# Xneonz0/JPEG-DSP-Studio

Measured on AMD Instinct MI355X. Metric: Mpixels/s forward+inverse pipeline @ Q=50 4:2:0; PSNR vs ref, higher is better.
Workload: dtype f32+f64; 1 GPU; 1920x1080 RGB, Q=50, 4:2:0, prefilter=on, 8x8 blocks (BASELINE configs[1]); global_batch_frames=64, pipeline=serial forward then inverse per step, parallelism=frame-shard x1, world_size=1, quant_table=local (one rank)

## Files before the change

### include/jds.h

```cpp
#ifndef JDS_H
#define JDS_H

#include <stdint.h>

#ifdef __cplusplus
extern "C" {
#endif

#define JDS_ABI_VERSION 3

#define JDS_OK       0
#define JDS_EINVAL  (-1)
#define JDS_ENOTSUP (-2)
#define JDS_EHIP    (-3)
#define JDS_ENOMEM  (-4)

#define JDS_SS_444 0
#define JDS_SS_422 1
#define JDS_SS_420 2
#define JDS_SS_GRAY 3

#define JDS_RUN_SSE 1u
#define JDS_RUN_FWD 2u
#define JDS_RUN_INV 4u
// ... 350 lines not shown
  int64_t H, W;
  int32_t has_box;
  float box[4];
  int32_t reserved;
} jds_resize_item;
int jds_resize_info(int32_t* tile_h, int32_t* tile_w, int32_t* max_taps);
int jds_rgb_resize(jds_ctx* ctx, const uint8_t* rgb, int32_t rgb_on_device, int64_t H, int64_t W, const float* box,
                   int64_t out_h, int64_t out_w, int32_t resample, uint8_t* out, int32_t out_on_device);
int jds_rgb_batch_resize(jds_ctx* ctx, const uint8_t* rgb_base_dev, const jds_resize_item* items, int32_t n,
                         int64_t out_h, int64_t out_w, int32_t resample, uint8_t* out_dev, void* stream);
int jds_jpeg_batch_to_tensor(jds_ctx* ctx, const uint8_t* const* data, const int64_t* lens, int32_t n, int64_t out_h,
                             int64_t out_w, int32_t resample, const int32_t* scale_denoms, const float* boxes,
                             uint8_t* out, int64_t out_cap, int32_t out_on_device, jds_jpeg_batch_item* items,
                             jds_jpeg_scaled_item* scaled, uint32_t* rounds_out);
int jds_selftest_resize(const uint8_t* rgb, int64_t H, int64_t W, const float* box, int64_t out_h, int64_t out_w,
                        int32_t resample, uint8_t* out, int64_t* worst);
int jds_selftest_resize_coeffs(int32_t in_size, float in0, float in1, int32_t out_size, int32_t resample,
                               int32_t* ksize, int32_t* bounds, int32_t* taps, int64_t cap);

#define JDS_PJPEG_MAX_SCANS 64
typedef struct {
  int32_t n_components;
  int32_t component[3];
  int32_t dc_table[3], ac_table[3];
  int32_t ss, se, ah, al;
  int32_t restart_interval;
  int32_t reserved;
  int64_t offset, length;
  int64_t dc_dht[3], ac_dht[3];
} jds_pjpeg_scan;

typedef struct {
  jds_jpeg_info frame;
  int32_t n_scans;
  int32_t complete;
  uint32_t status;
  uint32_t reserved;
  jds_pjpeg_scan scan[JDS_PJPEG_MAX_SCANS];
} jds_pjpeg_info;

int jds_pjpeg_parse(const uint8_t* data, int64_t len, jds_pjpeg_info* out);
int jds_pjpeg_decode(jds_ctx* ctx, const uint8_t* data, int64_t len, int16_t* coeffs, int64_t coeffs_cap,
                     jds_pjpeg_info* info);
int jds_pjpeg_decode_dev(jds_ctx* ctx, const uint8_t* data, int64_t len, int16_t* coeffs_dev, int64_t coeffs_cap,
                         jds_pjpeg_info* info);
int jds_selftest_pjpegdec(const uint8_t* data, int64_t len, int16_t* coeffs, int64_t coeffs_cap, jds_pjpeg_info* info);
int jds_pjpeg_scan_times(jds_ctx* ctx, double* us, int64_t cap, int64_t* count);
int jds_pjpeg_batch_layout(const uint8_t* const* data, const int64_t* lens, int32_t n, jds_jpeg_batch_item* items,
                           int64_t* rgb_bytes, int64_t* coef_entries, const int32_t* scale_denoms,
                           jds_jpeg_scaled_item* scaled);
int jds_pjpeg_batch_to_rgb(jds_ctx* ctx, const uint8_t* const* data, const int64_t* lens, int32_t n, uint8_t* rgb,
                           int64_t rgb_cap, int32_t rgb_on_device, int32_t render, const int32_t* scale_denoms,
                           jds_jpeg_batch_item* items, jds_jpeg_scaled_item* scaled, int16_t* coeffs);
int jds_pjpeg_to_rgb(jds_ctx* ctx, const uint8_t* data, int64_t len, uint8_t* rgb_out, int64_t rgb_cap,
                     int32_t rgb_on_device, int32_t render, int32_t scale_denom, int16_t* coeffs,
                     jds_pjpeg_info* info);
int jds_pjpeg_batch_transcode(jds_ctx* ctx, const uint8_t* const* data, const int64_t* lens, int32_t n,
                              int32_t optimize, uint8_t* out, int64_t out_cap, int32_t out_on_device,
                              jds_jpeg_transcode_item* items, int64_t* out_bytes);
int jds_pjpeg_transcode(jds_ctx* ctx, const uint8_t* data, int64_t len, int32_t optimize, uint8_t* out,
                        int64_t out_cap, int64_t* out_len, jds_pjpeg_info* info);

int jds_selftest_huffdec(const uint8_t* data, int64_t len, int32_t subseq_bits, int16_t* coeffs, int64_t coeffs_cap,
                         int32_t* rounds_out);

int jds_selftest_dct8x8(const double* in, double* out, int64_t n, int32_t inverse);
int jds_selftest_dct16x16(const double* in, double* out, int64_t n, int32_t inverse);

int jds_selftest_fwd32(int32_t subsampling, int32_t prefilter, const double* gauss, const uint8_t* rgb, int64_t H,
                       int64_t W, int32_t plane, int32_t rows_first, float* coeffs, double* bound);
int jds_selftest_fwd16(int32_t subsampling, int32_t prefilter, const double* gauss, const uint8_t* rgb, int64_t H,
                       int64_t W, int32_t plane, int32_t rows_first, float* coeffs, double* bound);

int jds_selftest_inv_fast(int32_t subsampling, const int16_t* coeffs, const double* qtable, int64_t H, int64_t W,
                          int32_t fuse, double* values, uint8_t* bytes);

int jds_selftest_inv_cert(const double* values, int64_t n, uint8_t* bytes, uint8_t* certain, double* consts);

int jds_selftest_inv_fast16(int32_t subsampling, const int16_t* coeffs, const double* qtable, int64_t H, int64_t W,
                            int32_t fuse, double* values, uint8_t* bytes);

int jds_selftest_inv_rows(int32_t subsampling, int64_t H, int32_t ty, int32_t* out, uint8_t* need);

int jds_selftest_area_tab(int32_t src, int32_t dst, int32_t* n, int32_t* si, double* a);

#ifdef __cplusplus
}
#endif

#endif
```

### jpeg-dsp-studio_amd/csrc/jds_abi.hip

```cpp
#include <algorithm>
#include <mutex>
#include <new>
#include <string>

#include "jds_abi.hpp"
#include "jds_dct16.hpp"
#include "jds_dct8.hpp"

#ifdef JDS_INV6
#define JDS_INV6_LIST 1
#else
#define JDS_INV6_LIST 0
#endif

static const double SSIM_C1 = (0.01 * 255) * (0.01 * 255);
static const double SSIM_C2 = (0.03 * 255) * (0.03 * 255);

thread_local char g_err[512] = "";

constexpr int SSIM_ROWS_MIN = 32;
constexpr size_t SSIM_SCRATCH = (size_t)16 << 30;

static int run_ssim_batch(jds_ctx* c, int items, const uint8_t* const* a, const uint8_t* const* b, int H, int W,
                          double* out, int out_stride, unsigned long long* sse) {
// ... 3 lines not shown
  auto bytes_of = [&](int k) {
    return ssim_batch_scratch_doubles(H, W, !rows, ssim_batch_planes(k)) * sizeof(double) * (size_t)k;
  };
  int group = std::min(per, items);
  if (bytes_of(group) > budget) {
    const size_t each_np = ssim_batch_scratch_doubles(H, W, !rows, false) * sizeof(double);
    group = (int)std::max<size_t>(1, std::min<size_t>((size_t)group, budget / each_np));
    if (ssim_batch_planes(group) && bytes_of(group) > budget) {
      const size_t each_p = ssim_batch_scratch_doubles(H, W, !rows, true) * sizeof(double);
      group = (int)std::max<size_t>(1, std::min<size_t>((size_t)group, budget / each_p));
    }
  }
  size_t need = bytes_of(group);
  const int last = items % group;
  if (last) need = std::max(need, bytes_of(last));
  HIP_TRY(c->ss_planes.ensure(need));
  if (!c->ss_side) {
    HIP_TRY(hipStreamCreateWithFlags(&c->ss_side, hipStreamNonBlocking));
    HIP_TRY(hipEventCreateWithFlags(&c->ss_fork, hipEventDisableTiming));
    HIP_TRY(hipEventCreateWithFlags(&c->ss_join, hipEventDisableTiming));
  }
  const size_t pbytes = sizeof(const void*) * 2 * (size_t)items;
  if (c->ss_pairs_cap < pbytes) {
    if (c->ss_pairs_host) HIP_TRY(hipHostFree(c->ss_pairs_host));
    c->ss_pairs_host = nullptr;
    c->ss_pairs_cap = 0;
    HIP_TRY(hipHostMalloc(&c->ss_pairs_host, pbytes, hipHostMallocDefault));
    c->ss_pairs_cap = pbytes;
  }
  const void** ph = (const void**)c->ss_pairs_host;
  for (int i = 0; i < items; ++i) {
    ph[2 * i] = a[i];
    ph[2 * i + 1] = b[i];
  }
  HIP_TRY(c->ss_pairs.ensure(pbytes));
  HIP_TRY(hipMemcpyAsync(c->ss_pairs.p, ph, pbytes, hipMemcpyHostToDevice, c->stream));
  auto pairs_at = [&](int i0) { return (const void*)((const char*)c->ss_pairs.p + sizeof(const void*) * 2 * (size_t)i0); };
  if (sse) HIP_TRY(hipMemsetAsync(sse, 0, sizeof(unsigned long long) * items, c->stream));
  if (rows) {
    const size_t each_rgb = ssim_rgb_scratch_doubles(H, W) * sizeof(double);
    const int group_rgb = (int)std::min<size_t>((size_t)items, std::max<size_t>(1, ((size_t)4 << 30) / each_rgb));
    HIP_TRY(c->ss_rgb.ensure(each_rgb * group_rgb));
    HIP_TRY(hipEventRecord(c->ss_fork, c->stream));
    HIP_TRY(hipStreamWaitEvent(c->ss_side, c->ss_fork, 0));
    for (int i0 = 0; i0 < items; i0 += group_rgb) {
      const int k = std::min(group_rgb, items - i0);
#ifdef JDS_SSIM_PROBE_NORGB
      continue;
#endif
      HIP_TRY(launch_ssim_rgb(pairs_at(i0), k, H, W, SSIM_C1, SSIM_C2, (double*)c->ss_rgb.p,
                              out + (size_t)i0 * out_stride, out_stride, c->ss_side));
    }
    HIP_TRY(hipEventRecord(c->ss_join, c->ss_side));
  }
  for (int i0 = 0; i0 < items; i0 += group) {
    const int k = std::min(group, items - i0);
#ifdef JDS_SSIM_PROBE_NOLUMA
    if (rows) continue;
#endif
    HIP_TRY(launch_psnr_ssim_batch(pairs_at(i0), k, H, W, SSIM_C1, SSIM_C2, (double*)c->ss_planes.p,
                                   out + (size_t)i0 * out_stride, out_stride, sse ? sse + i0 : nullptr, c->stream,
                                   !rows, c->ss_side, c->ss_fork, c->ss_join));
  }
  if (rows) HIP_TRY(hipStreamWaitEvent(c->stream, c->ss_join, 0));
  return JDS_OK;
}

static int run_ssim(jds_ctx* c, const uint8_t* a, const uint8_t* b, int H, int W, double* dres) {
  return run_ssim_batch(c, 1, &a, &b, H, W, dres, 5, nullptr);
}

struct jds_plan {
  jds_ctx* ctx = nullptr;
  int n = 0, mode = 0;
  int nq = 1;
  DevBuf dct32;
  bool pf = false;
  Geo g{};
  DevBuf fq, gk, part;
  DevBuf fq32, gk32, fixbits, fixlist, counters, part32;
  DevBuf invfix;
  DevBuf invlist;
  unsigned inv_runs = 0;
  bool last_inv_fast = false;
  bool inv_fast_ok = true;
  bool inv_fast_any = true;
  bool last_fwd16_fast = false;
  unsigned fwd16_runs = 0;
  unsigned fwd8_runs = 0;
  int last_fwd8_bank = -1;
  InvFix inv_fix() const {
    return {(unsigned*)invfix.p, (unsigned*)invfix.p + 16, 0, (int)(inv_runs & 1u), (int)(inv_runs % 3u),
            (int)(inv_runs % 16u == 15u), (uint2*)invlist.p, 0};
  }
  bool apriori_ok = false;
  DevBuf planes;
  double* qt = nullptr;
  DevBuf ent[8], ent_hdr, ent_tab;
  DevBuf dec_tab, dec_scr, dec_info;
  unsigned dec_rounds = 0;
  DevBuf rst_hdr, rst_work;
  int rst_hdr_interval = 0;
  DevBuf gen_tab, gen_sub, gen_rec;
  GenBufs gen() const { return {(const AreaTap*)gen_tab.p, (double*)gen_sub.p, (double*)gen_rec.p}; }
  bool prof_on = false;
  KMarks marks;
};

namespace jds {
thread_local KMarks* t_kmarks = nullptr;

void kmark(hipStream_t s, const char* fmt, ...) {
  KMarks* m = t_kmarks;
  if (!m) return;
  if (m->n >= m->cap) {
    m->dropped++;
    return;
  }
  if (hipEventRecord(m->ev[m->n], s) != hipSuccess) return;
  va_list ap;
  va_start(ap, fmt);
  vsnprintf(m->name[m->n], sizeof m->name[0], fmt, ap);
  va_end(ap);
  m->n++;
}
}

struct MarkScope {
  explicit MarkScope(jds_plan* p, hipStream_t s) {
    if (!p->prof_on) return;
    t_kmarks = &p->marks;
    kmark(s, "(between runs)");
  }
  ~MarkScope() { t_kmarks = nullptr; }
};

static void marks_release(KMarks& m) {
  for (int i = 0; i < m.cap; ++i) (void)hipEventDestroy(m.ev[i]);
  free(m.ev);
  free(m.name);
  m = KMarks{};
}


static int make_geo(const jds_params* p, int64_t H, int64_t W, Geo* g, int* mode_out, bool* pf_out) {
  if (!p || !g) return fail(JDS_EINVAL, "null argument");
  if (p->block_size != 8 && p->block_size != 16)
    return fail(JDS_ENOTSUP, "operands could not be broadcast together with shapes (%d,%d) (8,8) ",
                p->block_size, p->block_size);
  const int B = p->block_size;
  if (p->subsampling < JDS_SS_444 || p->subsampling > JDS_SS_420)
    return fail(JDS_EINVAL, "Unknown subsampling mode: %d", p->subsampling);
  if (int rc = check_taps(p->gauss, p->subsampling, p->prefilter)) return rc;
  if (H < 1 || W < 1 || H > 65536 || W > 65536 || H * W > (int64_t)1 << 28)
    return fail(JDS_EINVAL, "unsupported image size %lldx%lld", (long long)H, (long long)W);
  const int mode = p->subsampling;
  const int sy = mode == JDS_SS_420 ? 2 : 1, sx = mode == JDS_SS_444 ? 1 : 2;
  if (H / sy < 1 || W / sx < 1)
    return fail(JDS_EINVAL,
                "OpenCV(4.8.0) resize.cpp: error: (-215:Assertion failed) !dsize.empty() in function 'resize' "
                "(image %lldx%lld, %s)",
                (long long)H, (long long)W, mode == JDS_SS_420 ? "4:2:0" : "4:2:2");
  const bool gen = (sy == 2 && (H % 2)) || (sx == 2 && (W % 2));
  if (gen && B == 16)
    return fail(JDS_ENOTSUP, "16x16 blocks with an odd %s image size (%lldx%lld) are not supported",
                mode == JDS_SS_420 ? "4:2:0" : "4:2:2", (long long)H, (long long)W);
// ... 262 lines not shown
  if ((e = p->fq.ensure(sizeof(FrameQ) * n)) != hipSuccess || (e = p->gk.ensure(3 * sizeof(double))) != hipSuccess ||
      (e = p->part.ensure(sizeof(double) * (size_t)n *
                          (size_t)std::max(std::max(g.tiles_y * g.tiles_x, g.gen ? gen_px_tiles(g) : 0),
                                           g.bs == 16 ? inv16_tiles(mode, (int)H, (int)W) : 0))) !=
          hipSuccess ||
      (e = hipMemcpy(p->fq.p, hq, sizeof(FrameQ) * n, hipMemcpyHostToDevice)) != hipSuccess ||
      (e = hipMemcpy(p->gk.p, params[0].gauss, 3 * sizeof(double), hipMemcpyHostToDevice)) != hipSuccess) {
    free(hq);
    p->fq.release();
    p->gk.release();
    p->part.release();
    delete p;
    return fail(e == hipErrorOutOfMemory ? JDS_ENOMEM : JDS_EHIP, "plan upload: %s", hipGetErrorString(e));
  }
  free(hq);
  if (g.gen) {
    if ((rc = gen_prepare(g, n_frames, n, p->gen_tab, p->gen_sub, p->gen_rec, ctx->stream))) {
      jds_plan_destroy(p);
      return rc;
    }
  } else if (g.bs == 16) {
    const size_t fqs = fast_q16_size();
    char* h16 = (char*)malloc(fqs * (size_t)n);
    if (!h16) {
      jds_plan_destroy(p);
      return fail(JDS_ENOMEM, "host allocation failed");
    }
    for (int i = 0; i < n; ++i) fast_fwd16_thresholds(params[i].qtable, mode, pf, params[i].gauss, h16 + fqs * i);
    float gk32[5];
    combined_taps32(params[0].gauss, gk32);
    const size_t nblk = (size_t)n * (size_t)(g.cpf / 256);
    if ((e = p->planes.ensure(mode == JDS_SS_444 ? sizeof(double) * 2 * (size_t)n * g.hc * g.wc : 8)) !=
            hipSuccess ||
        (e = p->fq32.ensure(fqs * n)) != hipSuccess || (e = p->gk32.ensure(sizeof gk32)) != hipSuccess ||
        (e = p->fixlist.ensure(8 * nblk)) != hipSuccess || (e = p->counters.ensure(64)) != hipSuccess ||
        (e = p->invfix.ensure(64 + 12 * (size_t)n)) != hipSuccess ||
        (e = hipMemset(p->invfix.p, 0, 64 + 12 * (size_t)n)) != hipSuccess ||
        (e = p->part32.ensure(sizeof(uint32_t) * 52 * (size_t)n * g.tiles_y * g.tiles_x)) != hipSuccess ||
        (e = hipMemcpy(p->fq32.p, h16, fqs * n, hipMemcpyHostToDevice)) != hipSuccess ||
        (e = hipMemcpy(p->gk32.p, gk32, sizeof gk32, hipMemcpyHostToDevice)) != hipSuccess ||
        (e = hipMemset(p->counters.p, 0, 64)) != hipSuccess) {
      free(h16);
      jds_plan_destroy(p);
      return fail(e == hipErrorOutOfMemory ? JDS_ENOMEM : JDS_EHIP, "plan upload: %s", hipGetErrorString(e));
    }
    free(h16);
  } else {
    const size_t fqs = fast_q_size();
    char* h32 = (char*)malloc(fqs * (size_t)n);
    if (!h32) {
      jds_plan_destroy(p);
      return fail(JDS_ENOMEM, "host allocation failed");
    }
    for (int i = 0; i < n; ++i) {
      float* f = (float*)(h32 + fqs * i);
      fast_fwd_thresholds(params[i].qtable, mode, pf, params[i].gauss, f, f + 64);
    }
    const double* gs = params[0].gauss;
    float gk32[5];
    combined_taps32(gs, gk32);
    const size_t nblk = (size_t)n * (size_t)(g.cpf / 64);
    const size_t ptiles = (size_t)(n_q > 1 ? quant_mq_tiles(g) : g.tiles_y * g.tiles_x);
    if ((e = p->fq32.ensure(fqs * n)) != hipSuccess || (e = p->gk32.ensure(sizeof gk32)) != hipSuccess ||
        (e = p->fixbits.ensure(4 * (size_t)n * (size_t)fix_wpi(g))) != hipSuccess ||
        (e = p->fixlist.ensure(8 * nblk)) != hipSuccess ||
        (e = p->counters.ensure(8 * (size_t)n + 64)) != hipSuccess ||
        (e = p->part32.ensure(sizeof(uint32_t) * (n_q > 1 ? 52 * (size_t)n * ptiles
                                                          : std::max((size_t)52 * n * ptiles, fast_part_words(g, n))))) !=
            hipSuccess ||
        (e = hipMemset(p->part32.p, 0, p->part32.n)) != hipSuccess ||
        (e = p->invfix.ensure(64 + 12 * (size_t)n)) != hipSuccess ||
        (e = hipMemset(p->invfix.p, 0, 64 + 12 * (size_t)n)) != hipSuccess ||
        (JDS_INV6_LIST && mode == JDS_SS_420 && (e = p->invlist.ensure(8 * (size_t)n * inv_tiles(mode, (int)H, (int)W))) != hipSuccess) ||
        (n_q > 1 && (e = p->dct32.ensure(sizeof(float) * (size_t)n_frames * g.cpf)) != hipSuccess) ||
        (e = hipMemcpy(p->fq32.p, h32, fqs * n, hipMemcpyHostToDevice)) != hipSuccess ||
        (e = hipMemcpy(p->gk32.p, gk32, sizeof gk32, hipMemcpyHostToDevice)) != hipSuccess ||
        (e = hipMemset(p->counters.p, 0, 8 * (size_t)n + 64)) != hipSuccess ||
        (e = hipMemset(p->fixbits.p, 0, 4 * (size_t)n * (size_t)fix_wpi(g))) != hipSuccess) {
      free(h32);
      jds_plan_destroy(p);
      return fail(e == hipErrorOutOfMemory ? JDS_ENOMEM : JDS_EHIP, "plan upload: %s", hipGetErrorString(e));
    }
    free(h32);
    if (p->inv_fast_any && !p->inv_fast_ok) {
      std::vector<unsigned> seed(3 * (size_t)n, 0u);
      const unsigned nt = (unsigned)inv_tiles(mode, (int)H, (int)W);
      for (int i = 0; i < n; ++i)
        if (params[i].qtable[0] > 60.0) seed[i] = seed[n + i] = seed[2 * (size_t)n + i] = nt;
      if ((e = hipMemcpy((unsigned*)p->invfix.p + 16, seed.data(), sizeof(unsigned) * seed.size(),
                         hipMemcpyHostToDevice)) != hipSuccess) {
        jds_plan_destroy(p);
        return fail(JDS_EHIP, "plan upload: %s", hipGetErrorString(e));
      }
    }
  }
  *out = p;
  return JDS_OK;
}

int jds_plan_fix_counts(const jds_plan* p, uint32_t* counts) {
  if (!p || !counts) return fail(JDS_EINVAL, "null argument");
  counts[0] = counts[1] = 0u;
  if (p->g.bs == 16) {
    hipError_t e = hipDeviceSynchronize();
    if (e == hipSuccess && p->last_fwd16_fast)
      e = hipMemcpy(counts, (const uint32_t*)p->counters.p + 2, 4, hipMemcpyDeviceToHost);
    if (e == hipSuccess && p->last_inv_fast)
      e = hipMemcpy(counts + 1, (const uint32_t*)p->invfix.p + ((p->inv_runs + 1u) & 1u), 4, hipMemcpyDeviceToHost);
    if (e != hipSuccess) return fail(JDS_EHIP, "fix_counts: %s", hipGetErrorString(e));
    return JDS_OK;
  }
  if (p->g.gen || p->counters.n < 8 * (size_t)p->n) return JDS_OK;
  uint32_t* c = (uint32_t*)malloc(4 * (size_t)p->n + 4);
  if (!c) return fail(JDS_ENOMEM, "fix_counts: host allocation");
  hipError_t e = hipDeviceSynchronize();
  const int bank = p->nq > 1 ? 1 : (p->last_fwd8_bank < 0 ? 1 : p->last_fwd8_bank);
  if (e == hipSuccess)
    e = hipMemcpy(c, (const uint32_t*)p->counters.p + bank * p->n, 4 * (size_t)p->n, hipMemcpyDeviceToHost);
  if (e == hipSuccess && p->last_inv_fast)
    e = hipMemcpy(c + p->n, (const uint32_t*)p->invfix.p + ((p->inv_runs + 1u) & 1u), 4, hipMemcpyDeviceToHost);
  if (e != hipSuccess) {
    free(c);
    return fail(JDS_EHIP, "fix_counts: %s", hipGetErrorString(e));
  }
  for (int i = 0; i < p->n; ++i) counts[0] += std::min(c[i], (uint32_t)(p->g.cpf / 64));
  counts[1] = p->last_inv_fast ? c[p->n] : 0u;
  free(c);
  return JDS_OK;
}

int jds_plan_geometry(const jds_plan* p, jds_geometry* out) {
  if (!p || !out) return fail(JDS_EINVAL, "null argument");
  fill_geometry(p->g, p->mode, out);
  return JDS_OK;
}

int jds_plan_run(jds_plan* p, const uint8_t* rgb, uint8_t* rgb_out, int16_t* coeffs, jds_frame_stats* stats,
                 uint32_t flags, void* stream) {
  if (!p || !rgb || !rgb_out || !coeffs || !stats) return fail(JDS_EINVAL, "null argument");
  if (((uintptr_t)rgb | (uintptr_t)rgb_out | (uintptr_t)coeffs | (uintptr_t)stats) & 15u)
    return fail(JDS_EINVAL, "rgb, rgb_out, coeffs and stats must be 16-byte aligned");
  hipStream_t s = (hipStream_t)stream;
  const MarkScope marks_(p, s);
  int phases = (flags & JDS_RUN_FWD ? 1 : 0) | (flags & JDS_RUN_INV ? 2 : 0);
  if (!phases) phases = 3;
  const bool exact = (flags & JDS_RUN_EXACT) != 0;
  if (p->g.gen) {
    if (phases & 1) HIP_TRY(hipMemsetAsync(stats, 0, sizeof(jds_frame_stats) * p->n, s));
    const GenBufs gb = p->gen();
    HIP_TRY(launch_codec(p->mode, p->pf, p->g, p->n, rgb, rgb_out, coeffs, (const FrameQ*)p->fq.p,
                         (const double*)p->gk.p, stats, (double*)p->part.p, (flags & JDS_RUN_SSE) != 0, nullptr,
                         nullptr, nullptr, 0, s, nullptr, phases, p->nq, &gb));
    return JDS_OK;
  }
  if (p->g.bs == 16) {
    const Fwd16Fast ff{p->fq32.p, (const float*)p->gk32.p, (uint32_t*)p->part32.p, (uint2*)p->fixlist.p,
                       (unsigned*)p->counters.p,
                       (flags & JDS_RUN_FWD_FIXALL) ? 1 : 0, (int)(p->fwd16_runs & 1u)};
    if (phases & 1) HIP_TRY(hipMemsetAsync(stats, 0, sizeof(jds_frame_stats) * p->n, s));
    InvFix fx16 = p->inv_fix();
    fx16.fix_all = (flags & JDS_RUN_INV_FIXALL) ? 1 : 0;
    const bool fast_inv16 = (phases & 2) && !exact && !(flags & JDS_RUN_EXACT_INV) &&
                            !(flags & JDS_RUN_SSE) && p->mode != JDS_SS_444 && p->invfix.p;
    HIP_TRY(launch_codec16(p->mode, p->pf, p->g, p->n, rgb, rgb_out, coeffs, (const FrameQ*)p->fq.p,
                           (const double*)p->gk.p, stats, (double*)p->part.p, (double*)p->planes.p,
                           (flags & JDS_RUN_SSE) != 0, nullptr, nullptr, s, nullptr, phases, exact ? nullptr : &ff,
                           fast_inv16 ? &fx16 : nullptr));
    if (phases & 1) {
      p->last_fwd16_fast = !exact;
      if (!exact) p->fwd16_runs++;
    }
    if (phases & 2) {
      p->last_inv_fast = fast_inv16;
      if (fast_inv16) p->inv_runs++;
    }
    return JDS_OK;
  }
  if (phases & 1) {
    if (exact) HIP_TRY(hipMemsetAsync(stats, 0, sizeof(jds_frame_stats) * p->n, s));
    if (exact)
      HIP_TRY(launch_codec(p->mode, p->pf, p->g, p->n, rgb, rgb_out, coeffs, (const FrameQ*)p->fq.p,
                           (const double*)p->gk.p, stats, (double*)p->part.p, false, nullptr, nullptr, nullptr, 0,
                           s, nullptr, 1, p->nq, nullptr));
    else
      HIP_TRY(launch_fast_fwd(p->mode, p->pf, p->g, p->n, p->nq, rgb, coeffs, (const FrameQ*)p->fq.p, p->fq32.p,
                              (const double*)p->gk.p, (const float*)p->gk32.p, stats, (uint32_t*)p->part32.p,
                              (uint32_t*)p->fixbits.p, (uint2*)p->fixlist.p, (unsigned*)p->counters.p,
                              (float*)p->dct32.p, s,
                              phases == 1,
                              (int)(p->fwd8_runs & 1u)));
    if (!exact && p->nq == 1) p->last_fwd8_bank = (int)(p->fwd8_runs++ & 1u);
  }
  InvFix fx = p->inv_fix();
  fx.fix_all = (flags & JDS_RUN_INV_FIXALL) ? 1 : 0;
  fx.apriori = phases == 3 && p->apriori_ok;
  const bool exact_inv = exact || (flags & JDS_RUN_EXACT_INV) != 0 || (!p->inv_fast_any && !(flags & JDS_RUN_INV_FAST));
  if (phases & 2)
    HIP_TRY(launch_codec(p->mode, p->pf, p->g, p->n, rgb, rgb_out, coeffs, (const FrameQ*)p->fq.p,
                         (const double*)p->gk.p, stats, (double*)p->part.p, (flags & JDS_RUN_SSE) != 0, nullptr,
                         nullptr, nullptr, 0, s, nullptr, exact ? 6 : (phases == 3 ? 2 | 8 : 2), p->nq, nullptr,
                         exact_inv || !p->invfix.p ? nullptr : &fx));
  if (phases & 2) {
    const bool sse444 = (flags & JDS_RUN_SSE) && p->mode == JDS_SS_444;
    p->last_inv_fast = !exact_inv && p->invfix.p && !sse444;
    if (p->last_inv_fast) p->inv_runs++;
  }
  return JDS_OK;
}

static int marks_enable(KMarks& marks, bool& on, int device, int enable) {
  if (enable && !marks.cap) {
    HIP_TRY(hipSetDevice(device));
    const int cap = 8192;
    KMarks m;
    m.ev = (hipEvent_t*)calloc(cap, sizeof(hipEvent_t));
    m.name = (char(*)[64])calloc(cap, sizeof *m.name);
    if (!m.ev || !m.name) {
      free(m.ev);
      free(m.name);
      return fail(JDS_ENOMEM, "host allocation failed");
    }
    for (; m.cap < cap; ++m.cap) {
      hipError_t e = hipEventCreateWithFlags(&m.ev[m.cap], hipEventDisableSystemFence);
      if (e != hipSuccess) {
        marks_release(m);
        return fail(JDS_EHIP, "hipEventCreate: %s", hipGetErrorString(e));
      }
    }
    marks = m;
  }
  on = enable != 0;
  marks.n = 0;
  marks.dropped = 0;
  return JDS_OK;
}

int jds_plan_profile(jds_plan* p, int enable) {
  if (!p) return fail(JDS_EINVAL, "null argument");
  return marks_enable(p->marks, p->prof_on, p->ctx->device, enable);
}

static int marks_read(KMarks& m, int device, jds_kernel_time* out, int max, int* n_out, double* span_ms) {
  if (!n_out || (max > 0 && !out)) return fail(JDS_EINVAL, "null argument");
  *n_out = 0;
  if (span_ms) *span_ms = 0.0;
  if (m.dropped) {
    const long long d = m.dropped;
    if (m.n) (void)hipEventSynchronize(m.ev[m.n - 1]);
    m.n = 0;
    m.dropped = 0;
    return fail(JDS_EINVAL, "profile overflow: %lld launch marks dropped (pool of %d); read every <= %d runs",
                d, m.cap, m.cap / 8);
  }
  if (m.n < 2) {
    m.n = 0;
    return JDS_OK;
  }
  HIP_TRY(hipSetDevice(device));
  HIP_TRY(hipEventSynchronize(m.ev[m.n - 1]));
  int k = 0;
  for (int i = 1; i < m.n; ++i) {
    float ms = 0.f;
    HIP_TRY(hipEventElapsedTime(&ms, m.ev[i - 1], m.ev[i]));
    int j = 0;
    while (j < k && strncmp(out[j].name, m.name[i], sizeof out[j].name) != 0) ++j;
    if (j == k) {
      if (k == max) continue;
      memset(&out[k], 0, sizeof out[k]);
      snprintf(out[k].name, sizeof out[k].name, "%s", m.name[i]);
      ++k;
    }
    out[j].total_ms += ms;
    out[j].launches += 1;
  }
  if (span_ms) {
    float ms = 0.f;
    HIP_TRY(hipEventElapsedTime(&ms, m.ev[0], m.ev[m.n - 1]));
    *span_ms = ms;
  }
  *n_out = k;
  m.n = 0;
  return JDS_OK;
}

int jds_plan_profile_read(jds_plan* p, jds_kernel_time* out, int max, int* n_out, double* span_ms) {
  if (!p) return fail(JDS_EINVAL, "null argument");
  return marks_read(p->marks, p->ctx->device, out, max, n_out, span_ms);
}

int jds_ctx_profile(jds_ctx* c, int enable) {
  if (!c) return fail(JDS_EINVAL, "null argument");
  return marks_enable(c->marks, c->prof_on, c->device, enable);
}

int jds_ctx_profile_read(jds_ctx* c, jds_kernel_time* out, int max, int* n_out, double* span_ms) {
  if (!c) return fail(JDS_EINVAL, "null argument");
  return marks_read(c->marks, c->device, out, max, n_out, span_ms);
}

void jds_plan_destroy(jds_plan* p) {
  if (!p) return;
  (void)hipSetDevice(p->ctx->device);
  (void)hipStreamSynchronize(p->ctx->stream);
  p->fq.release();
  p->gk.release();
  p->part.release();
  p->fq32.release();
  p->gk32.release();
  p->fixlist.release();
  p->counters.release();
  p->fixbits.release();
  p->part32.release();
  p->invfix.release();
  p->invlist.release();
  p->planes.release();
  p->dct32.release();
  p->gen_tab.release();
  p->gen_sub.release();
  p->gen_rec.release();
  for (DevBuf& b : p->ent) b.release();
  p->ent_hdr.release();
  p->ent_tab.release();
  p->dec_tab.release();
  p->dec_scr.release();
  p->dec_info.release();
  p->rst_hdr.release();
  p->rst_work.release();
  free(p->qt);
  marks_release(p->marks);
  delete p;
}

int jds_compress_reconstruct(jds_ctx* c, const jds_params* prm, const uint8_t* rgb, int64_t H, int64_t W,
                             uint8_t* rgb_out, int16_t* coeffs, jds_frame_stats* stats, double* error_map_y,
                             double* error_map_rgb, int32_t sel_by, int32_t sel_bx, jds_selected_block* sel,
                             int32_t* sel_valid) {
  if (!c || !prm || !rgb || !rgb_out || !stats) return fail(JDS_EINVAL, "null argument");
  if ((error_map_y == nullptr) != (error_map_rgb == nullptr))
    return fail(JDS_EINVAL, "error_map_y and error_map_rgb must be requested together");
  Geo g;
  int mode;
  bool pf;
  int rc = make_geo(prm, H, W, &g, &mode, &pf);
  if (rc) return rc;
  if ((rc = check_tables(prm))) return rc;
  HIP_TRY(hipSetDevice(c->device));
  const size_t npx = (size_t)H * (size_t)W, nimg = npx * 3, ncf = (size_t)g.cpf;
  const int tiles = std::max(std::max(g.tiles_y * g.tiles_x, g.gen ? gen_px_tiles(g) : 0),
                             g.bs == 16 ? inv16_tiles(mode, (int)H, (int)W) : 0);
  HIP_TRY(c->rgb.ensure(nimg));
  HIP_TRY(c->out.ensure(nimg));
  HIP_TRY(c->coeffs.ensure(ncf * sizeof(int16_t)));
  HIP_TRY(c->stats.ensure(sizeof(jds_frame_stats)));
  HIP_TRY(c->part.ensure(sizeof(double) * tiles));
  HIP_TRY(c->fq.ensure(sizeof(FrameQ)));
  HIP_TRY(c->gk.ensure(3 * sizeof(double)));
  const bool maps = error_map_y != nullptr;
  if (maps) {
    HIP_TRY(c->erry.ensure(npx * sizeof(double)));
    HIP_TRY(c->errrgb.ensure(npx * sizeof(double)));
  }
  int sel_blk = -1;
  if (sel && g.bs == 16) {
    if (sel_valid) *sel_valid = 0;
  } else if (sel) {
    const long long bpr = g.nbx;
    const long long ti = (long long)sel_by * bpr + sel_bx;
    const long long nyb = (long long)g.nby * g.nbx;
    if (ti >= 0 && ti < nyb) sel_blk = (int)ti;
    if (sel_valid) *sel_valid = sel_blk >= 0;
    if (sel_blk >= 0) HIP_TRY(c->sel.ensure(sizeof(jds_selected_block)));
  }
  FrameQ hq;
  make_fq(prm, &hq);
  hipStream_t s = c->stream;
  GenBufs gb{};
  if (g.gen) {
    if ((rc = gen_prepare(g, 1, 1, c->gen_tab, c->gen_sub, c->gen_rec, s))) return rc;
    gb = {(const AreaTap*)c->gen_tab.p, (double*)c->gen_sub.p, (double*)c->gen_rec.p};
  }
  HIP_TRY(hipMemcpyAsync(c->fq.p, &hq, sizeof hq, hipMemcpyHostToDevice, s));
  HIP_TRY(hipMemcpyAsync(c->gk.p, prm->gauss, 3 * sizeof(double), hipMemcpyHostToDevice, s));
  HIP_TRY(hipMemcpyAsync(c->rgb.p, rgb, nimg, hipMemcpyHostToDevice, s));
  HIP_TRY(hipMemsetAsync(c->stats.p, 0, sizeof(jds_frame_stats), s));
  jds_selected_block* dsel = sel_blk >= 0 ? (jds_selected_block*)c->sel.p : nullptr;
  if (g.bs == 16) {
// ... 739 lines not shown
    return fail(JDS_EINVAL, "bad argument");
  const bool pf = prefilter != 0 && subsampling != JDS_SS_444;
  double E[128];
  fast_fwd_bounds(subsampling, pf, gauss, E);
  memcpy(bound, E + (plane ? 64 : 0), 64 * sizeof(double));
  if (fwd32_host_plane(subsampling, pf, gauss, rgb, (int)H, (int)W, plane, rows_first, coeffs))
    return fail(JDS_EINVAL, "plane size must be a multiple of 8");
  return JDS_OK;
}

int jds_selftest_fwd16(int32_t subsampling, int32_t prefilter, const double* gauss, const uint8_t* rgb, int64_t H,
                       int64_t W, int32_t plane, int32_t rows_first, float* coeffs, double* bound) {
  if (!gauss || !rgb || !coeffs || !bound || H < 1 || W < 1 || H > 4096 || W > 4096 || plane < 0 || plane > 2 ||
      subsampling < JDS_SS_444 || subsampling > JDS_SS_420)
    return fail(JDS_EINVAL, "bad argument");
  const bool pf = prefilter != 0 && subsampling != JDS_SS_444;
  double E[512];
  fast_fwd16_bounds(subsampling, pf, gauss, E);
  memcpy(bound, E + (plane ? 256 : 0), 256 * sizeof(double));
  if (fwd16_host_plane(subsampling, pf, gauss, rgb, (int)H, (int)W, plane, rows_first, coeffs))
    return fail(JDS_EINVAL, "plane size must be a multiple of 16");
  return JDS_OK;
}

int jds_selftest_inv_fast(int32_t subsampling, const int16_t* coeffs, const double* qtable, int64_t H, int64_t W,
                          int32_t fuse, double* values, uint8_t* bytes) {
  if (!coeffs || !qtable || !values || !bytes || H < 1 || W < 1 || H > 4096 || W > 4096 ||
      subsampling < JDS_SS_444 || subsampling > JDS_SS_420)
    return fail(JDS_EINVAL, "bad argument");
  if (inv_fast_host(subsampling, coeffs, qtable, (int)H, (int)W, fuse, 8, values, bytes))
    return fail(JDS_EINVAL, "odd chroma geometry: the certified inverse runs even sizes only");
  return JDS_OK;
}

int jds_selftest_inv_cert(const double* values, int64_t n, uint8_t* bytes, uint8_t* certain, double* consts) {
  if (!values || !bytes || !certain || !consts || n < 0) return fail(JDS_EINVAL, "bad argument");
  for (int64_t i = 0; i < n; ++i)
    if (!(fabs(values[i]) < 0x1p+19)) return fail(JDS_EINVAL, "values[%lld] outside (-2^19, 2^19)", (long long)i);
  inv_cert_forms_host(values, n, bytes, certain, consts);
  return JDS_OK;
}

int jds_selftest_inv_fast16(int32_t subsampling, const int16_t* coeffs, const double* qtable, int64_t H, int64_t W,
                            int32_t fuse, double* values, uint8_t* bytes) {
  if (!coeffs || !qtable || !values || !bytes || H < 1 || W < 1 || H > 4096 || W > 4096 ||
      subsampling < JDS_SS_444 || subsampling > JDS_SS_420)
    return fail(JDS_EINVAL, "bad argument");
  if (inv_fast_host(subsampling, coeffs, qtable, (int)H, (int)W, fuse, 16, values, bytes))
    return fail(JDS_EINVAL, "odd chroma geometry: the certified inverse runs even sizes only");
  return JDS_OK;
}

int jds_selftest_area_tab(int32_t src, int32_t dst, int32_t* n, int32_t* si, double* a) {
  if (src < 1 || dst < 1 || dst > src || !n || !si || !a) return fail(JDS_EINVAL, "bad argument");
  AreaTap* t = (AreaTap*)malloc(sizeof(AreaTap) * (size_t)dst);
  if (!t) return fail(JDS_ENOMEM, "host allocation failed");
  if (area_tab_build(src, dst, t) < 0) {
    free(t);
    return fail(JDS_EINVAL, "more than 4 taps per sample");
  }
  for (int d = 0; d < dst; ++d) {
    n[d] = t[d].n;
    for (int k = 0; k < 4; ++k) {
      si[4 * d + k] = k < t[d].n ? t[d].si[k] : -1;
      a[4 * d + k] = k < t[d].n ? t[d].a[k] : 0.0;
    }
  }
  free(t);
  return JDS_OK;
}

int jds_selftest_inv_rows(int32_t subsampling, int64_t H, int32_t ty, int32_t* out, uint8_t* need) {
  if (!out || H < 1 || H > 65536 || ty < 0 || subsampling < JDS_SS_444 || subsampling > JDS_SS_420)
    return fail(JDS_EINVAL, "bad argument");
  int o[8];
  inv_rows(subsampling, (int)H, ty, o);
  for (int i = 0; i < 8; ++i) out[i] = o[i];
  if (need)
    for (int i = 0; i < o[5]; ++i)
      for (int r = 0; r < 8; ++r) need[8 * i + r] = (uint8_t)inv_rows_need(subsampling, (int)H, ty, o[4] + i, r);
  return JDS_OK;
}

int jds_selftest_dct16x16(const double* in, double* out, int64_t n, int32_t inverse) {
  if (!in || !out || n < 0) return fail(JDS_EINVAL, "bad argument");
  for (int64_t b = 0; b < n; ++b) {
    double t[256], c[16];
    memcpy(t, in + 256 * b, sizeof t);
    for (int col = 0; col < 16; ++col) {
      for (int i = 0; i < 16; ++i) c[i] = t[i * 16 + col];
      if (inverse) dct3_line16(c); else dct2_line16(c);
      for (int i = 0; i < 16; ++i) t[i * 16 + col] = c[i];
    }
    for (int r = 0; r < 16; ++r) {
      if (inverse) dct3_line16(t + 16 * r); else dct2_line16(t + 16 * r);
    }
    for (int i = 0; i < 256; ++i) out[256 * b + i] = t[i] * 0.03125;
  }
  return JDS_OK;
}

}
```

### jpeg-dsp-studio_amd/csrc/jds_abi.hpp

```cpp
#pragma once

#include <hip/hip_runtime.h>
#include <math.h>
#include <stdarg.h>
#include <stdio.h>
#include <stdlib.h>
#include <string.h>

#include <cmath>
#include <thread>
#include <vector>

#include "jds_huffdec.hpp"
#include "jds_huffopt.hpp"
#include "jds_internal.hpp"
#include "jds_jpeg_inv.hpp"

namespace jds {
hipError_t launch_codec(int mode, bool pf, const Geo& g, int n, const uint8_t* rgb, uint8_t* rgb_out,
                        int16_t* coeffs, const FrameQ* fq, const double* gk, jds_frame_stats* st,
                        double* part, bool want_sse, double* err_y, double* err_rgb, jds_selected_block* sel,
                        int sel_blk, hipStream_t s, hipEvent_t* ev, int phases, int in_div, const GenBufs* gb,
                        const InvFix* fx = nullptr);
int inv_tiles(int mode, int H, int W);
void inv_rows(int mode, int H, int ty, int* out);
int inv_rows_need(int mode, int H, int ty, int by, int r);
int area_tab_build(int src, int dst, AreaTap* tab);
size_t gen_sub_doubles(const Geo& g);
size_t gen_rec_doubles(const Geo& g);
int gen_px_tiles(const Geo& g);
hipError_t stage_area_gen(const double* in, int H, int W, const AreaTap* ytab, const AreaTap* xtab, double* out,
                          int oh, int ow, hipStream_t s);
hipError_t launch_psnr_ssim_batch(const void* pairs_dev, int items, int H, int W, double c1, double c2,
                                  double* scratch, double* out, int out_stride, unsigned long long* sse,
                                  hipStream_t s, bool rgb, hipStream_t side, hipEvent_t fork, hipEvent_t join);
hipError_t launch_ssim_rgb(const void* pairs_dev, int items, int H, int W, double c1, double c2, double* scratch,
                           double* out, int out_stride, hipStream_t s);
size_t ssim_batch_scratch_doubles(int H, int W, bool rgb, bool planes);
bool ssim_batch_planes(int items);
size_t ssim_rgb_scratch_doubles(int H, int W);
int ssim_batch_max_items();
hipError_t launch_sse_u8(const uint8_t* a, const uint8_t* b, long long n, unsigned long long* out, hipStream_t s);
size_t mag_scratch_bytes(long long nblocks, int max_chunks);
hipError_t launch_mag_f32(const int16_t* coeffs, long long nblocks, unsigned* chunk_sum, int max_chunks,
                          double* out, hipStream_t s);
void combined_taps32(const double* gk, float* out5);
size_t fast_part_words(const Geo& g, int n);
hipError_t launch_fast_fwd(int mode, bool pf, const Geo& g, int n, int nq, const uint8_t* rgb, int16_t* coeffs,
                           const FrameQ* fq, const void* fq32, const double* gk, const float* gk32,
                           jds_frame_stats* st, uint32_t* part, uint32_t* fixbits, uint2* fixlist, unsigned* fixcount,
                           float* dct32,
                           hipStream_t s, bool finish, int par);
int quant_mq_tiles(const Geo& g);
int inv16_tiles(int mode, int H, int W);
constexpr int MAXQ_SHARED = 8;
void fast_fwd_bounds(int mode, bool pf, const double* gk, double* E);
int fwd32_host_plane(int mode, bool pf, const double* gk, const uint8_t* rgb, int H, int W, int plane,
                     int flags, float* out);
void fast_fwd_thresholds(const double* Q, int mode, bool pf, const double* gk, float* rq, float* thr);
int inv_fast_host(int mode, const int16_t* cf, const double* Q, int H, int W, int fuse, int block, double* vout,
                  uint8_t* bout);
void inv_cert_forms_host(const double* v, long long n, uint8_t* bytes, uint8_t* certain, double* consts);
size_t fast_q_size();
hipError_t stage_rgb_ycc(const double* in, double* out, long long n, int inverse, hipStream_t s);
hipError_t stage_subsample(const double* in, double* tmp, double* tmp2, double* out, int H, int W, int sy,
                           int prefilter, const double* k, hipStream_t s);
hipError_t stage_resize(const double* in, int h, int w, double* out, int H, int W, int nearest, hipStream_t s);
hipError_t stage_block(const double* in, double* out, long long n, int bs, int op, hipStream_t s);
hipError_t stage_quant(const void* in, const double* q, void* out, long long n, int dequant, int period,
                       hipStream_t s);
int tile_dims16(int mode, int* MY, int* MX);
struct EntTab;
void ent_build_tables(EntTab* t);
size_t ent_tab_size();
int ent_header(const double* q, int mode, int H, int W, uint8_t* o);
long long ent_capacity(const Geo& g);
void ent_sizes(const Geo& g, int n, size_t* sz);
hipError_t launch_entropy(const Geo& g, int n, const int16_t* coeffs, void* const* buf, const uint8_t* hdr_dev,
                          const void* tab_dev, uint8_t* out, long long stride, unsigned long long* lengths,
                          unsigned long long* scan_bits, hipStream_t s);
int ent_restart_interval();
int ent_header_rst(const double* q, int mode, int H, int W, int interval, uint8_t* o);
long long ent_capacity_rst(const Geo& g);
hipError_t launch_entropy_rst(const Geo& g, int n, const int16_t* coeffs, void* const* buf, const uint8_t* hdr_dev,
                              const void* tab_dev, uint8_t* out, long long stride, unsigned long long* lengths,
                              unsigned long long* scan_bits, hipStream_t s);
long long ent_capacity_opt(const Geo& g, bool rst);
hipError_t launch_entropy_opt(const Geo& g, int n, const int16_t* coeffs, void* const* buf, const uint8_t* hdr_dev,
                              const void* tab_dev, uint8_t* out, long long stride, unsigned long long* lengths,
                              unsigned long long* scan_bits, hipStream_t s);
hipError_t launch_entropy_rst_opt(const Geo& g, int n, const int16_t* coeffs, void* const* buf,
                                  const uint8_t* hdr_dev, const void* tab_dev, uint8_t* out, long long stride,
                                  unsigned long long* lengths, unsigned long long* scan_bits, hipStream_t s);
int ent_std_table(int idx, const uint8_t** bits, const uint8_t** vals);
void opt_table_host(const uint32_t* freq, HoTable* t);
hipError_t launch_opt_tables_selftest(int n, const uint32_t* freq, uint8_t* bits, uint8_t* vals, int32_t* nv,
                                      int32_t* fell, hipStream_t s);
void rst_constants(int* lane_max);
int rst_group_lanes();
size_t rst_work_bytes(int n, const RstGeo& rg);
hipError_t launch_dec_rst(const uint8_t* files, const RstIv* ivs_dev, long long niv, const HuffDecTab* tabs_dev,
                          int16_t* coeffs, uint32_t* status, hipStream_t s, const HdMcu* mcu_dev);
hipError_t launch_dec_rst_plan(const uint8_t* files, long long stride, const unsigned long long* lengths,
                               const uint8_t* hdr_dev, int hl, int n, const RstGeo& rg, void* work,
                               const HuffDecTab* tabs_dev, int16_t* coeffs, uint32_t* status, hipStream_t s);
void dec_constants(int* s, int* g);
long long dec_layout(DecScan* sc, int nscans, int* max_ngrp);
size_t dec_scratch_bytes(long long ngroups, int nscans);
size_t dec_hdr_bytes(int n);
hipError_t launch_dec_hdr(const uint8_t* files, long long stride, const unsigned long long* lengths,
                          const uint8_t* hdr_dev, int hl, int n, void* work, uint32_t* status, hipStream_t s);
hipError_t dec_run(const uint8_t* files, const DecScan* sc, int nscans, long long ngroups, int max_ngrp,
                   const HuffDecTab* tabs_dev, void* scratch, int16_t* coeffs, long long n_coeffs, uint32_t* status,
                   hipStream_t s, unsigned* rounds, int* too_many, const HdMcu* mcu_dev, int16_t* dcs);
hipError_t dec_run_groups(const uint8_t* files, const DecGroup* grp, int ngrp, const HuffDecTab* tabs_dev,
                          int16_t* coeffs, long long n_coeffs, uint32_t* status, hipStream_t s, unsigned* rounds,
                          int* too_many, const HdMcu* mcu_dev, int16_t* dcs);
hipError_t launch_codec16(int mode, bool pf, const Geo& g, int n, const uint8_t* rgb, uint8_t* rgb_out,
                          int16_t* coeffs, const FrameQ* fq, const double* gk, jds_frame_stats* st, double* part,
                          double* planes, bool want_sse, double* err_y, double* err_rgb, hipStream_t s,
                          hipEvent_t* ev, int phases, const Fwd16Fast* ff, const InvFix* fx);
void fast_fwd16_bounds(int mode, bool pf, const double* gk, double* E);
void fast_fwd16_thresholds(const double* Q8, int mode, bool pf, const double* gk, void* out);
size_t fast_q16_size();
int fwd16_host_plane(int mode, bool pf, const double* gk, const uint8_t* rgb, int H, int W, int plane,
                     int flags, float* out);
void jpeg_inv_constants(int* th, int* tw);
bool jpeg_inv_fits(const JInvArgs& a);
hipError_t launch_jpeg_inv(const JInvArgs& a, const int16_t* coeffs, uint8_t* rgb, hipStream_t s);
void jpeg_inv_host(const JInvArgs& a, const int16_t* coeffs, uint8_t* rgb);
hipError_t launch_jpeg_inv_batch(const JInvRec* recs, const JInvMap* maps, const int map_off[JI_MODES],
                                 const int nmap[JI_MODES], const int tiles[JI_MODES], const uint32_t* status,
                                 const int16_t* coeffs, uint8_t* rgb, hipStream_t s);
hipError_t launch_jpeg_ljt(const JInvArgs& a, const int16_t* coeffs, uint8_t* rgb, hipStream_t s);
hipError_t launch_jpeg_ljt_batch(const JInvRec* recs, const JInvMap* maps, const int map_off[JI_MODES],
// ... 159 lines not shown
```

### jpeg-dsp-studio_amd/csrc/jds_fast.hip

```cpp
#include <hip/hip_runtime.h>
#include <math.h>
#include <stdint.h>
#include <stdlib.h>

#include "jds_dct8.hpp"
#include "jds_device.hpp"
#include "jds_internal.hpp"
#include "jds_fwd_common.hpp"

#pragma clang fp contract(off)


namespace jds {

#define JA 0x1.6a09e6p-2f
#define JC1 0x1.f6297cp-2f
#define JC2 0x1.d906bcp-2f
#define JC3 0x1.a9b662p-2f
#define JC5 0x1.1c73b4p-2f
#define JC6 0x1.87de2ap-3f
#define JC7 0x1.8f8b84p-4f

static constexpr float FW[8][4] = {
    {JA, JA, JA, JA},      {JC1, JC3, JC5, JC7},    {JC2, JC6, -JC6, -JC2}, {JC3, -JC7, -JC1, -JC5},
    {JA, -JA, -JA, JA},    {JC5, -JC1, JC7, JC3},   {JC6, -JC2, JC2, -JC6}, {JC7, -JC5, JC3, -JC1},
};

__host__ __device__ __forceinline__ void fdct8_f32(float (&x)[8]) {
  const float s0 = x[0] + x[7], s1 = x[1] + x[6], s2 = x[2] + x[5], s3 = x[3] + x[4];
  const float d0 = x[0] - x[7], d1 = x[1] - x[6], d2 = x[2] - x[5], d3 = x[3] - x[4];
#pragma unroll
  for (int k = 0; k < 8; k += 2) {
    x[k] = fmaf(FW[k][3], s3, fmaf(FW[k][2], s2, fmaf(FW[k][1], s1, FW[k][0] * s0)));
    x[k + 1] = fmaf(FW[k + 1][3], d3, fmaf(FW[k + 1][2], d2, fmaf(FW[k + 1][1], d1, FW[k + 1][0] * d0)));
  }
}

__device__ __forceinline__ void unpack32(uint32_t v, float& R, float& G, float& B) {
  R = (float)(v & 255u);
  G = (float)((v >> 8) & 255u);
  B = (float)(v >> 16);
}

struct FastQ {
  float rq[64];
  float thr[2][64];
};

constexpr int BS32 = 72;

template <int SY>
__device__ __forceinline__ int csw(int row) { return (row / SY) & 3; }

template <int SY>
__device__ __forceinline__ int psw(int row) { return (row / SY) & 7; }

__device__ __forceinline__ uint32_t byte_at(const uint32_t (&w)[6], int b) { return (w[b >> 2] >> (8 * (b & 3))) & 255u; }

struct LaneStats {
  unsigned nz = 0u, mb = 0u, hn = 0u, nflag = 0u;
};

constexpr int RH_COPIES = 4, RH_STRIDE = 53;
constexpr int RH_WORDS = RH_COPIES * RH_STRIDE + 64;

__device__ __forceinline__ unsigned rare_bin_total(const unsigned* s_rh, int b) {
  unsigned t = 0u;
#pragma unroll
  for (int c = 0; c < RH_COPIES; ++c) t += s_rh[c * RH_STRIDE + b] + (b == 49 ? s_rh[c * RH_STRIDE + 50] : 0u);
  return t;
}

template <bool REPL = false>
__device__ __forceinline__ void quant8(const float (&v)[8], const float (&rq)[8], const float (&thr)[8], bool valid,
                                       int (&q)[8], LaneStats& ls, unsigned* s_st) {
  unsigned nrare = 0u;
  unsigned ok = 0xffffffffu, orr = 0u;
  unsigned top;
  asm("v_mov_b32 %0, 0x80000000" : "=v"(top));
#pragma unroll
  for (int k = 0; k < 8; ++k) {
    const float t = v[k] * rq[k];
    const float f = t + QMAGIC;
    const float r = f - QMAGIC;
    const uint32_t fb = __float_as_uint(f);
    const float e = fabsf(t - r) - fmaf(fabsf(t), -0x1p-22f, thr[k]);
    ok &= __float_as_uint(e);
    q[k] = (int)(fb - QMAGIC_BITS);
    const int x = __builtin_amdgcn_frexp_expf(r);
    ls.nz += (unsigned)(x + 15) >> 4;
    ls.mb += (unsigned)x;
    const unsigned o = fb - (QMAGIC_BITS - 12u);
    ls.hn += top >> ((o & 28u) ^ 31u);
    orr |= o;
  }
  ls.nflag += (~ok) >> 31;
  nrare = REPL ? orr : (orr >= 32u ? 1u : 0u);
  if constexpr (REPL) {
    if (nrare >= 32u) {
      const int lane = threadIdx.x & 63;
      unsigned* copy = s_st + (lane & (RH_COPIES - 1)) * RH_STRIDE;
      unsigned* dummy = s_st + RH_COPIES * RH_STRIDE + lane;
#pragma unroll
      for (int k = 0; k < 8; ++k) {
        const unsigned o = (unsigned)(q[k] + 12);
        const bool rare = o >= 32u;
        ls.hn -= rare ? 1u << (o & 28u) : 0u;
        const unsigned h = (unsigned)(q[k] + 100);
        atomicAdd(rare && valid && h <= 200u ? copy + (h >> 2) : dummy, 1u);
      }
    }
  } else if (nrare != 0u) {
#pragma unroll
    for (int k = 0; k < 8; ++k) {
      const unsigned o = (unsigned)(q[k] + 12);
      if (o >= 32u) {
        ls.hn -= 1u << (o & 28u);
        if (valid && (unsigned)(q[k] + 100) <= 200u) atomicAdd(&s_st[2 + (q[k] == 100 ? 49 : (q[k] + 100) >> 2)], 1u);
      }
    }
  }
}

__device__ __forceinline__ uint4 pack_q(const int (&q)[8]) {
  return make_uint4((uint32_t)(uint16_t)q[0] | ((uint32_t)(uint16_t)q[1] << 16),
                    (uint32_t)(uint16_t)q[2] | ((uint32_t)(uint16_t)q[3] << 16),
                    (uint32_t)(uint16_t)q[4] | ((uint32_t)(uint16_t)q[5] << 16),
                    (uint32_t)(uint16_t)q[6] | ((uint32_t)(uint16_t)q[7] << 16));
}

__device__ __forceinline__ void flag_block_list(const LaneStats& ls, bool valid, int line, int item, int plane,
                                                int bidx, uint2* fixlist, unsigned* fixcount, long long cap) {
  const unsigned long long fm = __ballot(valid && ls.nflag != 0u);
  if (!fm) return;
  const int lane = threadIdx.x & 63;
  const bool mine = valid && line == 0 && ((fm >> (lane & ~7)) & 0xffull);
  const unsigned long long lm = __ballot(mine);
  unsigned base = 0u;
  if (lane == __ffsll((long long)lm) - 1) base = atomicAdd(fixcount + item, (unsigned)__popcll(lm));
  base = __shfl(base, __ffsll((long long)lm) - 1, 64);
  if (mine) {
    const unsigned slot = base + (unsigned)__popcll(lm & ((1ull << lane) - 1ull));
    if (slot < (unsigned long long)cap)
      fixlist[(size_t)item * cap + slot] = make_uint2((unsigned)item, ((unsigned)plane << 24) | (unsigned)bidx);
  }
}

__device__ __forceinline__ void flag_block_bits(const LaneStats& ls, bool valid, int line, int item, long long gblk,
                                                uint32_t* fixbits, int wpi) {
  const unsigned long long fm = __ballot(valid && ls.nflag != 0u);
  if (!fm) return;
  const int lane = threadIdx.x & 63;
  if (valid && line == 0 && ((fm >> (lane & ~7)) & 0xffull))
    atomicOr(fixbits + (size_t)item * wpi + (gblk >> 5), 1u << (gblk & 31));
}

constexpr int NW_MAX = 8;
__device__ __forceinline__ void stats_flush(LaneStats ls, bool valid, uint32_t* __restrict__ slot) {
  if (!valid) ls = LaneStats();
  const unsigned h = ls.hn;
  unsigned v[3] = {h & 0x0f0f0f0fu, (h >> 4) & 0x0f0f0f0fu, ls.nz | ((valid ? 1u : 0u) << 8) | (ls.mb << 16)};
  row_sums3(v);
  const int lane = threadIdx.x & 63, w = threadIdx.x >> 6;
  if ((lane & 15) == 15)
    *reinterpret_cast<uint4*>(slot + 4 * (4 * w + (lane >> 4))) = make_uint4(v[0], v[1], v[2], 0u);
}

constexpr int PSLOT = 128;
__device__ __forceinline__ unsigned* rare_row(uint32_t* part, const Geo& g, int nframes, int frame) {
  return part + (size_t)nframes * g.tiles_y * g.tiles_x * PSLOT + (size_t)frame * 64;
}

template <int MODE, bool PF, bool MQ = false>
__global__ void __launch_bounds__(Cfg<MODE>::TF)
k_fwd32(const Geo g, const uint8_t* __restrict__ rgb, int16_t* __restrict__ coeffs,
        const FastQ* __restrict__ fq, const float* __restrict__ gk32, uint32_t* __restrict__ part,
        uint2* __restrict__ fixlist, unsigned* __restrict__ fixcount, const int border, const int4 rect,
        float* __restrict__ dct32,
        jds_frame_stats* __restrict__ stz, const int nzq) {
  using C = Cfg<MODE>;
  constexpr int WR = C::TH + 2, WC = C::TW + 2, WN = WR * WC;
  constexpr bool CPLANE = (MODE != M444) && PF;
  constexpr int BLK_F = C::NB * BS32;
  constexpr int GPL_F = CPLANE ? 2 * WN : 0;
  constexpr int U_F = GPL_F > BLK_F ? GPL_F : BLK_F;
  static_assert((WN * 4) % 16 == 0, "plane alignment");

  __shared__ uint32_t s_rgb[WN];
  __shared__ __attribute__((aligned(16))) float s_u[U_F];
  __shared__ __attribute__((aligned(16))) float s_rq[64];
  __shared__ __attribute__((aligned(16))) float s_thr[2][64];

  const int tid = threadIdx.x;
  const int frame = blockIdx.y;
  int ty, tx;
  if (stz != nullptr && blockIdx.x == 0) {
    uint64_t* z = reinterpret_cast<uint64_t*>(stz + (size_t)frame * nzq);
    for (int i = tid; i < nzq * (int)(sizeof(jds_frame_stats) / 8); i += blockDim.x) z[i] = 0ull;
    if (MQ && tid < nzq) fixcount[gridDim.y * nzq + frame * nzq + tid] = 0u;
  }
  if (border) {
    int e = blockIdx.x;
    const int top = rect.x * g.tiles_x, bottom = (g.tiles_y - 1 - rect.y) * g.tiles_x;
    const int rows = rect.y - rect.x + 1, left = rect.z * rows;
    if (e < top) {
      ty = e / g.tiles_x;
      tx = e - ty * g.tiles_x;
    } else if ((e -= top) < bottom) {
      ty = rect.y + 1 + e / g.tiles_x;
      tx = e - (ty - rect.y - 1) * g.tiles_x;
    } else if ((e -= bottom) < left) {
      ty = rect.x + e / rect.z;
      tx = e - (ty - rect.x) * rect.z;
    } else {
      e -= left;
      const int nr = g.tiles_x - 1 - rect.w;
      ty = rect.x + e / nr;
      tx = rect.w + 1 + e - (ty - rect.x) * nr;
    }
  } else {
    ty = blockIdx.x / g.tiles_x;
    tx = blockIdx.x - ty * g.tiles_x;
  }
  const int m0y = ty * C::MY - g.ty_off, m0x = tx * C::MX - g.tx_off;
  const int y0 = m0y * C::MH, x0 = m0x * C::MW;
  const uint8_t* img = rgb + (size_t)frame * g.H * g.W * 3;
  if (!MQ && tid < 64) {
    s_rq[tid] = fq[frame].rq[tid];
    s_thr[0][tid] = fq[frame].thr[0][tid];
    s_thr[1][tid] = fq[frame].thr[1][tid];
  }

  const int blk = tid >> 3, line = tid & 7;
  int plane, by_t, bx_t;
  if (blk < C::NYB) {
    plane = 0;
    by_t = blk / C::YBC;
    bx_t = blk % C::YBC;
  } else {
    const int bi = (blk - C::NYB) % C::NCB;
    plane = 1 + (blk - C::NYB) / C::NCB;
    by_t = bi / C::CBC;
    bx_t = bi % C::CBC;
  }
  const int gy = plane == 0 ? m0y * C::SY + by_t : m0y + by_t;
  const int gx = plane == 0 ? m0x * C::SX + bx_t : m0x + bx_t;
  const int nby = plane ? g.ncy : g.nby, nbx = plane ? g.ncx : g.nbx;
  const bool valid = gy >= 0 && gx >= 0 && gy < nby && gx < nbx;
  const int bidx = gy * nbx + gx;
  const float k0 = gk32[0], k1 = gk32[1], k2 = gk32[2];
  float v[8];

  const bool inside = y0 - 1 >= 0 && x0 - 1 >= 0 && y0 + C::TH + 1 <= g.H && x0 + C::TW + 1 <= g.W;
  constexpr int NL = (WN + C::TF - 1) / C::TF;
  {
    uint32_t px[NL];
#pragma unroll
    for (int l = 0; l < NL; ++l) {
      const int i = tid + l * C::TF;
      px[l] = 0u;
      if (i < WN) {
        const int r = i / WC, c = i - r * WC;
// ... 56 lines not shown
    if (plane == 0 || MODE == M444) {
      const int sx = reflect_pad(gx * 8 + line, g.W) - x0 + 1;
#pragma unroll
      for (int i = 0; i < 8; ++i) {
        const int sy = reflect_pad(gy * 8 + i, g.H) - y0 + 1;
        float R, G, B;
        unpack32(s_rgb[sy * WC + sx], R, G, B);
        v[i] = plane == 0 ? luma32(R, G, B) - 128.0f : (plane == 1 ? cb32m(R, G, B) : cr32m(R, G, B));
      }
    } else if constexpr (CPLANE) {
      constexpr int HW = C::TW / 2;
      const float* s_pl = s_u + (plane == 1 ? 0 : WN) + (reflect_pad(gx * 8 + line, g.wc) - x0 / C::SX);
#pragma unroll
      for (int i = 0; i < 8; ++i) {
        const int wr0 = C::SY * reflect_pad(gy * 8 + i, g.hc) - y0 + 1;
        const float* col = s_pl + wr0 * HW;
        if constexpr (C::SY == 2)
          v[i] = fmaf(k2, col[2 * HW], fmaf(gk32[4], col[HW], fmaf(gk32[3], col[0], k0 * col[-HW]))) * 0.25f;
        else
          v[i] = fmaf(k0, col[HW] + col[-HW], k1 * col[0]) * 0.5f;
      }
    } else {
      const float* s_pl = s_u + (plane == 1 ? 0 : WN);
      const int sc = reflect_pad(gx * 8 + line, g.wc);
      const int wc0 = C::SX * sc - x0 + 1;
#pragma unroll
      for (int i = 0; i < 8; ++i) {
        const int sr = reflect_pad(gy * 8 + i, g.hc);
        const int wr0 = C::SY * sr - y0 + 1;
        float s[C::SY][2];
#pragma unroll
        for (int a = 0; a < C::SY; ++a) {
#pragma unroll
          for (int b = 0; b < 2; ++b) {
            const int w = (wr0 + a) * WC + wc0 + b;
            {
              float R, G, B;
              unpack32(s_rgb[w], R, G, B);
              s[a][b] = plane == 1 ? cb32m(R, G, B) : cr32m(R, G, B);
            }
          }
        }
        if constexpr (C::SY == 2)
          v[i] = (((s[0][0] + s[0][1]) + s[1][0]) + s[1][1]) * 0.25f;
        else
          v[i] = (s[0][0] + s[0][1]) * 0.5f;
      }
    }
    fdct8_f32(v);
  }
  if constexpr (CPLANE) __syncthreads();
  float* s_blk = s_u + blk * BS32;
  if (valid) {
#pragma unroll
    for (int i = 0; i < 8; ++i) s_blk[i * 8 + line] = v[i];
  }
  __syncthreads();

  const int u = line;
#pragma unroll
  for (int k = 0; k < 8; ++k) v[k] = valid ? s_blk[u * 8 + k] : 0.0f;
  fdct8_f32(v);
  if constexpr (MQ) {
    if (valid) {
      float4* d = reinterpret_cast<float4*>(dct32 + (long long)frame * g.cpf +
                                            (plane == 0 ? 0 : (plane == 1 ? g.off_cb : g.off_cr)) +
                                            (long long)bidx * 64 + u * 8);
      d[0] = make_float4(v[0], v[1], v[2], v[3]);
      d[1] = make_float4(v[4], v[5], v[6], v[7]);
    }
    return;
  }
  const float4* rq4 = reinterpret_cast<const float4*>(s_rq + u * 8);
  const float4* th4 = reinterpret_cast<const float4*>(s_thr[plane ? 1 : 0] + u * 8);
  const float4 ra = rq4[0], rb = rq4[1], ta = th4[0], tb = th4[1];
  const float rq[8] = {ra.x, ra.y, ra.z, ra.w, rb.x, rb.y, rb.z, rb.w};
  const float thr[8] = {ta.x, ta.y, ta.z, ta.w, tb.x, tb.y, tb.z, tb.w};
  int q[8];
  LaneStats ls;
  quant8(v, rq, thr, valid, q, ls, rare_row(part, g, gridDim.y, frame));
  if (valid)
    *reinterpret_cast<uint4*>(coeffs + (long long)frame * g.cpf + (plane == 0 ? 0 : (plane == 1 ? g.off_cb : g.off_cr)) +
                              (long long)bidx * 64 + u * 8) = pack_q(q);
  flag_block_list(ls, valid, line, frame, plane, bidx, fixlist, fixcount, g.cpf / 64);
  stats_flush(ls, valid, part + ((size_t)frame * g.tiles_y * g.tiles_x + ty * g.tiles_x + tx) * PSLOT);
}

template <int MODE, bool PF, bool MQ = false>
__global__ void __launch_bounds__(Cfg<MODE>::TF)
k_fwd32i(const Geo g, const uint8_t* __restrict__ rgb, int16_t* __restrict__ coeffs,
         const FastQ* __restrict__ fq, const float* __restrict__ gk32, uint32_t* __restrict__ part,
         uint2* __restrict__ fixlist, unsigned* __restrict__ fixcount, const int4 rect,
         float* __restrict__ dct32,
         jds_frame_stats* __restrict__ stz, const int nzq) {
  using C = Cfg<MODE>;
  constexpr int TH = C::TH, TW = C::TW, WR = TH + 2, SEG = TW / 8;
  static_assert(16 % SEG == 0, "staging segment groups tile the 16-lane DPP rows");
  constexpr bool SUB = MODE != M444;
  constexpr bool CPLANE = SUB && PF;
  constexpr int CR = SUB ? (CPLANE ? WR : TH) : TH;
  constexpr int NCD = SUB ? 2 * C::NCB : 1;
  constexpr int YS = TW;
  __shared__ __attribute__((aligned(16))) float s_y[TH * YS];
  constexpr int CW = CPLANE ? TW / 2 : TW;
  __shared__ __attribute__((aligned(16))) float s_c[2 * CR * CW];
  __shared__ __attribute__((aligned(16))) float s_cd[NCD * BS32];
  __shared__ __attribute__((aligned(16))) float s_rqT[64];
  __shared__ __attribute__((aligned(16))) float s_thT[2][64];

  const int tid = threadIdx.x, frame = blockIdx.y;
  const int ncol = rect.w - rect.z + 1;
  if (stz != nullptr && blockIdx.x == 0) {
    uint64_t* z = reinterpret_cast<uint64_t*>(stz + (size_t)frame * nzq);
    for (int i = tid; i < nzq * (int)(sizeof(jds_frame_stats) / 8); i += blockDim.x) z[i] = 0ull;
    if (MQ && tid < nzq) fixcount[gridDim.y * nzq + frame * nzq + tid] = 0u;
  }
  const int ty = rect.x + (int)blockIdx.x / ncol, tx = rect.z + (int)blockIdx.x % ncol;
  const int m0y = ty * C::MY - g.ty_off, m0x = tx * C::MX - g.tx_off;
  const int y0 = m0y * C::MH, x0 = m0x * C::MW;
  const uint8_t* img = rgb + (size_t)frame * g.H * g.W * 3;
  static_assert((TH + 2) * (TW / 8) <= Cfg<MODE>::TF - 64, "the last wave is idle in the staging pass");
  if (!MQ && tid >= Cfg<MODE>::TF - 64) {
    const int l = tid - (Cfg<MODE>::TF - 64);
    const int t = (l & 7) * 8 + (l >> 3);
    s_rqT[l] = fq[frame].rq[t];
    s_thT[0][l] = fq[frame].thr[0][t];
    s_thT[1][l] = fq[frame].thr[1][t];
  }
  const float k0 = gk32[0], k1 = gk32[1], k2 = gk32[2];
  float* s_cb = s_c;
  float* s_cr = s_c + CR * CW;

  if (tid < WR * SEG) {
    const int r = tid < TH * SEG ? 1 + tid / SEG : (tid < (TH + 1) * SEG ? 0 : TH + 1), c = tid % SEG;
    if (CPLANE || (r >= 1 && r <= TH)) {
      int yrow = y0 - 1 + r;
      yrow = yrow < 0 ? -yrow : (yrow >= g.H ? 2 * g.H - 2 - yrow : yrow);
      const uint8_t* p = img + ((size_t)yrow * g.W + x0 + 8 * c) * 3;
      const uint2* p2 = reinterpret_cast<const uint2*>(p);
      const bool left_edge = x0 == 0, right_edge = x0 + TW == g.W;
      const uint2 a = p2[0], b = p2[1], d = p2[2];
      const uint2 ring = CPLANE ? p2[c == 0 ? (left_edge ? 0 : -1) : (right_edge ? 0 : 3)] : make_uint2(0u, 0u);
      const uint32_t w[6] = {a.x, a.y, b.x, b.y, d.x, d.y};
      float yy[8], cb[8], cr[8];
#pragma unroll
      for (int k = 0; k < 8; ++k) {
        const float R = (float)byte_at(w, 3 * k), G = (float)byte_at(w, 3 * k + 1), B = (float)byte_at(w, 3 * k + 2);
        yy[k] = luma32m(R, G, B);
        cb[k] = cb32m(R, G, B);
        cr[k] = cr32m(R, G, B);
      }
      const int o = (r - 1) * TW + 8 * c;
      if (r >= 1 && r <= TH) {
        fdct8_f32(yy);
        float4* dy = reinterpret_cast<float4*>(s_y + (r - 1) * YS + 8 * c);
        dy[0] = make_float4(yy[0], yy[1], yy[2], yy[3]);
        dy[1] = make_float4(yy[4], yy[5], yy[6], yy[7]);
      }
      if constexpr (!SUB) {
        if (r >= 1 && r <= TH) {
          fdct8_f32(cb);
          fdct8_f32(cr);
          float4* db = reinterpret_cast<float4*>(s_cb + o);
          float4* dr = reinterpret_cast<float4*>(s_cr + o);
          db[0] = make_float4(cb[0], cb[1], cb[2], cb[3]);
          db[1] = make_float4(cb[4], cb[5], cb[6], cb[7]);
          dr[0] = make_float4(cr[0], cr[1], cr[2], cr[3]);
          dr[1] = make_float4(cr[4], cr[5], cr[6], cr[7]);
        }
      } else if constexpr (CPLANE) {
        float lb = dpp_f32<0x111>(cb[7]), lr = dpp_f32<0x111>(cr[7]);
        float rb = dpp_f32<0x101>(cb[0]), rr = dpp_f32<0x101>(cr[0]);
        if (c == 0) {
          const float R = (float)((ring.y >> 8) & 255u), G = (float)((ring.y >> 16) & 255u), B = (float)(ring.y >> 24);
          lb = left_edge ? cb[1] : cb32m(R, G, B);
          lr = left_edge ? cr[1] : cr32m(R, G, B);
        }
// ... 73 lines not shown
    int q[8];
    quant8(v, rq, thr, valid, q, ls, rare_row(part, g, gridDim.y, frame));
    int16_t* tq = reinterpret_cast<int16_t*>(src);
#pragma unroll
    for (int k = 0; k < 8; ++k) tq[k * rs * 2 + line] = (int16_t)q[k];
    __builtin_amdgcn_wave_barrier();
    const uint4 row = *reinterpret_cast<const uint4*>(tq + line * rs * 2);
    if (valid) *reinterpret_cast<uint4*>(dst + line * 8) = row;
  };

  if constexpr (SUB) {
    if (plane == 0) {
      column(s_y + by_t * 8 * YS + bx_t * 8, YS, 0);
    } else {
      const float* P = plane == 1 ? s_cb : s_cr;
      const int i = line;
      int gs = gy * 8 + i;
      gs = (gs < g.hc || !valid) ? gs : 2 * (g.hc - 1) - gs;
      const int pr = C::SY * (gs - m0y * 8);
      const int xc = 2 * bx_t * 8;
      float v[8];
      if constexpr (CPLANE) {
        float R[C::SY + 2][8];
        const int f0 = 2 * bx_t;
#pragma unroll
        for (int j = 0; j < C::SY + 2; ++j) {
          const int hs = psw<C::SY>(pr + j);
          const float4* s4 = reinterpret_cast<const float4*>(P + (pr + j) * CW);
          const float4 x = s4[f0 ^ hs], y = s4[(f0 + 1) ^ hs];
          R[j][0] = x.x; R[j][1] = x.y; R[j][2] = x.z; R[j][3] = x.w;
          R[j][4] = y.x; R[j][5] = y.y; R[j][6] = y.z; R[j][7] = y.w;
        }
#pragma unroll
        for (int jj = 0; jj < 8; ++jj) {
          if constexpr (C::SY == 2)
            v[jj] = fmaf(k2, R[3][jj], fmaf(gk32[4], R[2][jj], fmaf(gk32[3], R[1][jj], k0 * R[0][jj]))) * 0.25f;
          else
            v[jj] = fmaf(k0, R[2][jj] + R[0][jj], k1 * R[1][jj]) * 0.5f;
        }
      } else {
#pragma unroll
      for (int h = 0; h < 2; ++h) {
        float rows[C::SY + 2][8];
#pragma unroll
        for (int j = 0; j < (CPLANE ? C::SY + 2 : C::SY); ++j) {
          const int hs = csw<C::SY>(pr + j), f = (xc + 8 * h) >> 2;
          const float4* s4 = reinterpret_cast<const float4*>(P + (pr + j) * TW);
          const float4 x = s4[f ^ hs], y = s4[(f + 1) ^ hs];
          rows[j][0] = x.x; rows[j][1] = x.y; rows[j][2] = x.z; rows[j][3] = x.w;
          rows[j][4] = y.x; rows[j][5] = y.y; rows[j][6] = y.z; rows[j][7] = y.w;
        }
#pragma unroll
        for (int jj = 0; jj < 4; ++jj) {
          float s[C::SY][2];
#pragma unroll
          for (int aa = 0; aa < C::SY; ++aa) {
#pragma unroll
            for (int bb = 0; bb < 2; ++bb) {
              const int x = 2 * jj + bb;
              if constexpr (CPLANE)
                s[aa][bb] = fmaf(k0, rows[aa + 2][x] + rows[aa][x], k1 * rows[aa + 1][x]);
              else
                s[aa][bb] = rows[aa][x];
            }
          }
          if constexpr (C::SY == 2)
            v[4 * h + jj] = (((s[0][0] + s[0][1]) + s[1][0]) + s[1][1]) * 0.25f;
          else
            v[4 * h + jj] = (s[0][0] + s[0][1]) * 0.5f;
        }
      }
      }
      fdct8_f32(v);
      float4* d4 = reinterpret_cast<float4*>(s_cd + (blk - C::NYB) * BS32 + i * 8);
      d4[0] = make_float4(v[0], v[1], v[2], v[3]);
      d4[1] = make_float4(v[4], v[5], v[6], v[7]);
      column(s_cd + (blk - C::NYB) * BS32, 8, plane);
    }
  } else {
    float* P = plane == 0 ? s_y : (plane == 1 ? s_cb : s_cr);
    column(P + by_t * 8 * TW + bx_t * 8, TW, plane);
  }
  if constexpr (!MQ) {
    flag_block_list(ls, valid, line, frame, plane, bidx, fixlist, fixcount, g.cpf / 64);
    stats_flush(ls, valid, part + ((size_t)frame * g.tiles_y * g.tiles_x + ty * g.tiles_x + tx) * PSLOT);
  }
}

constexpr int F444_WAVES = 4;

__global__ void __launch_bounds__(64 * F444_WAVES) __attribute__((amdgpu_waves_per_eu(5)))
k_fwd444w(const Geo g, const uint8_t* __restrict__ rgb, int16_t* __restrict__ coeffs, const FastQ* __restrict__ fq,
          uint32_t* __restrict__ part, uint2* __restrict__ fixlist, unsigned* __restrict__ fixcount,
          jds_frame_stats* __restrict__ stz) {
  __shared__ __attribute__((aligned(16))) float s_blk[8 * F444_WAVES * BS32];
  __shared__ __attribute__((aligned(16))) float s_rqT[64];
  __shared__ __attribute__((aligned(16))) float s_thT[2][64];
  const int tid = threadIdx.x, lv = tid & 7, lb = tid >> 3;
  const int frame = blockIdx.y;
  if (blockIdx.x == 0) {
    uint64_t* z = reinterpret_cast<uint64_t*>(stz + frame);
    for (int i = tid; i < (int)(sizeof(jds_frame_stats) / 8); i += blockDim.x) z[i] = 0ull;
  }
  if (tid < 64) {
    const int t = (tid & 7) * 8 + (tid >> 3);
    s_rqT[tid] = fq[frame].rq[t];
    s_thT[0][tid] = fq[frame].thr[0][t];
    s_thT[1][tid] = fq[frame].thr[1][t];
  }
  __syncthreads();

  const int nblk = g.nby * g.nbx;
  const int blk = blockIdx.x * (8 * F444_WAVES) + lb;
  const bool valid = blk < nblk;
  const int bq = valid ? blk : 0;
  const int by = bq / g.nbx, bx = bq - by * g.nbx;
  const int y = by * 8 + lv, x0 = bx * 8;
  const uint8_t* img = rgb + (size_t)frame * g.H * g.W * 3;
  uint32_t w[6];
  {
    const int yr = reflect_pad(y, g.H);
    const uint8_t* row = img + (size_t)yr * g.W * 3;
    if (x0 + 8 <= g.W && (g.W & 7) == 0) {
      const uint2* p2 = reinterpret_cast<const uint2*>(row + (size_t)x0 * 3);
      const uint2 a = p2[0], b = p2[1], c = p2[2];
      w[0] = a.x; w[1] = a.y; w[2] = b.x; w[3] = b.y; w[4] = c.x; w[5] = c.y;
    } else {
#pragma unroll
      for (int i = 0; i < 6; ++i) w[i] = 0u;
#pragma unroll
      for (int k = 0; k < 8; ++k) {
        const uint8_t* px = row + (size_t)reflect_pad(x0 + k, g.W) * 3;
#pragma unroll
        for (int c = 0; c < 3; ++c) w[(3 * k + c) >> 2] |= (uint32_t)px[c] << (8 * ((3 * k + c) & 3));
      }
    }
  }

  LaneStats ls;
  unsigned acc[4] = {0u, 0u, 0u, 0u};
  float* slot = s_blk + lb * BS32;
  int16_t* tq = reinterpret_cast<int16_t*>(slot);
#pragma unroll
  for (int p = 0; p < 3; ++p) {
    float v[8];
#pragma unroll
    for (int k = 0; k < 8; ++k) {
      const float R = (float)byte_at(w, 3 * k), G = (float)byte_at(w, 3 * k + 1), B = (float)byte_at(w, 3 * k + 2);
      v[k] = p == 0 ? luma32m(R, G, B) : (p == 1 ? cb32m(R, G, B) : cr32m(R, G, B));
    }
    fdct8_f32(v);
    float4* d4 = reinterpret_cast<float4*>(slot + lv * 8);
    d4[0] = make_float4(v[0], v[1], v[2], v[3]);
    d4[1] = make_float4(v[4], v[5], v[6], v[7]);
    __builtin_amdgcn_wave_barrier();
    float c[8];
#pragma unroll
    for (int i = 0; i < 8; ++i) c[i] = slot[i * 8 + lv];
    fdct8_f32(c);
    const float4* rq4 = reinterpret_cast<const float4*>(s_rqT + lv * 8);
    const float4* th4 = reinterpret_cast<const float4*>(s_thT[p ? 1 : 0] + lv * 8);
    const float4 ra = rq4[0], rb = rq4[1], ta = th4[0], tb = th4[1];
    const float rq[8] = {ra.x, ra.y, ra.z, ra.w, rb.x, rb.y, rb.z, rb.w};
    const float thr[8] = {ta.x, ta.y, ta.z, ta.w, tb.x, tb.y, tb.z, tb.w};
    int q[8];
    ls.hn = 0u;
    ls.nflag = 0u;
// ... 410 lines not shown
    const int bidx = (int)(b - (plane == 0 ? 0 : (plane == 1 ? nyb : nyb + ncb)));
    const float v[8] = {nx.x, nx.y, nx.z, nx.w, ny.x, ny.y, ny.z, ny.w};
    nrows += valid ? 1u : 0u;
    if (rw + step < rows) { nx = src[(rw + step) * 2]; ny = src[(rw + step) * 2 + 1]; }
#pragma unroll
    for (int q = 0; q < MAXQ; ++q) {
      if (q < nq) {
        const float4* rq4 = reinterpret_cast<const float4*>(&s_rq[q][u * 8]);
        const float4* th4 = reinterpret_cast<const float4*>(&s_th[q][plane ? 1 : 0][u * 8]);
        const float4 ra = rq4[0], rb = rq4[1], ta = th4[0], tb = th4[1];
        const float rq[8] = {ra.x, ra.y, ra.z, ra.w, rb.x, rb.y, rb.z, rb.w};
        const float thr[8] = {ta.x, ta.y, ta.z, ta.w, tb.x, tb.y, tb.z, tb.w};
        int qv[8];
        LaneStats ls;
        quant8<true>(v, rq, thr, valid, qv, ls, s_rh[q]);
        const int item = f * nq + q;
        if (valid) *reinterpret_cast<uint4*>(coeffs + (long long)item * g.cpf + rw * 8) = pack_q(qv);
        flag_block_bits(ls, valid, u, item, b, fixbits, fix_wpi(g));
        if (valid) {
          nz[q] += ls.nz;
          mb[q] += ls.mb;
          be[q] += ls.hn & 0x0f0f0f0fu;
          bo[q] += (ls.hn >> 4) & 0x0f0f0f0fu;
        }
      }
    }
  }
  const unsigned wrows = __reduce_add_sync(~0ull, nrows);
#pragma unroll
  for (int q = 0; q < MAXQ; ++q) {
    if (q < nq) {
      const unsigned w0 = __reduce_add_sync(~0ull, be[q] & 0x00ff00ffu), w1 = __reduce_add_sync(~0ull, (be[q] >> 8) & 0x00ff00ffu);
      const unsigned w2 = __reduce_add_sync(~0ull, bo[q] & 0x00ff00ffu), w3 = __reduce_add_sync(~0ull, (bo[q] >> 8) & 0x00ff00ffu);
      const unsigned wmb = __reduce_add_sync(~0ull, mb[q]), wnz = __reduce_add_sync(~0ull, nz[q]);
      if ((tid & 63) == 0) {
        atomicAdd(&s_st[q][0], wnz);
        atomicAdd(&s_st[q][1], wmb + wnz);
        const unsigned zeros = 8u * wrows - wnz;
        const unsigned c[8] = {w0 & 0xffffu, w2 & 0xffffu, w1 & 0xffffu, (w3 & 0xffffu) - zeros,
                               w0 >> 16,     w2 >> 16,     w1 >> 16,     w3 >> 16};
#pragma unroll
        for (int j = 0; j < 8; ++j)
          if (c[j]) atomicAdd(&s_st[q][2 + 22 + j], c[j]);
      }
    }
  }
  __syncthreads();
  for (int i = tid; i < nq * NSTAT; i += 256) {
    const int q = i / NSTAT, j = i - q * NSTAT;
    part[((size_t)(f * nq + q) * ptiles + blockIdx.x) * NSTAT + j] =
        s_st[q][j] + (j >= 2 ? rare_bin_total(s_rh[q], j - 2) : 0u);
  }
}


hipError_t launch_fwd_finish(const Geo& g, int n, jds_frame_stats* st, const uint32_t* part, int ptiles,
                             hipStream_t s);
template <int MODE>
static void fold_rows(const Geo& g, int4& rect) {
  using C = Cfg<MODE>;
  if (g.H % 8 != 0 || g.H < C::TH + 2) return;
  if (rect.x == 1) {
    const int y0 = -g.ty_off * C::MH;
    if (1 - y0 <= g.H - 1) rect.x = 0;
  }
  if (rect.y == g.tiles_y - 2) {
    const int y0 = ((g.tiles_y - 1) * C::MY - g.ty_off) * C::MH;
    bool ok = y0 >= 1 && y0 + C::TH <= 2 * g.H - 2;
    const int hp = g.ncy * 8;
    if (MODE != M444 && hp > g.hc) {
      const int rmin = 2 * (g.hc - 1) - (hp - 1);
      ok = ok && rmin >= 0 && C::SY * rmin >= y0;
    }
    if (ok) rect.y = g.tiles_y - 1;
  }
}

constexpr int FIX_GRID = 16384;

template <int MODE, bool PF>
static hipError_t fast_fwd_t(const Geo& g, int n, int nq, const uint8_t* rgb, int16_t* coeffs, const FrameQ* fq,
                             const FastQ* fq32, const double* gk, const float* gk32, jds_frame_stats* st,
                             uint32_t* part, uint32_t* fixbits, uint2* fixlist, unsigned* fixcount, float* dct32, hipStream_t s,
                             bool finish, int par) {
  using C = Cfg<MODE>;
  const bool mq = nq > 1;
  const int nf = n / nq;
  unsigned* const fc = mq ? fixcount : fixcount + par * n;
  if (MODE == M444 && !mq) {
    const int ng = fwd444w_groups(g);
    hipLaunchKernelGGL(k_fwd444w, dim3(ng, n), dim3(64 * F444_WAVES), 0, s, g, rgb, coeffs, fq32, part, fixlist, fc, st);
    kmark(s, "k_fwd444w");
    hipError_t e = hipGetLastError();
    if (e != hipSuccess) return e;
    const int gx = FIX_GRID / n > 1 ? FIX_GRID / n : 1;
    static_assert(F444_WAVES * 4 == 16, "16 row records per k_fwd444w workgroup");
    const int nred = (ng + FIX_RED_TILES - 1) / FIX_RED_TILES;
    hipLaunchKernelGGL((k_fix_fwd<MODE, PF, 16, 1>), dim3(gx + nred, n), dim3(64), 0, s, g, rgb, coeffs, fq, gk, st,
                       fixlist, fixcount + par * n, nq, 0, fixcount + (par ^ 1) * n, part, ng, nred);
    kmark(s, "k_fix_fwd<%d,%d>", MODE, (int)PF);
    if ((e = hipGetLastError()) != hipSuccess) return e;
    return finish ? launch_fwd_finish(g, n, st, nullptr, 0, s) : hipSuccess;
  }
  int4 rect;
  rect.x = (g.ty_off * C::MH > 0) ? 1 : 0;
  rect.y = (g.H / C::MH + g.ty_off) / C::MY - 1;
  rect.z = (g.tx_off * C::MW > 0) ? 1 : 0;
  rect.w = (g.W / C::MW + g.tx_off) / C::MX - 1;
  const bool split = (g.W % 8) == 0 && g.H >= 2 && g.W >= 2 && rect.y >= rect.x && rect.w >= rect.z;
  if (split) fold_rows<MODE>(g, rect);
  hipError_t e;
  if (split) {
    const int nin = (rect.y - rect.x + 1) * (rect.w - rect.z + 1), nout = g.tiles_y * g.tiles_x - nin;
    if (nout > 0) {
      if (mq)
        hipLaunchKernelGGL((k_fwd32<MODE, PF, true>), dim3(nout, nf), dim3(C::TF), 0, s, g, rgb, coeffs, fq32, gk32,
                           part, fixlist, fixcount, 1, rect, dct32, nullptr, nq);
      else
        hipLaunchKernelGGL((k_fwd32<MODE, PF>), dim3(nout, n), dim3(C::TF), 0, s, g, rgb, coeffs, fq32, gk32, part,
                           fixlist, fc, 1, rect, nullptr, nullptr, 1);
      kmark(s, "k_fwd32<%d,%d%s>", MODE, (int)PF, mq ? ",mq" : "");
      if ((e = hipGetLastError()) != hipSuccess) return e;
    }
    if (mq)
      hipLaunchKernelGGL((k_fwd32i<MODE, PF, true>), dim3(nin, nf), dim3(C::TF), 0, s, g, rgb, coeffs, fq32, gk32,
                         part, fixlist, fixcount, rect, dct32, st, nq);
    else
      hipLaunchKernelGGL((k_fwd32i<MODE, PF>), dim3(nin, n), dim3(C::TF), 0, s, g, rgb, coeffs, fq32, gk32, part,
                         fixlist, fc, rect, nullptr, st, 1);
    kmark(s, "k_fwd32i<%d,%d%s>", MODE, (int)PF, mq ? ",mq" : "");
    if ((e = hipGetLastError()) != hipSuccess) return e;
  } else {
    if (mq)
      hipLaunchKernelGGL((k_fwd32<MODE, PF, true>), dim3(g.tiles_y * g.tiles_x, nf), dim3(C::TF), 0, s, g, rgb,
                         coeffs, fq32, gk32, part, fixlist, fixcount, 0, rect, dct32, st, nq);
    else
      hipLaunchKernelGGL((k_fwd32<MODE, PF>), dim3(g.tiles_y * g.tiles_x, n), dim3(C::TF), 0, s, g, rgb, coeffs,
                         fq32, gk32, part, fixlist, fc, 0, rect, nullptr, st, 1);
    kmark(s, "k_fwd32<%d,%d%s>", MODE, (int)PF, mq ? ",mq" : "");
    if ((e = hipGetLastError()) != hipSuccess) return e;
  }
  int ptiles = g.tiles_y * g.tiles_x;
  if (mq) {
    ptiles = quant_mq_tiles(g);
    hipLaunchKernelGGL(k_quant_mq, dim3(ptiles, nf), dim3(256), 0, s, g, nq, dct32, coeffs, fq32, part, fixbits);
    kmark(s, "k_quant_mq");
    if ((e = hipGetLastError()) != hipSuccess) return e;
  }
  const int gx = FIX_GRID / n > 1 ? FIX_GRID / n : 1;
  if (!mq) {
    static_assert(C::TF <= 64 * NW_MAX, "row records fit the tile slot");
    const int nred = (ptiles + FIX_RED_TILES - 1) / FIX_RED_TILES;
    hipLaunchKernelGGL((k_fix_fwd<MODE, PF, 4 * (C::TF / 64)>), dim3(gx + nred, n), dim3(64), 0, s, g, rgb, coeffs,
                       fq, gk, st, fixlist, fixcount + par * n, nq, 0, fixcount + (par ^ 1) * n, part, ptiles, nred);
    kmark(s, "k_fix_fwd<%d,%d>", MODE, (int)PF);
    if ((e = hipGetLastError()) != hipSuccess) return e;
    return finish ? launch_fwd_finish(g, n, st, nullptr, 0, s) : hipSuccess;
  }
  hipLaunchKernelGGL(k_fwd_reduce_fix, dim3((ptiles + 63) / 64, n), dim3(512), 0, s, g, st, part, ptiles,
                     fixbits, fixlist, fixcount);
  kmark(s, "k_fwd_reduce_fix");
  if ((e = hipGetLastError()) != hipSuccess) return e;
  if (n < 8192) {
    hipLaunchKernelGGL((k_fix_fwd<MODE, PF>), dim3(FIX_GRID), dim3(64), sizeof(unsigned) * (n + 1), s, g, rgb,
                       coeffs, fq, gk, st, fixlist, fixcount + n, nq, n, nullptr);
    kmark(s, "k_fix_fwd<%d,%d>", MODE, (int)PF);
  } else {
    hipLaunchKernelGGL((k_fix_fwd<MODE, PF>), dim3(gx, n), dim3(64), 0, s, g, rgb, coeffs, fq, gk, st, fixlist,
                       fixcount + n, nq, 0, nullptr);
    kmark(s, "k_fix_fwd<%d,%d>", MODE, (int)PF);
  }
  if ((e = hipGetLastError()) != hipSuccess) return e;
  return finish ? launch_fwd_finish(g, n, st, nullptr, 0, s) : hipSuccess;
}

hipError_t launch_fast_fwd(int mode, bool pf, const Geo& g, int n, int nq, const uint8_t* rgb, int16_t* coeffs,
                           const FrameQ* fq, const void* fq32, const double* gk, const float* gk32,
                           jds_frame_stats* st, uint32_t* part, uint32_t* fixbits, uint2* fixlist, unsigned* fixcount, float* dct32,
                           hipStream_t s, bool finish, int par) {
  const FastQ* f = (const FastQ*)fq32;
  switch (mode) {
    case M420:
      return pf ? fast_fwd_t<M420, true>(g, n, nq, rgb, coeffs, fq, f, gk, gk32, st, part, fixbits, fixlist, fixcount, dct32, s, finish, par)
                : fast_fwd_t<M420, false>(g, n, nq, rgb, coeffs, fq, f, gk, gk32, st, part, fixbits, fixlist, fixcount, dct32, s, finish, par);
    case M422:
      return pf ? fast_fwd_t<M422, true>(g, n, nq, rgb, coeffs, fq, f, gk, gk32, st, part, fixbits, fixlist, fixcount, dct32, s, finish, par)
                : fast_fwd_t<M422, false>(g, n, nq, rgb, coeffs, fq, f, gk, gk32, st, part, fixbits, fixlist, fixcount, dct32, s, finish, par);
    default:
      return fast_fwd_t<M444, false>(g, n, nq, rgb, coeffs, fq, f, gk, gk32, st, part, fixbits, fixlist, fixcount, dct32, s, finish, par);
  }
}


void pass_bound(double X, double e, const double* Xin, const double* ein, double* Xout, double* eout,
                       const double W[8][4]) {
  const double u = 0x1p-24;
  for (int k = 0; k < 8; ++k) {
    double b = 0, P = 0, pre = 0;
    for (int i = 0; i < 4; ++i) {
      b += fabs(W[k][i]);
      pre += fabs(W[k][i]);
      P += pre;
    }
    const double x = Xin ? Xin[0] : X, er = ein ? ein[0] : e;
    Xout[k] = 2 * x * b;
    eout[k] = b * (2 * er + 2 * u * x) + 2 * u * x * (b + P);
  }
}

void combined_taps32(const double* gk, float* out5) {
  out5[0] = (float)gk[0];
  out5[1] = (float)gk[1];
  out5[2] = (float)gk[2];
  out5[3] = (float)(gk[0] + gk[1]);
  out5[4] = (float)(gk[1] + gk[2]);
}

static double combined_chain_error(const double* gk, double X, double e) {
  const double u = 0x1p-24;
  float h[5];
  combined_taps32(gk, h);
  const double hf[4] = {h[0], h[3], h[4], h[2]};
  const double hx[4] = {gk[0], gk[0] + gk[1], gk[1] + gk[2], gk[2]};
  double sh = 0, dh = 0, pre = 0, P = 0;
  for (int i = 0; i < 4; ++i) {
    sh += fabs(hf[i]);
    dh += fabs(hf[i] - hx[i]);
    pre += fabs(hf[i]);
    P += pre;
  }
  return sh * e + dh * X + u * X * P + 1e-12;
}

static double taps_abs_sum(const double* gk) {
  const double A = (fabs(gk[0]) + fabs(gk[1])) + fabs(gk[2]);
  return A <= 1.0 + 0x1p-40 ? 1.0 : A;
}

double fwd_sample_bound(int plane, int mode, bool pf, const double* gk) {
  if (plane == 0 || mode == M444 || !pf) return 128.0;
  const double A = taps_abs_sum(gk);
  return 128.0 * (A * A);
}

double fwd_input_error(int plane, int mode, bool pf, const double* gk, int chains) {
  const double u = 0x1p-24;
  const double dkl = fabs((double)0.299f - 0.299) + fabs((double)0.587f - 0.587) + fabs((double)0.114f - 0.114);
  if (plane == 0) return 255 * dkl + u * 255 * (0.299 + 0.886 + 1.0) + u * 128 + 1e-12;
  const double dkb = fabs((double)-0.168736f + 0.168736) + fabs((double)-0.331264f + 0.331264);
  const double dkr = fabs((double)-0.081312f + 0.081312) + fabs((double)-0.418688f + 0.418688);
  const double ec = 255 * (dkb > dkr ? dkb : dkr) + 2 * u * 128 + 1e-12;
  double e = ec;
  double e_comb = 0.0;
  double e_sum = 0.0;
  if (mode != M444 && pf) {
    const double k0 = fabs(gk[0]), k1 = fabs(gk[1]);
    const double k0f = fabs((double)(float)gk[0]), k1f = fabs((double)(float)gk[1]),
                 k2f = fabs((double)(float)gk[2]);
    const double dk = fabs((double)(float)gk[0] - gk[0]) + fabs((double)(float)gk[1] - gk[1]) +
                      fabs((double)(float)gk[2] - gk[2]);
    const double A = taps_abs_sum(gk);
    const double S = (gk[0] + gk[1]) + gk[2];
    const double S2 = S * S <= 1.0 + 0x1p-40 ? 1.0 : S * S;
    e_sum = 128 * (fabs(S * S - 1.0) + 0x1p-50 * S2);
    const double er = (k0f + k1f + k2f) * e + dk * 128 + u * 128 * (k0 + (k0 + k1) + A) + 1e-12;
    e = (k1f + 2 * k0f) * er + dk * (256 * A) + u * (256 * A + k1 * (128 * A) + 128 * (A * A)) + 1e-12;
    const double eh = combined_chain_error(gk, 128, ec);
    if (mode == M420)
      e_comb = combined_chain_error(gk, 256 * A, eh) / 4;
    else
      e_comb = ((k1f + 2 * k0f) * eh + dk * (512 * A) + u * (512 * A + k1 * (256 * A) + 256 * (A * A)) + 1e-12) / 2;
    if (mode == M420) e = e + u * ((256 + 384 + 512) * (A * A)) / 4;
// ... 127 lines not shown
```

### jpeg-dsp-studio_amd/csrc/jds_internal.hpp

```cpp
#pragma once
#include <hip/hip_runtime.h>
#include <stdint.h>

#include "jds.h"

namespace jds {

enum Mode : int { M444 = JDS_SS_444, M422 = JDS_SS_422, M420 = JDS_SS_420 };

struct Geo {
  int H, W;
  int hc, wc;
  int nby, nbx;
  int ncy, ncx;
  int nmy, nmx;
  int tiles_y, tiles_x, ty_off, tx_off;
  long long cpf;
  long long off_cb, off_cr;
  double up_sy, up_sx;
  int bs;
  int gen;
  int afx, afy;
  int inv_yoff;
};

__host__ __device__ inline int inv_tile_yoff(int mode, int H) {
  return mode == M420 && (H + 8 + 63) / 64 == (H + 63) / 64 ? 8 : 0;
}

inline void area_fast_scales(int src_h, int dst_h, int src_w, int dst_w, int* fy, int* fx) {
  const double sy = 1.0 / ((double)dst_h / (double)src_h), sx = 1.0 / ((double)dst_w / (double)src_w);
  const double ry = __builtin_rint(sy), rx = __builtin_rint(sx);
  const double eps = 2.220446049250313e-16;
  const bool fast = __builtin_fabs(sy - ry) < eps && __builtin_fabs(sx - rx) < eps;
  *fy = fast ? (int)ry : 0;
  *fx = fast ? (int)rx : 0;
}

struct AreaTap {
  int n;
  int si[4];
  int pad;
  double a[4];
};

struct GenBufs {
  const AreaTap* tabs;
  double* sub;
  double* rec;
};

__host__ __device__ inline int fix_wpi(const Geo& g) { return (int)((g.cpf / 64 + 31) / 32); }

struct Fwd16Fast {
  const void* fq16;
  const float* gk32;
  uint32_t* part;
  uint2* fixlist;
  unsigned* counters;
  int fix_all;
  int parity;
};

struct InvFix {
  unsigned* count;
  unsigned* item;
  int fix_all;
  int parity;
  int rot;
  int probe;
  uint2* list;
  int apriori;
};

struct FrameQ {
  double q16[64];
  double q[64];
  double qmax;
  double pad_;
};

template <int MODE>
struct Cfg {
  static constexpr int SY = (MODE == M420) ? 2 : 1;
  static constexpr int SX = (MODE == M444) ? 1 : 2;
  static constexpr int MH = 8 * SY, MW = 8 * SX;
  static constexpr int TH = (MODE == M444) ? 16 : 32;
  static constexpr int TW = 64;
  static constexpr int MY = TH / MH, MX = TW / MW;
  static constexpr int YBR = TH / 8, YBC = TW / 8;
  static constexpr int CBR = TH / MH, CBC = TW / MW;
  static constexpr int NYB = YBR * YBC, NCB = CBR * CBC;
  static constexpr int NB = NYB + 2 * NCB;
  static constexpr int TF = NB * 8;
  static constexpr int RY = (SY == 2) ? 1 : 0, RX = (SX == 2) ? 1 : 0;
  static constexpr int RBR = CBR + 2 * RY, RBC = CBC + 2 * RX;
  static constexpr int NRB = RBR * RBC;
  static constexpr int CWR = 8 * CBR + 2 * RY;
  static constexpr int CWC = 8 * CBC + 2 * RX;
  static constexpr int TI = 384;
};

struct KMarks {
  hipEvent_t* ev = nullptr;
  char (*name)[64] = nullptr;
  int n = 0, cap = 0;
  long long dropped = 0;
};
extern thread_local KMarks* t_kmarks;
void kmark(hipStream_t s, const char* fmt, ...) __attribute__((format(printf, 2, 3)));

__device__ inline void finalize_frame(const Geo& g, jds_frame_stats* s, int zero_bin) {
  s->total_coeffs = (uint64_t)g.cpf;
  s->block_overhead_bits = 2ull * (uint64_t)g.nby * (uint64_t)g.nbx;
  s->pixels = (uint64_t)g.H * (uint64_t)g.W;
  if (zero_bin) s->hist[25] += (uint64_t)g.cpf - s->nonzero;
}

__device__ inline void reduce_partials(jds_frame_stats* st, const uint32_t* __restrict__ part, int ptiles) {
  __shared__ unsigned long long s_sum[8][64];
  const int f = blockIdx.y, j = threadIdx.x & 63, grp = threadIdx.x >> 6;
  const int t0 = blockIdx.x * 64 + grp * 8;
  unsigned long long a = 0ull;
  if (j < 52) {
    unsigned v[8];
#pragma unroll
    for (int i = 0; i < 8; ++i) v[i] = t0 + i < ptiles ? part[((size_t)f * ptiles + t0 + i) * 52 + j] : 0u;
#pragma unroll
    for (int i = 0; i < 8; ++i) a += v[i];
  }
  s_sum[grp][j] = a;
  __syncthreads();
  if (threadIdx.x < 52) {
    unsigned long long b = 0ull;
#pragma unroll
    for (int i = 0; i < 8; ++i) b += s_sum[i][threadIdx.x];
    jds_frame_stats* s = st + f;
    unsigned long long* dst = threadIdx.x == 0 ? (unsigned long long*)&s->nonzero
                              : threadIdx.x == 1 ? (unsigned long long*)&s->magnitude_bits
                                                 : (unsigned long long*)&s->hist[threadIdx.x - 2];
    if (b) atomicAdd(dst, b);
  }
}

}
```

### jpeg-dsp-studio_amd/csrc/jds_inv.hip

```cpp
#include <hip/hip_runtime.h>
#include <stdint.h>

#include "jds_dct8.hpp"
#include "jds_device.hpp"
#include "jds_internal.hpp"
#include "jds_inv_common.hpp"
#include "jds_inv_exact.hpp"

#pragma clang fp contract(off)

namespace jds {

template <int MODE, int XTRA>
__global__ void __launch_bounds__(Inv<MODE>::NT) __attribute__((amdgpu_waves_per_eu(XTRA > 1 ? 2 : Inv<MODE>::WPE)))
k_inv2(const Geo g, const int tiles_x, const int16_t* __restrict__ coeffs, const FrameQ* __restrict__ fq,
       const uint8_t* __restrict__ rgb_in, uint8_t* __restrict__ rgb_out, jds_frame_stats* __restrict__ st,
       double* __restrict__ sse_y_part, double* __restrict__ err_y, double* __restrict__ err_rgb, const int in_div,
       const int fin) {
  __shared__ __attribute__((aligned(16))) InvShared<MODE, XTRA> sh;
  if (XTRA == 0 && fin >= 0 && blockIdx.x == 0 && threadIdx.x == 0) finalize_frame(g, st + blockIdx.y, fin);
  inv2_tile<MODE, XTRA>(sh, g, tiles_x, gridDim.x, blockIdx.y, blockIdx.x, coeffs, fq, rgb_in, rgb_out, st,
                        sse_y_part, err_y, err_rgb, in_div);
}

__global__ void __launch_bounds__(64) k_sel_recon(const int16_t* __restrict__ coeffs, const FrameQ* __restrict__ fq,
                                                  jds_selected_block* sel, int sel_blk) {
  __shared__ __attribute__((aligned(16))) double s[MS];
  const int t = threadIdx.x;
  if (t < 8) {
    int qs[64];
#pragma unroll
    for (int r = 0; r < 8; ++r) qs[r * 8 + t] = (int)fq[0].q[r * 8 + t];
    idct_col(coeffs + (long long)sel_blk * 64, qs, t, s);
  }
  __syncthreads();
  if (t < 8) {
    double c[8];
    idct_row(s, t, c);
#pragma unroll
    for (int k = 0; k < 8; ++k) sel->reconstructed[t * 8 + k] = c[k];
  }
}


template <int MODE>
static int inv_tiles_t(int H, int W, int* tx) {
  const int ty = (H + Inv<MODE>::TH - 1) / Inv<MODE>::TH;
  *tx = (W + Inv<MODE>::TW - 1) / Inv<MODE>::TW;
  return ty * *tx;
}

int inv_tiles(int mode, int H, int W) {
  int tx;
  return mode == M420 ? inv_tiles_t<M420>(H, W, &tx)
                      : (mode == M422 ? inv_tiles_t<M422>(H, W, &tx) : inv_tiles_t<M444>(H, W, &tx));
}

template <int MODE>
static void inv_rows_t(int H, int ty, int* out) {
  const int yoff = inv_tile_yoff(MODE, H);
  const InvRows<MODE> r(ty, yoff);
  out[0] = yoff;
  out[1] = (H + Inv<MODE>::TH - 1) / Inv<MODE>::TH;
  out[2] = r.y0;
  out[3] = Inv<MODE>::TH;
  out[4] = r.cby0;
  out[5] = r.ncbr;
  out[6] = r.cwy0;
  out[7] = Inv<MODE>::CWR;
}
void inv_rows(int mode, int H, int ty, int* out) {
  if (mode == M420) inv_rows_t<M420>(H, ty, out);
  else if (mode == M422) inv_rows_t<M422>(H, ty, out);
  else inv_rows_t<M444>(H, ty, out);
}
int inv_rows_need(int mode, int H, int ty, int by, int r) {
  const int yoff = inv_tile_yoff(mode, H);
  return mode == M420 ? InvRows<M420>(ty, yoff).need(by, r)
                      : (mode == M422 ? InvRows<M422>(ty, yoff).need(by, r) : InvRows<M444>(ty, yoff).need(by, r));
}

template <int MODE>
static hipError_t inv2_t(const Geo& g, int n, const int16_t* coeffs, const FrameQ* fq, const uint8_t* rgb_in,
                         uint8_t* rgb_out, jds_frame_stats* st, double* part, double* err_y, double* err_rgb,
                         hipStream_t s, int in_div, int fin) {
  int tx;
  const int tiles = inv_tiles_t<MODE>(g.H, g.W, &tx);
  const dim3 grid(tiles, n), blk(Inv<MODE>::NT);
  if (err_y)
    hipLaunchKernelGGL((k_inv2<MODE, 2>), grid, blk, 0, s, g, tx, coeffs, fq, rgb_in, rgb_out, st, part, err_y,
                       err_rgb, in_div, -1);
  else if (rgb_in)
    hipLaunchKernelGGL((k_inv2<MODE, 1>), grid, blk, 0, s, g, tx, coeffs, fq, rgb_in, rgb_out, st, part, nullptr,
                       nullptr, in_div, -1);
  else
    hipLaunchKernelGGL((k_inv2<MODE, 0>), grid, blk, 0, s, g, tx, coeffs, fq, nullptr, rgb_out, st, part, nullptr,
                       nullptr, in_div, fin);
  kmark(s, "k_inv2<%d,%d>", MODE, err_y ? 2 : rgb_in ? 1 : 0);
  return hipGetLastError();
}

hipError_t launch_inv2(int mode, const Geo& g, int n, const int16_t* coeffs, const FrameQ* fq,
                       const uint8_t* rgb_in, uint8_t* rgb_out, jds_frame_stats* st, double* part, double* err_y,
                       double* err_rgb, hipStream_t s, int in_div, int fin) {
  switch (mode) {
    case M420: return inv2_t<M420>(g, n, coeffs, fq, rgb_in, rgb_out, st, part, err_y, err_rgb, s, in_div, fin);
    case M422: return inv2_t<M422>(g, n, coeffs, fq, rgb_in, rgb_out, st, part, err_y, err_rgb, s, in_div, fin);
    default: return inv2_t<M444>(g, n, coeffs, fq, rgb_in, rgb_out, st, part, err_y, err_rgb, s, in_div, fin);
  }
}

hipError_t launch_sel_recon(const int16_t* coeffs, const FrameQ* fq, jds_selected_block* sel, int sel_blk,
                            hipStream_t s) {
  hipLaunchKernelGGL(k_sel_recon, dim3(1), dim3(64), 0, s, coeffs, fq, sel, sel_blk);
  kmark(s, "k_sel_recon");
  return hipGetLastError();
}

}
```

### jpeg-dsp-studio_amd/csrc/jds_inv_common.hpp

```cpp
#pragma once
#include <hip/hip_runtime.h>
#include <stdint.h>

#include "jds_internal.hpp"


namespace jds {

template <int MODE>
struct Inv {
  static constexpr int SY = Cfg<MODE>::SY, SX = Cfg<MODE>::SX;
  static constexpr int TH = (MODE == M420) ? 64 : 32;
  static constexpr int TW = (MODE == M444) ? 64 : 128;
  static constexpr int NT = (MODE == M444) ? 256 : 512;
  static constexpr int RY = (SY == 2) ? 1 : 0, RX = (SX == 2) ? 1 : 0;
  static constexpr int YBC = TW / 8, NYB = (TH / 8) * YBC;
  static constexpr int RB = NT / 8;
  static constexpr int CBR = TH / (8 * SY) + 2 * RY, CBC = TW / (8 * SX) + 2 * RX;
  static constexpr int NCB = CBR * CBC;
  static constexpr int CWR = TH / SY + 2 * RY, CWC = TW / SX + 2 * RX;
  static constexpr int CWS = SX == 2 ? CWC + 4 : CWC;
  static constexpr int NROW = (CBR - 2 * RY) * CBC * 8 + 2 * RY * CBC;
  static constexpr int MB = NCB > RB ? NCB : RB;
  static constexpr int WPE = (MODE == M444) ? 3 : 4;
  static_assert(NCB * 8 <= NT && NROW <= NT && NYB % RB == 0, "one round per chroma plane");
};

template <int MODE>
struct InvRows {
  int y0, cby0, ncbr, cwy0;
  __host__ __device__ __forceinline__ InvRows(int ty, int yoff) {
    using I = Inv<MODE>;
    y0 = ty * I::TH - yoff;
    cby0 = ty * (I::TH / (8 * I::SY)) - I::RY;
    ncbr = I::CBR - (yoff ? 1 : 0);
    cwy0 = y0 / I::SY - I::RY;
  }
  __host__ __device__ __forceinline__ bool need(int by, int r) const {
    return !Inv<MODE>::RY || (unsigned)(by * 8 + r - cwy0) < (unsigned)Inv<MODE>::CWR;
  }
};

constexpr int MS = 72;

__device__ __forceinline__ int tslot(int r, int c) { return r * 8 + ((((c >> 1) ^ (r & 3)) << 1) | (c & 1)); }

struct Col16 {
  int16_t q[8];
};
__device__ __forceinline__ Col16 load_col(const int16_t* __restrict__ plane, long long boff, int v, bool ok) {
  const int16_t* blk = plane + (ok ? boff : 0ll);
  Col16 c;
#pragma unroll
  for (int r = 0; r < 8; ++r) c.q[r] = blk[r * 8 + v];
  return c;
}

struct Col32 {
  int q[8];
};
__device__ __forceinline__ Col32 load_col32(const int16_t* __restrict__ plane, long long boff, int v, bool ok) {
  const int16_t* blk = plane + (ok ? boff : 0ll);
  Col32 c;
#pragma unroll
  for (int r = 0; r < 8; ++r) c.q[r] = __builtin_annotation((int)blk[r * 8 + v], "sext16");
  return c;
}

#ifdef JDS_INV6
typedef short jds_short2 __attribute__((ext_vector_type(2)));
struct Col16p {
  jds_short2 w[4];
  __device__ __forceinline__ int q(int r) const { return (int)((r & 1) ? w[r >> 1].y : w[r >> 1].x); }
};
__device__ __forceinline__ Col16p load_colp(const int16_t* __restrict__ plane, long long boff, int v, bool ok) {
  const int16_t* blk = plane + (ok ? boff : 0ll);
  Col16p c;
#pragma unroll
  for (int i = 0; i < 4; ++i) {
    c.w[i].x = blk[(2 * i) * 8 + v];
    c.w[i].y = blk[(2 * i + 1) * 8 + v];
  }
  return c;
}

__device__ __forceinline__ uint4 load_rowq(const int16_t* __restrict__ plane, long long boff, int k, bool ok) {
  return *reinterpret_cast<const uint4*>(plane + (ok ? boff : 0ll) + 8 * k);
}
__device__ __forceinline__ uint4 load_rowq_b(__amdgpu_buffer_rsrc_t r, long long boff, int k, bool ok) {
  typedef unsigned u4 __attribute__((ext_vector_type(4)));
  const u4 v = __builtin_amdgcn_raw_buffer_load_b128(r, (int)(((ok ? boff : 0ll) + 8 * k) * 2), 0, 0);
  return make_uint4(v.x, v.y, v.z, v.w);
}
__device__ __forceinline__ Col16p xpose_q16(uint4 v) {
  uint32_t w[4] = {v.x, v.y, v.z, v.w};
#pragma unroll
  for (int i = 0; i < 2; ++i) {
    const auto a = __builtin_amdgcn_permlane32_swap(w[i], w[i + 2], false, false);
    w[i] = a[0];
    w[i + 2] = a[1];
  }
#pragma unroll
  for (int i = 0; i < 4; i += 2) {
    const auto a = __builtin_amdgcn_permlane16_swap(w[i], w[i + 1], false, false);
    w[i] = a[0];
    w[i + 1] = a[1];
  }
  const bool odd = (threadIdx.x >> 3) & 1;
  const uint32_t sel = odd ? 0x03020706u : 0x05040100u;
  Col16p c;
#pragma unroll
  for (int i = 0; i < 4; ++i) {
    const uint32_t p = (uint32_t)__builtin_amdgcn_mov_dpp((int)w[i], 0x128, 0xf, 0xf, true);
    const uint32_t r = __builtin_amdgcn_perm(p, w[i], sel);
    c.w[i].x = (short)(r & 0xffffu);
    c.w[i].y = (short)(r >> 16);
  }
  return c;
}

struct W6 {
  static constexpr int TH = 64, TW = 128, NT = 512, SY = 2, SX = 2;
  static constexpr int RB = 64, NYB = 128, YBC = 16;
  static constexpr int CBR = 6, CBC = 10, NCB = 60;
  static constexpr int CWR = 34, CX = 8, CWC = 80, CWS = 82;
// ... 41 lines not shown
```

### jpeg-dsp-studio_amd/csrc/jds_inv_exact.hpp

```cpp
#pragma once
#include <hip/hip_runtime.h>
#include <stdint.h>

#include "jds_dct8.hpp"
#include "jds_device.hpp"
#include "jds_internal.hpp"
#include "jds_inv_common.hpp"

#pragma clang fp contract(off)

namespace jds {

__device__ __forceinline__ void idct_col(const int16_t* __restrict__ blk, const int* __restrict__ qi, int v,
                                         double* __restrict__ dst) {
  double c[8];
#pragma unroll
  for (int r = 0; r < 8; ++r) c[r] = (double)__mul24((int)blk[r * 8 + v], qi[r * 8 + v]);
  dct3_line(c[0], c[1], c[2], c[3], c[4], c[5], c[6], c[7]);
#pragma unroll
  for (int r = 0; r < 8; ++r) dst[tslot(r, v)] = c[r];
}

__device__ __forceinline__ void idct_col(const Col16& in, const int* __restrict__ qi, int v,
                                         double* __restrict__ dst) {
// ... 43 lines not shown
      for (int i = 0; i < 4; ++i) {
        const double e = fma(s[i], 0.25, q75[i + 1]), o = fma(s[i + 2], 0.25, q75[i + 1]);
        if (rr == 0) {
          h0[2 * i] = e;
          h0[2 * i + 1] = o;
        } else {
          C[2 * i] = vblend(h0[2 * i], e);
          C[2 * i + 1] = vblend(h0[2 * i + 1], o);
        }
      }
    }
    if constexpr (I::SY == 1) {
#pragma unroll
      for (int k = 0; k < 8; ++k) C[k] = h0[k];
    }
#pragma unroll
    for (int side = 0; side < 2; ++side) {
      const int kl = side == 0 ? (x0 == 0 ? 0 : -1) : (g.W - 1 - x0 < 8 ? g.W - 1 - x0 : -1);
      if (kl >= 0) {
        const int e = (side == 0 ? 0 : g.wc - 1) - cwx0;
        const double v0 = cw[wq * I::CWS + e];
        double v = v0;
        if constexpr (I::SY == 2) v = vblend(v0, cw[wt * I::CWS + e]);
#pragma unroll
        for (int k = 0; k < 8; ++k) C[k] = k == kl ? v : C[k];
      }
    }
  }
}

__device__ __forceinline__ void colour8_exact_cb(const double (&Yv)[8], const double (&Cb)[8], double (&Gt)[8],
                                                 uint32_t (&pk)[6]) {
#pragma unroll
  for (int w = 0; w < 6; ++w) pk[w] = 0u;
#pragma unroll
  for (int k = 0; k < 8; ++k) {
    const double B = Yv[k] + 1.772 * (Cb[k] - 128.0);
    Gt[k] = Yv[k] - 0.344136 * (Cb[k] - 128.0);
    const int b = 3 * k + 2;
    pk[b >> 2] |= (uint32_t)clampi((int)B, 0, 255) << (8 * (b & 3));
  }
}
__device__ __forceinline__ void colour8_exact_cr(const double (&Yv)[8], const double (&Gt)[8], const double (&Cr)[8],
                                                 uint32_t (&pk)[6]) {
#pragma unroll
  for (int k = 0; k < 8; ++k) {
    const double R = Yv[k] + 1.402 * (Cr[k] - 128.0);
    const double G = Gt[k] - 0.714136 * (Cr[k] - 128.0);
    const int b = 3 * k;
    pk[b >> 2] |= (uint32_t)clampi((int)R, 0, 255) << (8 * (b & 3));
    pk[(b + 1) >> 2] |= (uint32_t)clampi((int)G, 0, 255) << (8 * ((b + 1) & 3));
  }
}

template <int MODE, int XTRA>
struct InvShared {
  double mid[Inv<MODE>::MB * MS];
  double cw[2][Inv<MODE>::CWR * Inv<MODE>::CWS];
  int q[64];
  double red[Inv<MODE>::NT / 64];
  unsigned long long sse;
  int redo;
};

template <int MODE, int XTRA, bool REDO = false>
__device__ __forceinline__ void inv2_tile(InvShared<MODE, XTRA>& sh, const Geo& g, const int tiles_x, const int ntiles,
                                          const int frame, const int tile, const int16_t* __restrict__ coeffs,
                                          const FrameQ* __restrict__ fq, const uint8_t* __restrict__ rgb_in,
                                          uint8_t* __restrict__ rgb_out, jds_frame_stats* __restrict__ st,
                                          double* __restrict__ sse_y_part, double* __restrict__ err_y,
                                          double* __restrict__ err_rgb, const int in_div,
                                          const unsigned redo_mask = ~0u, unsigned long long* rsse = nullptr,
                                          double* rssy = nullptr) {
  using I = Inv<MODE>;
  static_assert(I::NYB / I::RB <= 2, "at most two luma rounds per lane");
  double* s_mid = sh.mid;
  double (*s_cw)[I::CWR * I::CWS] = sh.cw;
  int* s_q = sh.q;
  double* s_red = sh.red;
  unsigned long long& s_sse = sh.sse;

  const int tid = threadIdx.x, lv = tid & 7, lb = tid >> 3;
  const int ty = tile / tiles_x, tx = tile - ty * tiles_x;
  const InvRows<MODE> rows(ty, g.inv_yoff);
  const int Y0 = rows.y0, X0 = tx * I::TW;
  const int16_t* cf = coeffs + (size_t)frame * g.cpf;
  if (tid < 64) s_q[tid] = (int)fq[frame].q[tid];
  if (XTRA && tid == 0) s_sse = 0ull;
  __syncthreads();

  const int cby0 = rows.cby0, cbx0 = X0 / (8 * I::SX) - I::RX;
  const int cwy0 = rows.cwy0, cwx0 = X0 / I::SX - I::RX;
  auto luma_blk = [&](int r, int& by, int& bx) {
    const int blk = r * I::RB + lb;
    const int bi = blk / I::YBC, bj = blk - bi * I::YBC;
    by = Y0 / 8 + bi;
    bx = X0 / 8 + bj;
    return by >= 0 && by < g.nby && bx < g.nbx;
  };
  Col16 lq;
  {
    int by, bx;
    const bool ok = luma_blk(0, by, bx);
    lq = load_col(cf, ((long long)by * g.nbx + bx) * 64, lv, ok);
  }
  if (lb < rows.ncbr * I::CBC) {
    const int i = lb / I::CBC, j = lb - i * I::CBC;
    const int by = cby0 + i, bx = cbx0 + j;
    const bool bvalid = by >= 0 && bx >= 0 && by < g.ncy && bx < g.ncx;
    const bool need = rows.need(by, lv);
    const long long boff = ((long long)by * g.ncx + bx) * 64;
    Col16 cq = load_col(cf + g.off_cb, boff, lv, bvalid);
#pragma unroll 1
    for (int p = 0; p < 2; ++p) {
      const Col16 cur = cq;
      if (p == 0) cq = load_col(cf + g.off_cr, boff, lv, bvalid);
      if (bvalid) {
        idct_col(cur, s_q, lv, s_mid + lb * MS);
        if (need) {
          double c[8];
          idct_row(s_mid + lb * MS, lv, c);
          double* w = &s_cw[p][(by * 8 + lv - cwy0) * I::CWS];
          const int wc0 = bx * 8 - cwx0;
#pragma unroll
          for (int k = 0; k < 8; ++k)
            if ((unsigned)(wc0 + k) < (unsigned)I::CWC) w[wc0 + k] = c[k];
        }
      }
    }
  }
  __syncthreads();
  const bool want_in = XTRA > 0;
  unsigned long long sse = 0ull;
  double ssy = 0.0;
  const uint8_t* in_f = want_in ? rgb_in + (size_t)(frame / in_div) * g.H * g.W * 3 : nullptr;
  uint8_t* out_f = rgb_out + (size_t)frame * g.H * g.W * 3;
#pragma unroll 1
  for (int r = 0; r < I::NYB / I::RB; ++r) {
    int by, bx;
    const bool bvalid = luma_blk(r, by, bx) && (!REDO || ((redo_mask >> r) & 1u));
    unsigned long long r_sse = 0ull;
    double r_ssy = 0.0;
    const Col16 cur = lq;
    if (r + 1 < I::NYB / I::RB) {
      int by1, bx1;
      const bool ok1 = luma_blk(r + 1, by1, bx1);
      lq = load_col(cf, ((long long)by1 * g.nbx + bx1) * 64, lv, ok1);
    }
    if (bvalid) idct_col(cur, s_q, lv, s_mid + lb * MS);
    const int y = by * 8 + lv, x0 = bx * 8;
    if (bvalid && y < g.H && x0 < g.W) {
      double Yv[8];
      idct_row(s_mid + lb * MS, lv, Yv);
      int wq, wt = 0;
      if constexpr (I::SY == 2) {
        float fy = (float)((y + 0.5) * g.up_sy - 0.5);
        const int sy = (int)floorf(fy);
        fy -= (float)sy;
        const int r0 = clampi(clampi(sy, 0, g.hc - 1) - cwy0, 0, I::CWR - 1);
        const int r1 = clampi(clampi(sy + 1, 0, g.hc - 1) - cwy0, 0, I::CWR - 1);
        const bool q0 = fy == 0.75f;
        wq = q0 ? r0 : r1;
        wt = q0 ? r1 : r0;
      } else {
        wq = y - cwy0;
      }
      const int nx = g.W - x0 < 8 ? g.W - x0 : 8;
      uint8_t* o = out_f + ((size_t)y * g.W + x0) * 3;
      const bool wide = nx == 8 && ((((uintptr_t)o) & 7u) == 0);
      uint32_t in[6] = {0u, 0u, 0u, 0u, 0u, 0u};
      if constexpr (XTRA > 0) {
        const uint8_t* src = in_f + ((size_t)y * g.W + x0) * 3;
        if (wide) {
          const uint2* s2 = reinterpret_cast<const uint2*>(src);
          const uint2 a = s2[0], b = s2[1], c = s2[2];
          in[0] = a.x; in[1] = a.y; in[2] = b.x; in[3] = b.y; in[4] = c.x; in[5] = c.y;
        } else {
#pragma unroll
          for (int k = 0; k < 24; ++k)
            if (k < 3 * nx) in[k >> 2] |= (uint32_t)src[k] << (8 * (k & 3));
        }
      }
      auto byte_of = [](const uint32_t (&w)[6], int b) { return (int)((w[b >> 2] >> (8 * (b & 3))) & 255u); };
      uint32_t pk[6] = {0u, 0u, 0u, 0u, 0u, 0u};
      double eB[8];
      {
        double C[8], Gt[8];
        chroma8<MODE>(s_cw[0], g, x0, cwx0, wq, wt, C);
#pragma unroll
        for (int k = 0; k < 8; ++k) {
          const double B = Yv[k] + 1.772 * (C[k] - 128.0);
          Gt[k] = Yv[k] - 0.344136 * (C[k] - 128.0);
// ... 79 lines not shown
```

### jpeg-dsp-studio_amd/csrc/jds_inv_fast.hip

```cpp
#include <hip/hip_runtime.h>
#include <stdint.h>
#include <string.h>

#include <algorithm>
#include <cmath>
#include <vector>

#include "jds_device.hpp"
#include "jds_internal.hpp"
#include "jds_inv_common.hpp"
#include "jds_inv_exact.hpp"
#include "jds_inv16_exact.hpp"

#pragma clang fp contract(fast)

namespace jds {

constexpr double K_LIN = 8.762155e-13 * 1.01;
constexpr double K_CONST = 1.024801e-12 * 1.01;
constexpr double K_LIN16 = 3.345910e-12 * 1.01;
constexpr double K_CONST16 = 1.024801e-12 * 1.01;

constexpr double AP_DMAX = 1152.0;
constexpr uint32_t ceil_u32(double x) { return (uint32_t)x + ((double)(uint32_t)x < x ? 1u : 0u); }
// ... 135 lines not shown
      C[2 * i + 1] = fhsum(vb[i + 2], vb[i + 1]);
    }
  }
}

constexpr double MAGIC = 0x1.8p+20;
constexpr uint32_t MAGIC_HI = 0x41380000u;

__device__ __forceinline__ uint32_t byte_cert_y(double y, uint32_t& lo_min, uint32_t& lo_max) {
  const uint32_t lo = (uint32_t)__double2loint(y), hi = (uint32_t)__double2hiint(y);
  lo_min = lo_min < lo ? lo_min : lo;
  lo_max = lo_max > lo ? lo_max : lo;
  const uint32_t c = hi < MAGIC_HI ? MAGIC_HI : hi;
  return c > MAGIC_HI + 255u ? MAGIC_HI + 255u : c;
}

template <bool AP = false>
__device__ __forceinline__ uint32_t cert_hi(double y, uint32_t& lo_min, uint32_t& lo_max) {
  const uint32_t lo = (uint32_t)__double2loint(y), hi = (uint32_t)__double2hiint(y);
  lo_min = lo_min < lo ? lo_min : lo;
  if constexpr (!AP) lo_max = lo_max > lo ? lo_max : lo;
  return hi;
}
template <bool AP>
constexpr double Y_OFF = MAGIC + 128.0 + (AP ? (double)AP_S * 0x1p-32 : 0.0);
__device__ __forceinline__ uint32_t sat_pk_u8_i16(uint32_t x) {
  uint32_t r;
  asm("v_sat_pk_u8_i16 %0, %1" : "=v"(r) : "v"(x));
  return r;
}
__device__ __forceinline__ uint32_t pack4s(uint32_t a, uint32_t b, uint32_t c, uint32_t d) {
  const uint32_t ab = sat_pk_u8_i16(__builtin_amdgcn_perm(b, a, 0x05040100u));
  const uint32_t cd = sat_pk_u8_i16(__builtin_amdgcn_perm(d, c, 0x05040100u));
  return ab | (cd << 16);
}

__device__ __forceinline__ uint32_t pack4(uint32_t a, uint32_t b, uint32_t c, uint32_t d) {
  const uint32_t ab = __builtin_amdgcn_perm(b, a, 0x0c0c0400u);
  const uint32_t cd = __builtin_amdgcn_perm(d, c, 0x04000c0cu);
  return ab | cd;
}

template <int SH>
__device__ __forceinline__ void cert_row_step(uint32_t& mn, uint32_t& mx, uint32_t& qm) {
  const uint32_t a = (uint32_t)__builtin_amdgcn_update_dpp((int)0xffffffff, (int)mn, 0x110 + SH, 0xf, 0xf, false);
  const uint32_t b = (uint32_t)__builtin_amdgcn_update_dpp(0, (int)mx, 0x110 + SH, 0xf, 0xf, false);
  const uint32_t c = (uint32_t)__builtin_amdgcn_update_dpp(0, (int)qm, 0x110 + SH, 0xf, 0xf, false);
  mn = mn < a ? mn : a;
  mx = mx > b ? mx : b;
  qm = qm > c ? qm : c;
}
__device__ __forceinline__ void cert_to_lds(uint32_t mn, uint32_t mx, uint32_t qm, uint32_t* s_cert) {
  cert_row_step<1>(mn, mx, qm);
  cert_row_step<2>(mn, mx, qm);
  cert_row_step<4>(mn, mx, qm);
  cert_row_step<8>(mn, mx, qm);
  if ((threadIdx.x & 15) == 15) {
    atomicMin(&s_cert[0], mn);
    atomicMax(&s_cert[1], mx);
    atomicMax(&s_cert[2], qm);
  }
}

template <int MODE, int XTRA, bool AP>
__device__ __forceinline__ bool inv_fast_tile(InvShared<MODE, XTRA>& sh, const Geo& g, const int tiles_x,
                                              const int frame, const int tile, const int16_t* __restrict__ coeffs,
                                              const FrameQ* __restrict__ fq, const uint8_t* __restrict__ rgb_in,
                                              uint8_t* __restrict__ rgb_out, jds_frame_stats* __restrict__ st,
                                              double* __restrict__ sse_y_part, unsigned* __restrict__ fixcount,
                                              unsigned* __restrict__ next_count, unsigned* __restrict__ cnt_now,
                                              const int in_div, const int fix_all) {
  using I = Inv<MODE>;
  constexpr int USH_ = USH<I::SY, I::SX>;
  double* s_mid = sh.mid;
  double (*s_cw)[I::CWR * I::CWS] = sh.cw;
  __shared__ __attribute__((aligned(16))) double s_qs[QS_WORDS];
  __shared__ double s_qmax;
  __shared__ double s_red[I::NT / 64], s_dq[I::NT / 64];
  __shared__ uint32_t s_lmin[I::NT / 64], s_lmax[I::NT / 64];
  __shared__ uint32_t s_cert[3];
  __shared__ unsigned long long s_sse;
  const int tid = threadIdx.x, lv = tid & 7, lb = tid >> 3;
  const int ty = tile / tiles_x, tx = tile - ty * tiles_x;
  const InvRows<MODE> rows(ty, g.inv_yoff);
  const int Y0 = rows.y0, X0 = tx * I::TW;
  const int16_t* cf = coeffs + (size_t)frame * g.cpf;
  int qhi = 0, qlo = 0;

  const int cby0 = rows.cby0, cbx0 = X0 / (8 * I::SX) - I::RX;
  const int cwy0 = rows.cwy0, cwx0 = X0 / I::SX - I::RX;
  auto luma_blk = [&](int r, int& by, int& bx) {
    const int blk = r * I::RB + lb;
    const int bi = blk / I::YBC, bj = blk - bi * I::YBC;
    by = Y0 / 8 + bi;
    bx = X0 / 8 + bj;
    return by >= 0 && by < g.nby && bx < g.nbx;
  };
  auto table_setup = [&]() {
    if (tid < 64) {
      const double q = fq[frame].q[tid];
      s_qs[qs_index(tid >> 3, tid & 7)] = q * c_aan[tid >> 3] * c_aan[tid & 7] * 0.125;
      if (!AP && tid == 0) {
        s_cert[0] = 0xffffffffu;
        s_cert[1] = 0u;
        s_cert[2] = 0u;
      }
    }
    if (XTRA && tid == 0) s_sse = 0ull;
    __syncthreads();
  };
  auto luma_load = [&](int r) {
    int by, bx;
    const bool ok = luma_blk(r, by, bx);
    return load_col32(cf, ((long long)by * g.nbx + bx) * 64, lv, ok);
  };
  Col32 lq = luma_load(0);
  auto chroma_task = [&](const int p, const int by, const int bx, const Col32& cur) __attribute__((always_inline)) {
    const bool need = rows.need(by, lv);
    fast_col<AP>(cur, s_qs, lv, s_mid + lb * MS, qhi, qlo);
    if (need) {
      double c[8];
      fast_row<-128>(s_mid + lb * MS, lv, c);
      double* w = &s_cw[p][(by * 8 + lv - cwy0) * I::CWS];
      const int wc0 = bx * 8 - cwx0;
      if constexpr (I::RX == 0) {
#pragma unroll
        for (int k = 0; k < 8; ++k) w[wc0 + k] = c[k];
      } else {
        static_assert((I::TW / I::SX) % 8 == 0, "block columns at 8 j - 7");
        const int j = bx - cbx0;
        const bool ring = j == 0 || j == I::CBC - 1;
        double* const base = ring ? s_mid + lb * MS + lv * 8 : w + wc0;
#pragma unroll
        for (int k = 0; k < 8; ++k) base[k] = c[k];
        if (ring) *(j == 0 ? w : w + (I::CWC - 1)) = j == 0 ? c[7] : c[0];
      }
      if constexpr (I::SX == 2) {
        if (bx == 0 && wc0 >= 1) w[wc0 - 1] = c[0];
        const int ke = g.wc - 1 - bx * 8;
        if ((unsigned)ke < 8u) {
          const double e = (ke == 0 ? c[0] : ke == 1 ? c[1] : ke == 2 ? c[2] : ke == 3 ? c[3]
                            : ke == 4 ? c[4] : ke == 5 ? c[5] : ke == 6 ? c[6] : c[7]);
          for (int col = wc0 + ke + 1; col < I::CWC; ++col) w[col] = e;
        }
      }
    }
  };
  constexpr bool MIXP = 1 && MODE == M422 && 2 * I::NCB > I::RB && 2 * I::NCB <= 2 * I::RB;
  if constexpr (MIXP) {
    constexpr int NTASK = 2 * I::NCB;
    auto tinfo = [&](int tt, int& pp, int& ii, int& by, int& bx, bool& ok) -> long long {
      pp = tt >= I::NCB ? 1 : 0;
      const int b = tt - pp * I::NCB;
      ii = b / I::CBC;
      const int jj = b - ii * I::CBC;
      by = cby0 + ii;
      bx = cbx0 + jj;
      ok = tt < NTASK && by >= 0 && bx >= 0 && by < g.ncy && bx < g.ncx;
      return ((long long)by * g.ncx + bx) * 64;
    };
    static_assert(NTASK <= 2 * I::RB, "two tasks per lane group at the most");
    int p0, p1, ii, by0, bx0, by1, bx1;
    bool ok0, ok1;
    const long long off0 = tinfo(lb, p0, ii, by0, bx0, ok0);
    const Col32 cq0 = load_col32(cf + (p0 ? g.off_cr : g.off_cb), off0, lv, ok0);
    table_setup();
    if (!AP && tid == 0) s_qmax = fq[frame].qmax;
    const bool two = lb + I::RB < NTASK;
    const long long off1 = tinfo(lb + I::RB, p1, ii, by1, bx1, ok1);
    Col32 cq1;
    if (two) cq1 = load_col32(cf + (p1 ? g.off_cr : g.off_cb), off1, lv, ok1);
    if (ok0) chroma_task(p0, by0, bx0, cq0);
    if (two && ok1) chroma_task(p1, by1, bx1, cq1);
  } else {
    const bool ctask = lb < rows.ncbr * I::CBC;
    const int ci = lb / I::CBC, cj = lb - ci * I::CBC;
    const int cby = cby0 + ci, cbx = cbx0 + cj;
    const bool cvalid = ctask && cby >= 0 && cbx >= 0 && cby < g.ncy && cbx < g.ncx;
    const long long cboff = ((long long)cby * g.ncx + cbx) * 64;
    const Col32 cqb = load_col32(cf + g.off_cb, cboff, lv, cvalid);
    table_setup();
    if (!AP && tid == 0) s_qmax = fq[frame].qmax;
    if (ctask) {
      const Col32 cqr = load_col32(cf + g.off_cr, cboff, lv, cvalid);
      if (cvalid) {
        chroma_task(0, cby, cbx, cqb);
        chroma_task(1, cby, cbx, cqr);
      }
    }
  }
  __syncthreads();

  uint32_t lo_min = 0xffffffffu, lo_max = 0u;
  unsigned long long sse = 0ull;
  double ssy = 0.0;
  const uint8_t* in_f = XTRA ? rgb_in + (size_t)(frame / in_div) * g.H * g.W * 3 : nullptr;
  uint8_t* out_f = rgb_out + (size_t)frame * g.H * g.W * 3;
  auto luma_round = [&](const int r, const Col32& cur) __attribute__((always_inline)) {
    int by, bx;
    const bool bvalid = luma_blk(r, by, bx);
    unsigned long long r_sse = 0ull;
    double r_ssy = 0.0;
    if (bvalid) fast_col<AP>(cur, s_qs, lv, s_mid + lb * MS, qhi, qlo);
    const int y = by * 8 + lv, x0 = bx * 8;
    if (bvalid && y < g.H && x0 < g.W) {
      double Yv[8];
      fast_row<-128>(s_mid + lb * MS, lv, Yv);
      int wq, wt = 0;
      if constexpr (I::SY == 2) {
        const int m = y >> 1;
        const int rq = (y & 1) ? m + 1 : m - 1;
        wq = clampi(clampi(rq, 0, g.hc - 1) - cwy0, 0, I::CWR - 1);
        wt = clampi(clampi(m, 0, g.hc - 1) - cwy0, 0, I::CWR - 1);
      } else {
        wq = y - cwy0;
      }
      const int nx = g.W - x0 < 8 ? g.W - x0 : 8;
      uint8_t* o = out_f + ((size_t)y * g.W + x0) * 3;
      const bool wide = nx == 8 && ((((uintptr_t)o) & 7u) == 0);
      uint32_t in[6] = {0u, 0u, 0u, 0u, 0u, 0u};
      if constexpr (XTRA > 0) {
        const uint8_t* src = in_f + ((size_t)y * g.W + x0) * 3;
        if (wide) {
          const uint2* s2 = reinterpret_cast<const uint2*>(src);
          const uint2 a = s2[0], b2 = s2[1], c = s2[2];
          in[0] = a.x; in[1] = a.y; in[2] = b2.x; in[3] = b2.y; in[4] = c.x; in[5] = c.y;
        } else {
#pragma unroll
          for (int k = 0; k < 24; ++k)
            if (k < 3 * nx) in[k >> 2] |= (uint32_t)src[k] << (8 * (k & 3));
        }
      }
      uint32_t pk[6];
      uint32_t r_min = 0xffffffffu, r_max = 0u;
      {
        uint32_t cb[24];
        double C[8], Gt[8];
        chroma8_fast<MODE>(s_cw[0], x0, cwx0, wq, wt, C);
#pragma unroll
        for (int k = 0; k < 8; ++k) {
          Yv[k] = Yv[k] + Y_OFF<AP>;
          const double B = col_b<MadDev, USH_>(Yv[k], C[k]);
          Gt[k] = col_gt<MadDev, USH_>(Yv[k], C[k]);
          cb[3 * k + 2] = cert_hi<AP>(B, r_min, r_max);
        }
        chroma8_fast<MODE>(s_cw[1], x0, cwx0, wq, wt, C);
#pragma unroll
        for (int k = 0; k < 8; ++k) {
          const double R = col_r<MadDev, USH_>(Yv[k], C[k]);
          const double G = col_g<MadDev, USH_>(Gt[k], C[k]);
          cb[3 * k] = cert_hi<AP>(R, r_min, r_max);
          cb[3 * k + 1] = cert_hi<AP>(G, r_min, r_max);
        }
#pragma unroll
        for (int w = 0; w < 6; ++w) pk[w] = pack4s(cb[4 * w], cb[4 * w + 1], cb[4 * w + 2], cb[4 * w + 3]);
      }
      lo_min = lo_min < r_min ? lo_min : r_min;
      if constexpr (!AP) lo_max = lo_max > r_max ? lo_max : r_max;
      if (wide) {
        uint2* o2 = reinterpret_cast<uint2*>(o);
        o2[0] = make_uint2(pk[0], pk[1]);
        o2[1] = make_uint2(pk[2], pk[3]);
        o2[2] = make_uint2(pk[4], pk[5]);
      } else {
#pragma unroll
        for (int b = 0; b < 24; ++b)
          if (b < 3 * nx) o[b] = (uint8_t)(pk[b >> 2] >> (8 * (b & 3)));
      }
      if constexpr (XTRA > 0) {
        auto byte_of = [](const uint32_t (&w)[6], int b) { return (int)((w[b >> 2] >> (8 * (b & 3))) & 255u); };
#pragma unroll
        for (int k = 0; k < 8; ++k) {
          if (k < nx) {
            const int b = 3 * k;
            const int o0 = byte_of(in, b), o1 = byte_of(in, b + 1), o2 = byte_of(in, b + 2);
            const int ur = byte_of(pk, b), ug = byte_of(pk, b + 1), ub = byte_of(pk, b + 2);
            const int d0 = o0 - ur, d1 = o1 - ug, d2 = o2 - ub;
            r_sse += (unsigned long long)(d0 * d0 + d1 * d1 + d2 * d2);
            r_ssy = r_ssy + luma_sse_e6(d0, d1, d2);
          }
        }
      }
    }
    if constexpr (XTRA > 0) {
      sse += r_sse;
      ssy = ssy + r_ssy;
    }
  };
  constexpr int NR = I::NYB / I::RB;
#pragma unroll 1
  for (int r = 0; r < NR; r += 2) {
    Col32 nq;
    if (r + 1 < NR) nq = luma_load(r + 1);
    luma_round(r, lq);
    if (r + 1 < NR) {
      if (r + 2 < NR) lq = luma_load(r + 2);
      luma_round(r + 1, nq);
    }
  }

  if constexpr (AP) {
    if (__ballot(lo_min < 2u * AP_S || fix_all) != 0ull && (tid & 63) == 0) sh.redo = 1;
  } else {
    int qm = max(qhi, -qlo);
    cert_to_lds(lo_min, lo_max, (uint32_t)qm, s_cert);
  }
  if constexpr (XTRA > 0) {
    unsigned long long s = sse;
#pragma unroll
    for (int o = 32; o > 0; o >>= 1) s += __shfl_xor(s, o, 64);
    if ((tid & 63) == 0) atomicAdd(&s_sse, s);
    double d = ssy;
#pragma unroll
    for (int o = 32; o > 0; o >>= 1) d = d + __shfl_xor(d, o, 64);
    if ((tid & 63) == 0) s_red[tid >> 6] = d;
  }
  __syncthreads();
  if (tid == 0) {
    if constexpr (!AP) {
      const uint32_t mn = s_cert[0], mx = s_cert[1];
      const double q = (double)s_cert[2];
      const double E = K_LIN * (q * s_qmax) + K_CONST + 0x1p-31;
      const double T = ceil(E * 0x1p+32) + 1.0;
      const bool uncertain = (double)mn <= T || (double)mx >= 0x1p+32 - 1.0 - T;
      sh.redo = uncertain || fix_all;
    }
    if (sh.redo) {
      atomicAdd(fixcount, 1u);
      atomicAdd(cnt_now + frame, 1u);
    } else if constexpr (XTRA > 0) {
      double a = 0.0;
      for (int i = 0; i < I::NT / 64; ++i) a = a + s_red[i];
      sse_y_part[(size_t)frame * gridDim.x + tile] = a;
      atomicAdd((unsigned long long*)&st[frame].sse_rgb, s_sse);
    }
    if (frame == 0 && tile == 0) *next_count = 0u;
  }
  if constexpr (!AP) __syncthreads();
  return sh.redo != 0;
}

template <int MODE, int XTRA, bool AP>
__global__ void __launch_bounds__(Inv<MODE>::NT) __attribute__((amdgpu_waves_per_eu(Inv<MODE>::WPE)))
k_inv_fast(const Geo g, const int tiles_x, const int16_t* __restrict__ coeffs, const FrameQ* __restrict__ fq,
           const uint8_t* __restrict__ rgb_in, uint8_t* __restrict__ rgb_out, jds_frame_stats* __restrict__ st,
           double* __restrict__ sse_y_part, unsigned* __restrict__ fixcount, unsigned* __restrict__ next_count,
           unsigned* __restrict__ item_cnt, const int rot, const int probe, const int in_div, const int fix_all,
           const int fin) {
  __shared__ __attribute__((aligned(16))) InvShared<MODE, XTRA> sh;
#ifdef JDS_PROBE_LDS_PAD
  __shared__ unsigned s_pad[JDS_PROBE_LDS_PAD];
  if (threadIdx.x == 0) s_pad[blockIdx.x % JDS_PROBE_LDS_PAD] = 0u;
#endif
  const int tid = threadIdx.x;
  const int frame = blockIdx.y, tile = blockIdx.x;
  if (fin >= 0 && tile == 0 && tid == 0) finalize_frame(g, st + frame, fin);
  const unsigned n_items = gridDim.y, ntile = gridDim.x;
  unsigned* cnt_prev = item_cnt + ((rot + 2) % 3) * n_items;
  unsigned* cnt_now = item_cnt + rot * n_items;
  const unsigned prev = cnt_prev[frame];
  if (tile == 0 && tid == 0) item_cnt[((rot + 1) % 3) * n_items + frame] = 0u;
  const bool item_exact = !probe && !fix_all && prev * 8u > ntile;
  bool redo = false;
  if (item_exact) {
    if (tile == 0 && tid == 0) {
      cnt_now[frame] = prev;
      atomicAdd(fixcount, ntile);
      if (frame == 0) *next_count = 0u;
    }
  } else {
    sh.redo = 0;
    redo = inv_fast_tile<MODE, XTRA, AP>(sh, g, tiles_x, frame, tile, coeffs, fq, rgb_in, rgb_out, st, sse_y_part,
                                         fixcount, next_count, cnt_now, in_div, fix_all);
  }
#ifndef JDS_PROBE_NOFALLBACK
  if (item_exact || redo)
    inv2_tile<MODE, XTRA>(sh, g, tiles_x, ntile, frame, tile, coeffs, fq, rgb_in, rgb_out, st, sse_y_part, nullptr,
                          nullptr, in_div);
#endif
}

#ifdef JDS_INV6
typedef double dv2 __attribute__((ext_vector_type(2)));
typedef __attribute__((address_space(3))) volatile dv2 lds_dv2;

__device__ __forceinline__ void chroma8_fast_w6(const double* __restrict__ cw, int c0, int wq, int wt,
                                                double (&C)[8]) {
  double vb[6];
#pragma unroll
  for (int j = 0; j < 6; ++j) vb[j] = fvsum(cw[wq * W6::CWS + c0 + j], cw[wt * W6::CWS + c0 + j]);
#pragma unroll
  for (int i = 0; i < 4; ++i) {
    C[2 * i] = fhsum(vb[i], vb[i + 1]);
    C[2 * i + 1] = fhsum(vb[i + 2], vb[i + 1]);
  }
}

__device__ __forceinline__ void deq_col(const Col16p& in, const double* __restrict__ qs, int k, bool track,
                                        double (&c)[8], int& qhi, int& qlo) {
  double t[8];
  int off = k * QS_STRIDE;
  asm volatile("" : "+v"(off));
#pragma unroll
  for (int p = 0; p < 4; ++p) {
    const double2 d = *reinterpret_cast<const double2*>(qs + off + 2 * p);
    t[2 * p] = d.x;
    t[2 * p + 1] = d.y;
  }
#pragma unroll
  for (int r = 0; r < 8; ++r) {
    const int q = in.q(r);
    qhi = track ? max(qhi, q) : qhi;
    qlo = track ? min(qlo, q) : qlo;
    c[r] = (double)q * t[r];
  }
}

#ifndef JDS_K6_WPE
#define JDS_K6_WPE 6
#endif
__global__ void __launch_bounds__(W6::NT) __attribute__((amdgpu_waves_per_eu(JDS_K6_WPE)))
k_inv_fast6(const Geo g, const int tiles_x, const int16_t* __restrict__ coeffs, const FrameQ* __restrict__ fq,
            uint8_t* __restrict__ rgb_out, jds_frame_stats* __restrict__ st, unsigned* __restrict__ fixcount,
            unsigned* __restrict__ next_count, unsigned* __restrict__ item_cnt, uint2* __restrict__ fixlist,
            const int rot, const int probe, const int fix_all, const int fin) {
  __shared__ __attribute__((aligned(16))) double s_cw[2][W6::CWR * W6::CWS];
  __shared__ __attribute__((aligned(16))) double s_qs[QS_WORDS];
  __shared__ uint32_t s_cert[3];
  __shared__ double s_qmax;
  const int tid = threadIdx.x;
  const int frame = blockIdx.y, tile = blockIdx.x;
  if (fin >= 0 && tile == 0 && tid == 0) finalize_frame(g, st + frame, fin);
  const unsigned n_items = gridDim.y, ntile = gridDim.x;
  unsigned* cnt_prev = item_cnt + ((rot + 2) % 3) * n_items;
  unsigned* cnt_now = item_cnt + rot * n_items;
  const unsigned prev = cnt_prev[frame];
  if (tid == 0) {
    if (tile == 0) item_cnt[((rot + 1) % 3) * n_items + frame] = 0u;
    if (frame == 0 && tile == 0) *next_count = 0u;
  }
#ifndef JDS_K6_PROBE
#define JDS_K6_PROBE 0
#endif
  const bool item_exact = !JDS_K6_PROBE && !probe && !fix_all && prev * 8u > ntile;
  if (item_exact) {
    if (tid == 0) {
      if (tile == 0) cnt_now[frame] = prev;
      fixlist[atomicAdd(fixcount, 1u)] = make_uint2((unsigned)frame, (unsigned)tile);
    }
    return;
  }

  const int k = (tid >> 3) & 7, lb = ((tid >> 6) << 3) | (tid & 7);
  const int ty = tile / tiles_x, tx = tile - ty * tiles_x;
  const int Y0 = ty * W6::TH, X0 = tx * W6::TW;
  const __amdgpu_buffer_rsrc_t cf = __builtin_amdgcn_make_buffer_rsrc(
      (void*)(coeffs + (size_t)frame * g.cpf), 0, (int)(g.cpf * 2), 0x00020000);
  const int cwy0 = Y0 / 2 - 1;
  auto luma_blk = [&](int r, int& by, int& bx) {
    const int blk = r * W6::RB + lb;
    by = Y0 / 8 + (blk >> 4);
    bx = X0 / 8 + (blk & 15);
// ... 565 lines not shown
          ch[3 * k + 1] = byte_cert_m(col_g<MadDev, USH_>(Gt[8 * h + k], C[k]), ok, lo_min, lo_max);
          ch[3 * k + 2] = (bpk[2 * h + (k >> 2)] >> (8 * (k & 3))) & 255u;
        }
        uint32_t pk[6];
#pragma unroll
        for (int w = 0; w < 6; ++w) pk[w] = pack4(ch[4 * w], ch[4 * w + 1], ch[4 * w + 2], ch[4 * w + 3]);
        uint8_t* o = out_f + ((size_t)y * g.W + x0) * 3;
        if (nx == 8 && ((((uintptr_t)o) & 7u) == 0)) {
          uint2* o2 = reinterpret_cast<uint2*>(o);
          o2[0] = make_uint2(pk[0], pk[1]);
          o2[1] = make_uint2(pk[2], pk[3]);
          o2[2] = make_uint2(pk[4], pk[5]);
        } else {
#pragma unroll
          for (int b = 0; b < 24; ++b)
            if (b < 3 * nx) o[b] = (uint8_t)(pk[b >> 2] >> (8 * (b & 3)));
        }
      }
    }
  }

  int qm = max(qhi, -qlo);
  cert_to_lds(lo_min, lo_max, (uint32_t)qm, s_cert);
  __syncthreads();
  if (tid == 0) {
    const uint32_t mn = s_cert[0], mx = s_cert[1];
    const double q = (double)s_cert[2];
    const double E = K_LIN16 * (q * s_qmax) + K_CONST16 + 0x1p-31;
    const double T = ceil(E * 0x1p+32) + 1.0;
    const bool uncertain = (double)mn <= T || (double)mx >= 0x1p+32 - 1.0 - T;
    s_redo = uncertain || fix_all;
    if (s_redo) {
      atomicAdd(fixcount, 1u);
      atomicAdd(cnt_now + frame, 1u);
    }
  }
  __syncthreads();
#ifndef JDS_PROBE_NOFALLBACK
  if (s_redo)
    inv16s_tile<MODE, 0>(s_b, s_cw, fq[frame].q, nullptr, nullptr, g, tiles_x, (int)gridDim.x, frame, tile, coeffs,
                         nullptr, rgb_out, nullptr, nullptr, nullptr, nullptr);
#endif
}

hipError_t launch_inv16_fast(int mode, const Geo& g, int n, const int16_t* coeffs, const FrameQ* fq,
                             uint8_t* rgb_out, const InvFix& fx, hipStream_t s, jds_frame_stats* st, int fin) {
  auto go = [&](auto kern, int TH, int TW) {
    const int tx = (g.W + TW - 1) / TW, ty = (g.H + TH - 1) / TH;
    hipLaunchKernelGGL(kern, dim3(ty * tx, n), dim3(256), 0, s, g, tx, coeffs, fq, rgb_out, fx.count + fx.parity,
                       fx.count + (fx.parity ^ 1), fx.item, fx.rot, fx.fix_all, st, fin);
    kmark(s, "k_inv16_fast<%d>", mode);
    return hipGetLastError();
  };
  if (mode == M420) return go(k_inv16_fast<M420>, Inv16<M420>::TH, Inv16<M420>::TW);
  if (mode == M422) return go(k_inv16_fast<M422>, Inv16<M422>::TH, Inv16<M422>::TW);
  return hipErrorInvalidValue;
}


constexpr int INV6_FIX_GRID = 256;

template <int MODE>
static hipError_t inv_fast_t(const Geo& g, int n, const int16_t* coeffs, const FrameQ* fq, const uint8_t* rgb_in,
                             uint8_t* rgb_out, jds_frame_stats* st, double* part, const InvFix& fx, hipStream_t s,
                             int in_div, int fin) {
  const int ty = (g.H + Inv<MODE>::TH - 1) / Inv<MODE>::TH, tx = (g.W + Inv<MODE>::TW - 1) / Inv<MODE>::TW;
  const dim3 grid(ty * tx, n), blk(Inv<MODE>::NT);
  unsigned* cnt = fx.count + fx.parity;
  unsigned* nxt = fx.count + (fx.parity ^ 1);
#ifdef JDS_INV6
  if (MODE == M420 && fx.list) {
    hipLaunchKernelGGL(k_inv_fast6, grid, dim3(W6::NT), 0, s, g, tx, coeffs, fq, rgb_out, st, cnt, nxt, fx.item,
                       fx.list, fx.rot, fx.probe, fx.fix_all, fin);
    kmark(s, "k_inv_fast6");
    hipError_t e = hipGetLastError();
    if (e != hipSuccess) return e;
    const int nfix = std::min(ty * tx * n, INV6_FIX_GRID);
    hipLaunchKernelGGL(k_inv6_fix, dim3(nfix), dim3(Inv<M420>::NT), 0, s, g, tx, coeffs, fq, rgb_out, cnt, fx.list);
    kmark(s, "k_inv6_fix");
    return hipGetLastError();
  }
#endif
  auto go = [&](auto kern, const uint8_t* rin, int xtra, int f) {
    hipLaunchKernelGGL(kern, grid, blk, 0, s, g, tx, coeffs, fq, rin, rgb_out, st, part, cnt, nxt, fx.item, fx.rot,
                       fx.probe, in_div, fx.fix_all, f);
    kmark(s, "k_inv_fast<%d,%d>", MODE, xtra);
    return hipGetLastError();
  };
  if (rgb_in != nullptr)
    return fx.apriori ? go(k_inv_fast<MODE, 1, true>, rgb_in, 1, -1) : go(k_inv_fast<MODE, 1, false>, rgb_in, 1, -1);
  return fx.apriori ? go(k_inv_fast<MODE, 0, true>, nullptr, 0, fin) : go(k_inv_fast<MODE, 0, false>, nullptr, 0, fin);
}

hipError_t launch_inv_fast(int mode, const Geo& g, int n, const int16_t* coeffs, const FrameQ* fq,
                           const uint8_t* rgb_in, uint8_t* rgb_out, jds_frame_stats* st, double* part,
                           const InvFix& fx, hipStream_t s, int in_div, int fin) {
  switch (mode) {
    case M420: return inv_fast_t<M420>(g, n, coeffs, fq, rgb_in, rgb_out, st, part, fx, s, in_div, fin);
    case M422: return inv_fast_t<M422>(g, n, coeffs, fq, rgb_in, rgb_out, st, part, fx, s, in_div, fin);
    default: {
      (void)rgb_in;
      (void)part;
      (void)in_div;
      const long long nblk = (long long)g.nby * g.nbx;
      const dim3 grid((unsigned)((nblk + 8 * I444_WAVES - 1) / (8 * I444_WAVES)), n), blk(64 * I444_WAVES);
      if (fx.apriori)
        hipLaunchKernelGGL(k_inv_fast444<true>, grid, blk, 0, s, g, coeffs, fq, rgb_out, st, fx.count + fx.parity,
                           fx.count + (fx.parity ^ 1), fx.item, fx.rot, fx.fix_all, fin);
      else
        hipLaunchKernelGGL(k_inv_fast444<false>, grid, blk, 0, s, g, coeffs, fq, rgb_out, st, fx.count + fx.parity,
                           fx.count + (fx.parity ^ 1), fx.item, fx.rot, fx.fix_all, fin);
      kmark(s, "k_inv_fast444");
      return hipGetLastError();
    }
  }
}

template <class M, int BS, bool AP = false>
static void inv_fast_host_t(int mode, const int16_t* cf, const double* Q, int H, int W, double* vout,
                            uint8_t* bout) {
  const int sy = mode == M420 ? 2 : 1, sx = mode == M444 ? 1 : 2;
  double qs[64];
  for (int i = 0; i < 64; ++i) qs[i] = Q[i] * h_aan[i >> 3] * h_aan[i & 7] * 0.125;
  auto deq = [&](int q, int u, int v) {
    if constexpr (BS == 8) return (double)q * qs[u * 8 + v];
    return ((double)(q * (int)Q[(u >> 1) * 8 + (v >> 1)]) * s16_of(h_aan, u)) * s16_of(h_aan, v);
  };
  auto line = [](double(&c)[BS]) {
    if constexpr (BS == 8)
      aan8<M>(c);
    else
      fidct16<M>(c);
  };
  std::vector<double> pl[3];
  int ph[3], pw[3], st[3];
  size_t off = 0;
  for (int p = 0; p < 3; ++p) {
    ph[p] = p ? H / sy : H;
    pw[p] = p ? W / sx : W;
    const int nby = (ph[p] + BS - 1) / BS, nbx = (pw[p] + BS - 1) / BS;
    st[p] = nbx * BS;
    pl[p].assign((size_t)nby * BS * st[p], 0.0);
    for (int by = 0; by < nby; ++by)
      for (int bx = 0; bx < nbx; ++bx) {
        const int16_t* b = cf + off + ((size_t)by * nbx + bx) * BS * BS;
        double mid[BS][BS];
        for (int v = 0; v < BS; ++v) {
          double c[BS];
          for (int r = 0; r < BS; ++r) c[r] = deq(b[r * BS + v], r, v);
          line(c);
          for (int r = 0; r < BS; ++r) mid[r][v] = c[r];
        }
        for (int u = 0; u < BS; ++u) {
          double c[BS];
          for (int k = 0; k < BS; ++k) c[k] = mid[u][k];
          line(c);
          for (int k = 0; k < BS; ++k)
            pl[p][(size_t)(by * BS + u) * st[p] + bx * BS + k] = fmin(fmax(c[k], -128.0), 127.0);
        }
      }
    off += (size_t)nby * nbx * BS * BS;
  }
  auto S = [&](int p, int r, int c) {
    r = r < 0 ? 0 : (r > ph[p] - 1 ? ph[p] - 1 : r);
    c = c < 0 ? 0 : (c > pw[p] - 1 ? pw[p] - 1 : c);
    return pl[p][(size_t)r * st[p] + c];
  };
  for (int y = 0; y < H; ++y)
    for (int x = 0; x < W; ++x) {
      double C[3];
// ... 90 lines not shown
```

### jpeg-dsp-studio_amd/jds/_abi.py

```python
from __future__ import annotations

import ctypes as C
import importlib.util
import os
import threading

import numpy as np

_HERE = os.path.dirname(os.path.abspath(__file__))
LIB_PATH = os.environ.get('JDS_LIB_PATH') or os.path.join(_HERE, 'libjds.so')

JDS_OK, JDS_EINVAL, JDS_ENOTSUP, JDS_EHIP, JDS_ENOMEM = 0, -1, -2, -3, -4
SS_444, SS_422, SS_420 = 0, 1, 2
MODE_CODES = {'4:4:4': SS_444, '4:2:2': SS_422, '4:2:0': SS_420}
SS_GRAY = 3
JPEG_MODE_CODES = dict(MODE_CODES, gray=SS_GRAY)
RENDER_CODES = {'reference': 0, 'libjpeg': 1}
RUN_SSE, RUN_FWD, RUN_INV, RUN_EXACT, RUN_EXACT_INV, RUN_INV_FIXALL, RUN_FWD_FIXALL, RUN_INV_FAST = 1, 2, 4, 8, 16, 32, 64, 128


SCALE_DENOMS = (1, 2, 4, 8)


def scale_denom_arg(scale_denom, render=None) -> int:
# ... 231 lines not shown
    'jds_jpeg_batch_to_rgb': (C.c_int, [_P, _P, _P, C.c_int32, _P, C.c_int64, C.c_int32, _P, C.POINTER(JpegBatchItem),
                                        C.POINTER(C.c_uint32)]),
    'jds_selftest_jpeg_batch': (C.c_int, [_P, _P, C.c_int32, C.c_int32, _P, C.c_int64, _P, C.POINTER(JpegBatchItem)]),
    'jds_jpeg_render_dev': (C.c_int, [_P, C.POINTER(JpegInfo), _P, _P, _P, C.c_int32]),
    'jds_jpeg_to_rgb_render': (C.c_int, [_P, _P, C.c_int64, _P, C.c_int64, C.c_int32, _P, C.POINTER(JpegInfo),
                                         C.c_int32]),
    'jds_selftest_jpeg_render': (C.c_int, [C.POINTER(JpegInfo), _P, _P, C.c_int32]),
    'jds_jpeg_batch_to_rgb_render': (C.c_int, [_P, _P, _P, C.c_int32, _P, C.c_int64, C.c_int32, _P,
                                               C.POINTER(JpegBatchItem), C.POINTER(C.c_uint32), C.c_int32]),
    'jds_selftest_jpeg_batch_render': (C.c_int, [_P, _P, C.c_int32, C.c_int32, _P, C.c_int64, _P,
                                                 C.POINTER(JpegBatchItem), C.c_int32]),
    'jds_jpeg_scaled_size': (C.c_int, [C.c_int64, C.c_int64, C.c_int32, C.POINTER(C.c_int64), C.POINTER(C.c_int64)]),
    'jds_jpeg_render_scaled_dev': (C.c_int, [_P, C.POINTER(JpegInfo), _P, _P, _P, C.c_int32, C.c_int32]),
    'jds_jpeg_to_rgb_scaled': (C.c_int, [_P, _P, C.c_int64, _P, C.c_int64, C.c_int32, _P, C.POINTER(JpegInfo),
                                         C.c_int32, C.c_int32]),
    'jds_jpeg_batch_layout_scaled': (C.c_int, [_P, _P, C.c_int32, C.POINTER(JpegBatchItem), C.POINTER(C.c_int64),
                                               C.POINTER(C.c_int64), _P, C.POINTER(JpegScaledItem)]),
    'jds_jpeg_batch_to_rgb_scaled': (C.c_int, [_P, _P, _P, C.c_int32, _P, C.c_int64, C.c_int32, _P,
                                               C.POINTER(JpegBatchItem), C.POINTER(C.c_uint32), C.c_int32, _P,
                                               C.POINTER(JpegScaledItem)]),
    'jds_selftest_jpeg_render_scaled': (C.c_int, [C.POINTER(JpegInfo), _P, _P, C.c_int32, C.c_int32]),
    'jds_selftest_jpeg_batch_render_scaled': (C.c_int, [_P, _P, C.c_int32, C.c_int32, _P, C.c_int64, _P,
                                                        C.POINTER(JpegBatchItem), C.c_int32, _P,
                                                        C.POINTER(JpegScaledItem)]),
    'jds_encode_jpeg': (C.c_int, [_P, C.POINTER(JpegInfo), _P, C.c_int32, _P, C.c_int64, _P, C.c_int64,
                                  C.POINTER(C.c_int64)]),
    'jds_jpeg_transcode': (C.c_int, [_P, _P, C.c_int64, C.c_int32, _P, C.c_int64, C.POINTER(C.c_int64),
                                     C.POINTER(JpegInfo)]),
    'jds_jpeg_batch_transcode': (C.c_int, [_P, _P, _P, C.c_int32, C.c_int32, _P, C.c_int64, C.c_int32,
                                           C.POINTER(JpegTranscodeItem), C.POINTER(C.c_int64)]),
    'jds_selftest_jpeg_transcode': (C.c_int, [_P, C.c_int64, C.c_int32, _P, C.c_int64, C.POINTER(C.c_int64)]),
    'jds_pjpeg_parse': (C.c_int, [_P, C.c_int64, C.POINTER(PjpegInfo)]),
    'jds_pjpeg_decode': (C.c_int, [_P, _P, C.c_int64, _P, C.c_int64, C.POINTER(PjpegInfo)]),
    'jds_pjpeg_decode_dev': (C.c_int, [_P, _P, C.c_int64, _P, C.c_int64, C.POINTER(PjpegInfo)]),
    'jds_pjpeg_scan_times': (C.c_int, [_P, _P, C.c_int64, C.POINTER(C.c_int64)]),
    'jds_selftest_pjpegdec': (C.c_int, [_P, C.c_int64, _P, C.c_int64, C.POINTER(PjpegInfo)]),
    'jds_pjpeg_batch_layout': (C.c_int, [_P, _P, C.c_int32, C.POINTER(JpegBatchItem), C.POINTER(C.c_int64),
                                         C.POINTER(C.c_int64), _P, C.POINTER(JpegScaledItem)]),
    'jds_pjpeg_batch_to_rgb': (C.c_int, [_P, _P, _P, C.c_int32, _P, C.c_int64, C.c_int32, C.c_int32, _P,
                                         C.POINTER(JpegBatchItem), C.POINTER(JpegScaledItem), _P]),
    'jds_pjpeg_to_rgb': (C.c_int, [_P, _P, C.c_int64, _P, C.c_int64, C.c_int32, C.c_int32, C.c_int32, _P,
                                   C.POINTER(PjpegInfo)]),
    'jds_pjpeg_batch_transcode': (C.c_int, [_P, _P, _P, C.c_int32, C.c_int32, _P, C.c_int64, C.c_int32,
                                            C.POINTER(JpegTranscodeItem), C.POINTER(C.c_int64)]),
    'jds_pjpeg_transcode': (C.c_int, [_P, _P, C.c_int64, C.c_int32, _P, C.c_int64, C.POINTER(C.c_int64),
                                      C.POINTER(PjpegInfo)]),
    'jds_selftest_jpeg_encode': (C.c_int, [C.POINTER(JpegInfo), _P, C.c_int32, _P, C.c_int64, _P, C.c_int64,
                                           C.POINTER(C.c_int64)]),
    'jds_selftest_jpeg_hist_dev': (C.c_int, [_P, C.POINTER(JpegInfo), _P, _P]),
    'jds_jpeg_transform_info': (C.c_int, [_P, C.c_int64, C.c_int32, C.POINTER(C.c_int32), C.POINTER(C.c_int64),
                                          C.POINTER(C.c_int64)]),
    'jds_jpeg_transform': (C.c_int, [_P, _P, C.c_int64, C.c_int32, C.c_int32, _P, C.c_int64, C.POINTER(C.c_int64),
                                     C.POINTER(JpegInfo)]),
    'jds_jpeg_batch_transform': (C.c_int, [_P, _P, _P, C.c_int32, _P, C.c_int32, _P, C.c_int64, C.c_int32,
                                           C.POINTER(JpegTranscodeItem), C.POINTER(C.c_int64)]),
    'jds_selftest_jpeg_transform': (C.c_int, [_P, C.c_int64, C.c_int32, C.c_int32, _P, C.c_int64,
                                              C.POINTER(C.c_int64)]),
    'jds_selftest_coef_transform_dev': (C.c_int, [_P, C.POINTER(JpegInfo), C.c_int32, _P, _P]),
    'jds_jpeg_quality_info': (C.c_int, [C.c_int32, C.c_int32, C.c_int64, C.c_int64, C.POINTER(JpegInfo)]),
    'jds_jpeg_forward_dev': (C.c_int, [_P, C.POINTER(JpegInfo), _P, _P, _P]),
    'jds_rgb_to_jpeg': (C.c_int, [_P, _P, C.c_int32, C.c_int64, C.c_int64, C.c_int32, C.c_int32, C.c_int32, _P,
                                  C.c_int64, C.POINTER(C.c_int64)]),
    'jds_rgb_batch_to_jpeg': (C.c_int, [_P, _P, C.c_int32, C.POINTER(RgbItem), C.c_int32, C.c_int32, _P, C.c_int64,
                                        C.c_int32, C.POINTER(JpegTranscodeItem), C.POINTER(C.c_int64)]),
    'jds_selftest_jpeg_forward': (C.c_int, [C.POINTER(JpegInfo), _P, _P]),
    'jds_resize_info': (C.c_int, [C.POINTER(C.c_int32), C.POINTER(C.c_int32), C.POINTER(C.c_int32)]),
    'jds_rgb_resize': (C.c_int, [_P, _P, C.c_int32, C.c_int64, C.c_int64, _P, C.c_int64, C.c_int64, C.c_int32, _P,
                                 C.c_int32]),
    'jds_rgb_batch_resize': (C.c_int, [_P, _P, C.POINTER(ResizeItem), C.c_int32, C.c_int64, C.c_int64, C.c_int32, _P,
                                       _P]),
    'jds_jpeg_batch_to_tensor': (C.c_int, [_P, _P, _P, C.c_int32, C.c_int64, C.c_int64, C.c_int32, _P, _P, _P,
                                           C.c_int64, C.c_int32, C.POINTER(JpegBatchItem), C.POINTER(JpegScaledItem),
                                           C.POINTER(C.c_uint32)]),
    'jds_selftest_resize': (C.c_int, [_P, C.c_int64, C.c_int64, _P, C.c_int64, C.c_int64, C.c_int32, _P,
                                      C.POINTER(C.c_int64)]),
    'jds_selftest_resize_coeffs': (C.c_int, [C.c_int32, C.c_float, C.c_float, C.c_int32, C.c_int32,
                                             C.POINTER(C.c_int32), _P, _P, C.c_int64]),
    'jds_selftest_jpeg_fwd_quant': (C.c_int, [C.c_int32, C.c_int32, _P, C.POINTER(C.c_int32)]),
    'jds_selftest_jpeg_window': (C.c_int, [C.c_int32, C.c_int32, C.c_int32, C.c_int32, C.c_int32, _P]),
    'jds_selftest_dct8x8': (C.c_int, [_P, _P, C.c_int64, C.c_int32]),
    'jds_selftest_dct16x16': (C.c_int, [_P, _P, C.c_int64, C.c_int32]),
    'jds_selftest_area_tab': (C.c_int, [C.c_int32, C.c_int32, _P, _P, _P]),
    'jds_selftest_inv_rows': (C.c_int, [C.c_int32, C.c_int64, C.c_int32, _P, _P]),
    'jds_selftest_inv_fast': (C.c_int, [C.c_int32, _P, _P, C.c_int64, C.c_int64, C.c_int32, _P, _P]),
    'jds_selftest_inv_fast16': (C.c_int, [C.c_int32, _P, _P, C.c_int64, C.c_int64, C.c_int32, _P, _P]),
    'jds_selftest_inv_cert': (C.c_int, [_P, C.c_int64, _P, _P, _P]),
    'jds_selftest_fwd32': (C.c_int, [C.c_int32, C.c_int32, _P, _P, C.c_int64, C.c_int64, C.c_int32, C.c_int32, _P,
                                     _P]),
    'jds_selftest_fwd16': (C.c_int, [C.c_int32, C.c_int32, _P, _P, C.c_int64, C.c_int64, C.c_int32, C.c_int32, _P,
                                     _P]),
}
_OPTIONAL_SIGS: dict = {}

_lib = None
_lock = threading.Lock()


def _preload_torch_hip():
    spec = importlib.util.find_spec('torch')
    if spec is None or not spec.submodule_search_locations:
        return None
    cand = os.path.join(list(spec.submodule_search_locations)[0], 'lib', 'libamdhip64.so')
    if os.path.exists(cand):
        return C.CDLL(cand, mode=C.RTLD_GLOBAL)
    return None


def lib():
    global _lib
    if _lib is not None:
        return _lib
    with _lock:
        if _lib is not None:
            return _lib
        if not os.path.exists(LIB_PATH):
            raise ImportError(f'{LIB_PATH} is missing: build it with `python -c "import __graft_entry__ as g; '
                              f'g.build()"` (hipcc --offload-arch=gfx950)')
        _preload_torch_hip()
        h = C.CDLL(LIB_PATH, mode=C.RTLD_GLOBAL)
        for name, (res, args) in _SIGS.items():
            f = getattr(h, name)
            f.restype, f.argtypes = res, args
        for name, (res, args) in _OPTIONAL_SIGS.items():
            f = getattr(h, name, None)
            if f is not None:
                f.restype, f.argtypes = res, args
        if h.jds_abi_version() != ABI_VERSION:
            raise ImportError('libjds.so ABI version mismatch')
        _lib = h
        return h


def check(rc: int):
    if rc == JDS_OK:
        return
    msg = lib().jds_last_error().decode(errors='replace')
    if rc in (JDS_EINVAL, JDS_ENOTSUP):
        raise ValueError(msg)
    raise JDSError(f'libjds error {rc}: {msg}')


def ptr(a: np.ndarray) -> int:
    return a.ctypes.data


def device_count() -> int:
    n = C.c_int(0)
    rc = lib().jds_device_count(C.byref(n))
    return n.value if rc == JDS_OK else 0


class Context:

    def __init__(self, device: int = 0):
        h = C.c_void_p()
        check(lib().jds_ctx_create(device, C.byref(h)))
        self.handle = h
        self.device = device

    def set_ssim_scratch(self, nbytes: int = 0):
        check(lib().jds_ctx_set_ssim_scratch(self.handle, int(nbytes)))

    def profile(self, enable: bool = True):
        check(lib().jds_ctx_profile(self.handle, 1 if enable else 0))

    def profile_read(self):
# ... 133 lines not shown
```

Before: 244,000 Mpixels/s.

## Overlap forward fix kernel with inverse via side stream and per-tile dirty map

The forward fix-up kernel now runs on a side stream forked by events, and the forward kernels mark the inverse tiles touched by flagged blocks in a per-frame tile bitmap. The inverse runs in two passes. The first handles unflagged tiles concurrently with the fix kernel, and the second waits on a join event and handles only the marked tiles, then clears their bits. This hides the serial fix-kernel latency behind inverse work, at the cost of atomics in the forward kernels, an extra launch, and more complex ordering of the counter resets.

```diff
diff --git a/include/jds.h b/include/jds.h
--- a/include/jds.h
+++ b/include/jds.h
@@ -456,6 +456,9 @@
 
 int jds_selftest_inv_rows(int32_t subsampling, int64_t H, int32_t ty, int32_t* out, uint8_t* need);
 
+int jds_selftest_inv_tilemap(int32_t subsampling, int64_t H, int64_t W, int32_t tile, int32_t plane, int32_t by,
+                             int32_t bx, int32_t* out, int32_t* n_out);
+
 int jds_selftest_area_tab(int32_t src, int32_t dst, int32_t* n, int32_t* si, double* a);
 
 #ifdef __cplusplus
diff --git a/jpeg-dsp-studio_amd/csrc/jds_abi.hip b/jpeg-dsp-studio_amd/csrc/jds_abi.hip
--- a/jpeg-dsp-studio_amd/csrc/jds_abi.hip
+++ b/jpeg-dsp-studio_amd/csrc/jds_abi.hip
@@ -109,6 +109,9 @@
   DevBuf invfix;
   DevBuf invlist;
   unsigned inv_runs = 0;
+  DevBuf invtile;
+  hipStream_t fix_side = nullptr;
+  hipEvent_t fix_fork = nullptr, fix_join = nullptr;
   bool last_inv_fast = false;
   bool inv_fast_ok = true;
   bool inv_fast_any = true;
@@ -537,6 +540,23 @@
       return fail(e == hipErrorOutOfMemory ? JDS_ENOMEM : JDS_EHIP, "plan upload: %s", hipGetErrorString(e));
     }
     free(h32);
+    if (n_q == 1 && mode != JDS_SS_444) {
+      const size_t words = 4 * (size_t)n * (size_t)inv_tiles(mode, (int)H, (int)W);
+      auto event = [](hipEvent_t* ev) {
+        hipError_t r = hipEventCreateWithFlags(ev, hipEventDisableTiming | hipEventDisableSystemFence);
+        if (r != hipSuccess) {
+          (void)hipGetLastError();
+          r = hipEventCreateWithFlags(ev, hipEventDisableTiming);
+        }
+        return r;
+      };
+      if ((e = p->invtile.ensure(words)) != hipSuccess || (e = hipMemset(p->invtile.p, 0, words)) != hipSuccess ||
+          (e = hipStreamCreateWithFlags(&p->fix_side, hipStreamNonBlocking)) != hipSuccess ||
+          (e = event(&p->fix_fork)) != hipSuccess || (e = event(&p->fix_join)) != hipSuccess) {
+        jds_plan_destroy(p);
+        return fail(e == hipErrorOutOfMemory ? JDS_ENOMEM : JDS_EHIP, "plan side stream: %s", hipGetErrorString(e));
+      }
+    }
     if (p->inv_fast_any && !p->inv_fast_ok) {
       std::vector<unsigned> seed(3 * (size_t)n, 0u);
       const unsigned nt = (unsigned)inv_tiles(mode, (int)H, (int)W);
@@ -631,6 +651,17 @@
     }
     return JDS_OK;
   }
+  InvFix fx = p->inv_fix();
+  fx.fix_all = (flags & JDS_RUN_INV_FIXALL) ? 1 : 0;
+  fx.apriori = phases == 3 && p->apriori_ok;
+  const bool exact_inv = exact || (flags & JDS_RUN_EXACT_INV) != 0 || (!p->inv_fast_any && !(flags & JDS_RUN_INV_FAST));
+  const bool overlap = phases == 3 && !exact_inv && !fx.fix_all && p->invfix.p && p->invtile.p &&
+                       !(JDS_INV6_LIST && p->mode == JDS_SS_420);
+  const FixSide side{(unsigned*)p->invtile.p, p->fix_side, p->fix_fork, p->fix_join};
+  if (overlap) {
+    fx.tilew = side.tilew;
+    fx.join = side.join;
+  }
   if (phases & 1) {
     if (exact) HIP_TRY(hipMemsetAsync(stats, 0, sizeof(jds_frame_stats) * p->n, s));
     if (exact)
@@ -643,13 +674,9 @@
                               (uint32_t*)p->fixbits.p, (uint2*)p->fixlist.p, (unsigned*)p->counters.p,
                               (float*)p->dct32.p, s,
                               phases == 1,
-                              (int)(p->fwd8_runs & 1u)));
+                              (int)(p->fwd8_runs & 1u), overlap ? &side : nullptr));
     if (!exact && p->nq == 1) p->last_fwd8_bank = (int)(p->fwd8_runs++ & 1u);
   }
-  InvFix fx = p->inv_fix();
-  fx.fix_all = (flags & JDS_RUN_INV_FIXALL) ? 1 : 0;
-  fx.apriori = phases == 3 && p->apriori_ok;
-  const bool exact_inv = exact || (flags & JDS_RUN_EXACT_INV) != 0 || (!p->inv_fast_any && !(flags & JDS_RUN_INV_FAST));
   if (phases & 2)
     HIP_TRY(launch_codec(p->mode, p->pf, p->g, p->n, rgb, rgb_out, coeffs, (const FrameQ*)p->fq.p,
                          (const double*)p->gk.p, stats, (double*)p->part.p, (flags & JDS_RUN_SSE) != 0, nullptr,
@@ -757,6 +784,13 @@
   if (!p) return;
   (void)hipSetDevice(p->ctx->device);
   (void)hipStreamSynchronize(p->ctx->stream);
+  if (p->fix_side) {
+    (void)hipStreamSynchronize(p->fix_side);
+    (void)hipStreamDestroy(p->fix_side);
+  }
+  if (p->fix_fork) (void)hipEventDestroy(p->fix_fork);
+  if (p->fix_join) (void)hipEventDestroy(p->fix_join);
+  p->invtile.release();
   p->fq.release();
   p->gk.release();
   p->part.release();
@@ -1662,6 +1696,25 @@
   return JDS_OK;
 }
 
+int jds_selftest_inv_tilemap(int32_t subsampling, int64_t H, int64_t W, int32_t tile, int32_t plane, int32_t by,
+                             int32_t bx, int32_t* out, int32_t* n_out) {
+  if (!out || !n_out || (subsampling != JDS_SS_420 && subsampling != JDS_SS_422) || plane < 0 || plane > 2)
+    return fail(JDS_EINVAL, "bad argument");
+  jds_params prm;
+  memset(&prm, 0, sizeof prm);
+  prm.block_size = 8;
+  prm.subsampling = subsampling;
+  Geo g;
+  if (int rc = make_geo(&prm, H, W, &g, nullptr, nullptr)) return rc;
+  if (g.gen) return fail(JDS_ENOTSUP, "the tiled inverse does not take odd 4:2:x sizes");
+  if (tile < 0 && (by < 0 || bx < 0 || by >= (plane ? g.ncy : g.nby) || bx >= (plane ? g.ncx : g.nbx)))
+    return fail(JDS_EINVAL, "no such block");
+  const int n = inv_tilemap(subsampling, g, tile, plane, by, bx, out);
+  if (n < 0) return fail(JDS_EINVAL, "no such tile");
+  *n_out = n;
+  return JDS_OK;
+}
+
 int jds_selftest_dct16x16(const double* in, double* out, int64_t n, int32_t inverse) {
   if (!in || !out || n < 0) return fail(JDS_EINVAL, "bad argument");
   for (int64_t b = 0; b < n; ++b) {
diff --git a/jpeg-dsp-studio_amd/csrc/jds_abi.hpp b/jpeg-dsp-studio_amd/csrc/jds_abi.hpp
--- a/jpeg-dsp-studio_amd/csrc/jds_abi.hpp
+++ b/jpeg-dsp-studio_amd/csrc/jds_abi.hpp
@@ -23,6 +23,7 @@
                         int sel_blk, hipStream_t s, hipEvent_t* ev, int phases, int in_div, const GenBufs* gb,
                         const InvFix* fx = nullptr);
 int inv_tiles(int mode, int H, int W);
+int inv_tilemap(int mode, const Geo& g, int tile, int plane, int by, int bx, int* out);
 void inv_rows(int mode, int H, int ty, int* out);
 int inv_rows_need(int mode, int H, int ty, int by, int r);
 int area_tab_build(int src, int dst, AreaTap* tab);
@@ -50,7 +51,7 @@
                            const FrameQ* fq, const void* fq32, const double* gk, const float* gk32,
                            jds_frame_stats* st, uint32_t* part, uint32_t* fixbits, uint2* fixlist, unsigned* fixcount,
                            float* dct32,
-                           hipStream_t s, bool finish, int par);
+                           hipStream_t s, bool finish, int par, const FixSide* fs = nullptr);
 int quant_mq_tiles(const Geo& g);
 int inv16_tiles(int mode, int H, int W);
 constexpr int MAXQ_SHARED = 8;
diff --git a/jpeg-dsp-studio_amd/csrc/jds_fast.hip b/jpeg-dsp-studio_amd/csrc/jds_fast.hip
--- a/jpeg-dsp-studio_amd/csrc/jds_fast.hip
+++ b/jpeg-dsp-studio_amd/csrc/jds_fast.hip
@@ -6,6 +6,7 @@
 #include "jds_dct8.hpp"
 #include "jds_device.hpp"
 #include "jds_internal.hpp"
+#include "jds_inv_common.hpp"
 #include "jds_fwd_common.hpp"
 
 #pragma clang fp contract(off)
@@ -129,8 +130,11 @@
                     (uint32_t)(uint16_t)q[6] | ((uint32_t)(uint16_t)q[7] << 16));
 }
 
+template <int MODE = M444>
 __device__ __forceinline__ void flag_block_list(const LaneStats& ls, bool valid, int line, int item, int plane,
-                                                int bidx, uint2* fixlist, unsigned* fixcount, long long cap) {
+                                                int bidx, uint2* fixlist, unsigned* fixcount, long long cap,
+                                                unsigned* tilew = nullptr, const Geo* g = nullptr, int by = 0,
+                                                int bx = 0) {
   const unsigned long long fm = __ballot(valid && ls.nflag != 0u);
   if (!fm) return;
   const int lane = threadIdx.x & 63;
@@ -143,6 +147,12 @@
     const unsigned slot = base + (unsigned)__popcll(lm & ((1ull << lane) - 1ull));
     if (slot < (unsigned long long)cap)
       fixlist[(size_t)item * cap + slot] = make_uint2((unsigned)item, ((unsigned)plane << 24) | (unsigned)bidx);
+    if (tilew != nullptr) {
+      int nty, ntx;
+      inv_tile_grid<MODE>(g->H, g->W, nty, ntx);
+      unsigned* const w = tilew + (size_t)item * (nty * ntx);
+      inv_block_tiles<MODE>(g->H, g->W, g->inv_yoff, plane, by, bx, [&](int tile) { atomicOr(w + tile, 1u); });
+    }
   }
 }
 
@@ -177,7 +187,7 @@
         const FastQ* __restrict__ fq, const float* __restrict__ gk32, uint32_t* __restrict__ part,
         uint2* __restrict__ fixlist, unsigned* __restrict__ fixcount, const int border, const int4 rect,
         float* __restrict__ dct32,
-        jds_frame_stats* __restrict__ stz, const int nzq) {
+        jds_frame_stats* __restrict__ stz, const int nzq, unsigned* __restrict__ tilew = nullptr) {
   using C = Cfg<MODE>;
   constexpr int WR = C::TH + 2, WC = C::TW + 2, WN = WR * WC;
   constexpr bool CPLANE = (MODE != M444) && PF;
@@ -400,7 +410,7 @@
   if (valid)
     *reinterpret_cast<uint4*>(coeffs + (long long)frame * g.cpf + (plane == 0 ? 0 : (plane == 1 ? g.off_cb : g.off_cr)) +
                               (long long)bidx * 64 + u * 8) = pack_q(q);
-  flag_block_list(ls, valid, line, frame, plane, bidx, fixlist, fixcount, g.cpf / 64);
+  flag_block_list<MODE>(ls, valid, line, frame, plane, bidx, fixlist, fixcount, g.cpf / 64, tilew, &g, gy, gx);
   stats_flush(ls, valid, part + ((size_t)frame * g.tiles_y * g.tiles_x + ty * g.tiles_x + tx) * PSLOT);
 }
 
@@ -410,7 +420,7 @@
          const FastQ* __restrict__ fq, const float* __restrict__ gk32, uint32_t* __restrict__ part,
          uint2* __restrict__ fixlist, unsigned* __restrict__ fixcount, const int4 rect,
          float* __restrict__ dct32,
-         jds_frame_stats* __restrict__ stz, const int nzq) {
+         jds_frame_stats* __restrict__ stz, const int nzq, unsigned* __restrict__ tilew = nullptr) {
   using C = Cfg<MODE>;
   constexpr int TH = C::TH, TW = C::TW, WR = TH + 2, SEG = TW / 8;
   static_assert(16 % SEG == 0, "staging segment groups tile the 16-lane DPP rows");
@@ -650,7 +660,7 @@
     column(P + by_t * 8 * TW + bx_t * 8, TW, plane);
   }
   if constexpr (!MQ) {
-    flag_block_list(ls, valid, line, frame, plane, bidx, fixlist, fixcount, g.cpf / 64);
+    flag_block_list<MODE>(ls, valid, line, frame, plane, bidx, fixlist, fixcount, g.cpf / 64, tilew, &g, gy, gx);
     stats_flush(ls, valid, part + ((size_t)frame * g.tiles_y * g.tiles_x + ty * g.tiles_x + tx) * PSLOT);
   }
 }
@@ -1227,8 +1237,9 @@
 static hipError_t fast_fwd_t(const Geo& g, int n, int nq, const uint8_t* rgb, int16_t* coeffs, const FrameQ* fq,
                              const FastQ* fq32, const double* gk, const float* gk32, jds_frame_stats* st,
                              uint32_t* part, uint32_t* fixbits, uint2* fixlist, unsigned* fixcount, float* dct32, hipStream_t s,
-                             bool finish, int par) {
+                             bool finish, int par, const FixSide* fs) {
   using C = Cfg<MODE>;
+  unsigned* const tilew = fs && !(nq > 1) && MODE != M444 ? fs->tilew : nullptr;
   const bool mq = nq > 1;
   const int nf = n / nq;
   unsigned* const fc = mq ? fixcount : fixcount + par * n;
@@ -1263,7 +1274,7 @@
                            part, fixlist, fixcount, 1, rect, dct32, nullptr, nq);
       else
         hipLaunchKernelGGL((k_fwd32<MODE, PF>), dim3(nout, n), dim3(C::TF), 0, s, g, rgb, coeffs, fq32, gk32, part,
-                           fixlist, fc, 1, rect, nullptr, nullptr, 1);
+                           fixlist, fc, 1, rect, nullptr, nullptr, 1, tilew);
       kmark(s, "k_fwd32<%d,%d%s>", MODE, (int)PF, mq ? ",mq" : "");
       if ((e = hipGetLastError()) != hipSuccess) return e;
     }
@@ -1272,7 +1283,7 @@
                          part, fixlist, fixcount, rect, dct32, st, nq);
     else
       hipLaunchKernelGGL((k_fwd32i<MODE, PF>), dim3(nin, n), dim3(C::TF), 0, s, g, rgb, coeffs, fq32, gk32, part,
-                         fixlist, fc, rect, nullptr, st, 1);
+                         fixlist, fc, rect, nullptr, st, 1, tilew);
     kmark(s, "k_fwd32i<%d,%d%s>", MODE, (int)PF, mq ? ",mq" : "");
     if ((e = hipGetLastError()) != hipSuccess) return e;
   } else {
@@ -1281,7 +1292,7 @@
                          coeffs, fq32, gk32, part, fixlist, fixcount, 0, rect, dct32, st, nq);
     else
       hipLaunchKernelGGL((k_fwd32<MODE, PF>), dim3(g.tiles_y * g.tiles_x, n), dim3(C::TF), 0, s, g, rgb, coeffs,
-                         fq32, gk32, part, fixlist, fc, 0, rect, nullptr, st, 1);
+                         fq32, gk32, part, fixlist, fc, 0, rect, nullptr, st, 1, tilew);
     kmark(s, "k_fwd32<%d,%d%s>", MODE, (int)PF, mq ? ",mq" : "");
     if ((e = hipGetLastError()) != hipSuccess) return e;
   }
@@ -1296,10 +1307,17 @@
   if (!mq) {
     static_assert(C::TF <= 64 * NW_MAX, "row records fit the tile slot");
     const int nred = (ptiles + FIX_RED_TILES - 1) / FIX_RED_TILES;
-    hipLaunchKernelGGL((k_fix_fwd<MODE, PF, 4 * (C::TF / 64)>), dim3(gx + nred, n), dim3(64), 0, s, g, rgb, coeffs,
+    hipStream_t sf = s;
+    if (tilew) {
+      sf = fs->side;
+      if ((e = hipEventRecord(fs->fork, s)) != hipSuccess || (e = hipStreamWaitEvent(sf, fs->fork, 0)) != hipSuccess)
+        return e;
+    }
+    hipLaunchKernelGGL((k_fix_fwd<MODE, PF, 4 * (C::TF / 64)>), dim3(gx + nred, n), dim3(64), 0, sf, g, rgb, coeffs,
                        fq, gk, st, fixlist, fixcount + par * n, nq, 0, fixcount + (par ^ 1) * n, part, ptiles, nred);
-    kmark(s, "k_fix_fwd<%d,%d>", MODE, (int)PF);
+    if (!tilew) kmark(s, "k_fix_fwd<%d,%d>", MODE, (int)PF);
     if ((e = hipGetLastError()) != hipSuccess) return e;
+    if (tilew && (e = hipEventRecord(fs->join, sf)) != hipSuccess) return e;
     return finish ? launch_fwd_finish(g, n, st, nullptr, 0, s) : hipSuccess;
   }
   hipLaunchKernelGGL(k_fwd_reduce_fix, dim3((ptiles + 63) / 64, n), dim3(512), 0, s, g, st, part, ptiles,
@@ -1322,17 +1340,17 @@
 hipError_t launch_fast_fwd(int mode, bool pf, const Geo& g, int n, int nq, const uint8_t* rgb, int16_t* coeffs,
                            const FrameQ* fq, const void* fq32, const double* gk, const float* gk32,
                            jds_frame_stats* st, uint32_t* part, uint32_t* fixbits, uint2* fixlist, unsigned* fixcount, float* dct32,
-                           hipStream_t s, bool finish, int par) {
+                           hipStream_t s, bool finish, int par, const FixSide* fs) {
   const FastQ* f = (const FastQ*)fq32;
   switch (mode) {
     case M420:
-      return pf ? fast_fwd_t<M420, true>(g, n, nq, rgb, coeffs, fq, f, gk, gk32, st, part, fixbits, fixlist, fixcount, dct32, s, finish, par)
-                : fast_fwd_t<M420, false>(g, n, nq, rgb, coeffs, fq, f, gk, gk32, st, part, fixbits, fixlist, fixcount, dct32, s, finish, par);
+      return pf ? fast_fwd_t<M420, true>(g, n, nq, rgb, coeffs, fq, f, gk, gk32, st, part, fixbits, fixlist, fixcount, dct32, s, finish, par, fs)
+                : fast_fwd_t<M420, false>(g, n, nq, rgb, coeffs, fq, f, gk, gk32, st, part, fixbits, fixlist, fixcount, dct32, s, finish, par, fs);
     case M422:
-      return pf ? fast_fwd_t<M422, true>(g, n, nq, rgb, coeffs, fq, f, gk, gk32, st, part, fixbits, fixlist, fixcount, dct32, s, finish, par)
-                : fast_fwd_t<M422, false>(g, n, nq, rgb, coeffs, fq, f, gk, gk32, st, part, fixbits, fixlist, fixcount, dct32, s, finish, par);
+      return pf ? fast_fwd_t<M422, true>(g, n, nq, rgb, coeffs, fq, f, gk, gk32, st, part, fixbits, fixlist, fixcount, dct32, s, finish, par, fs)
+                : fast_fwd_t<M422, false>(g, n, nq, rgb, coeffs, fq, f, gk, gk32, st, part, fixbits, fixlist, fixcount, dct32, s, finish, par, fs);
     default:
-      return fast_fwd_t<M444, false>(g, n, nq, rgb, coeffs, fq, f, gk, gk32, st, part, fixbits, fixlist, fixcount, dct32, s, finish, par);
+      return fast_fwd_t<M444, false>(g, n, nq, rgb, coeffs, fq, f, gk, gk32, st, part, fixbits, fixlist, fixcount, dct32, s, finish, par, fs);
   }
 }
 
diff --git a/jpeg-dsp-studio_amd/csrc/jds_internal.hpp b/jpeg-dsp-studio_amd/csrc/jds_internal.hpp
--- a/jpeg-dsp-studio_amd/csrc/jds_internal.hpp
+++ b/jpeg-dsp-studio_amd/csrc/jds_internal.hpp
@@ -71,6 +71,14 @@
   int probe;
   uint2* list;
   int apriori;
+  unsigned* tilew;
+  hipEvent_t join;
+};
+
+struct FixSide {
+  unsigned* tilew;
+  hipStream_t side;
+  hipEvent_t fork, join;
 };
 
 struct FrameQ {
diff --git a/jpeg-dsp-studio_amd/csrc/jds_inv.hip b/jpeg-dsp-studio_amd/csrc/jds_inv.hip
--- a/jpeg-dsp-studio_amd/csrc/jds_inv.hip
+++ b/jpeg-dsp-studio_amd/csrc/jds_inv.hip
@@ -81,6 +81,43 @@
 }
 
 template <int MODE>
+static int inv_tilemap_t(const Geo& g, int tile, int plane, int by, int bx, int* out) {
+  using I = Inv<MODE>;
+  int n = 0;
+  if (tile < 0) {
+    inv_block_tiles<MODE>(g.H, g.W, g.inv_yoff, plane, by, bx, [&](int t) {
+      if (n < 4) out[n] = t;
+      ++n;
+    });
+    return n;
+  }
+  int nty, ntx;
+  inv_tile_grid<MODE>(g.H, g.W, nty, ntx);
+  if (tile >= nty * ntx) return -1;
+  const InvTasks<MODE> tk(tile / ntx, tile % ntx, g.inv_yoff);
+  auto put = [&](int p, int y, int x) {
+    out[3 * n] = p;
+    out[3 * n + 1] = y;
+    out[3 * n + 2] = x;
+    ++n;
+  };
+  for (int b = 0; b < I::NYB; ++b) {
+    tk.luma(b, by, bx);
+    if (tk.luma_in(g, by, bx)) put(0, by, bx);
+  }
+  for (int p = 1; p <= 2; ++p)
+    for (int b = 0; b < tk.nchroma(); ++b) {
+      tk.chroma(b, by, bx);
+      if (tk.chroma_in(g, by, bx)) put(p, by, bx);
+    }
+  return n;
+}
+int inv_tilemap(int mode, const Geo& g, int tile, int plane, int by, int bx, int* out) {
+  return mode == M420 ? inv_tilemap_t<M420>(g, tile, plane, by, bx, out)
+                      : (mode == M422 ? inv_tilemap_t<M422>(g, tile, plane, by, bx, out) : -1);
+}
+
+template <int MODE>
 static hipError_t inv2_t(const Geo& g, int n, const int16_t* coeffs, const FrameQ* fq, const uint8_t* rgb_in,
                          uint8_t* rgb_out, jds_frame_stats* st, double* part, double* err_y, double* err_rgb,
                          hipStream_t s, int in_div, int fin) {
diff --git a/jpeg-dsp-studio_amd/csrc/jds_inv_common.hpp b/jpeg-dsp-studio_amd/csrc/jds_inv_common.hpp
--- a/jpeg-dsp-studio_amd/csrc/jds_inv_common.hpp
+++ b/jpeg-dsp-studio_amd/csrc/jds_inv_common.hpp
@@ -41,6 +41,69 @@
   }
 };
 
+template <int MODE>
+struct InvCols {
+  int x0, cbx0, cwx0;
+  __host__ __device__ __forceinline__ explicit InvCols(int tx) {
+    using I = Inv<MODE>;
+    x0 = tx * I::TW;
+    cbx0 = x0 / (8 * I::SX) - I::RX;
+    cwx0 = x0 / I::SX - I::RX;
+  }
+};
+
+template <int MODE>
+struct InvTasks {
+  using I = Inv<MODE>;
+  InvRows<MODE> rows;
+  InvCols<MODE> cols;
+  __host__ __device__ __forceinline__ InvTasks(int ty, int tx, int yoff) : rows(ty, yoff), cols(tx) {}
+  __host__ __device__ __forceinline__ void luma(int blk, int& by, int& bx) const {
+    const int bi = blk / I::YBC, bj = blk - bi * I::YBC;
+    by = rows.y0 / 8 + bi;
+    bx = cols.x0 / 8 + bj;
+  }
+  __host__ __device__ __forceinline__ int nchroma() const { return rows.ncbr * I::CBC; }
+  __host__ __device__ __forceinline__ void chroma(int b, int& by, int& bx) const {
+    const int i = b / I::CBC, j = b - i * I::CBC;
+    by = rows.cby0 + i;
+    bx = cols.cbx0 + j;
+  }
+  __host__ __device__ static __forceinline__ bool luma_in(const Geo& g, int by, int bx) {
+    return by >= 0 && by < g.nby && bx < g.nbx;
+  }
+  __host__ __device__ static __forceinline__ bool chroma_in(const Geo& g, int by, int bx) {
+    return by >= 0 && bx >= 0 && by < g.ncy && bx < g.ncx;
+  }
+  __host__ __device__ __forceinline__ bool has_luma(int by, int bx) const {
+    return (unsigned)(by - rows.y0 / 8) < (unsigned)(I::NYB / I::YBC) && (unsigned)(bx - cols.x0 / 8) < (unsigned)I::YBC;
+  }
+  __host__ __device__ __forceinline__ bool has_chroma(int by, int bx) const {
+    return (unsigned)(by - rows.cby0) < (unsigned)rows.ncbr && (unsigned)(bx - cols.cbx0) < (unsigned)I::CBC;
+  }
+};
+
+template <int MODE>
+__host__ __device__ __forceinline__ void inv_tile_grid(int H, int W, int& nty, int& ntx) {
+  nty = (H + Inv<MODE>::TH - 1) / Inv<MODE>::TH;
+  ntx = (W + Inv<MODE>::TW - 1) / Inv<MODE>::TW;
+}
+
+template <int MODE, class F>
+__host__ __device__ __forceinline__ void inv_block_tiles(int H, int W, int yoff, int plane, int by, int bx, F&& f) {
+  using I = Inv<MODE>;
+  int nty, ntx;
+  inv_tile_grid<MODE>(H, W, nty, ntx);
+  const int tyc = (by * 8 * (plane ? I::SY : 1) + yoff) / I::TH, txc = bx * 8 * (plane ? I::SX : 1) / I::TW;
+  const int d = plane ? 1 : 0;
+  for (int ty = tyc - d; ty <= tyc + d; ++ty)
+    for (int tx = txc - d; tx <= txc + d; ++tx) {
+      if ((unsigned)ty >= (unsigned)nty || (unsigned)tx >= (unsigned)ntx) continue;
+      const InvTasks<MODE> t(ty, tx, yoff);
+      if (plane ? t.has_chroma(by, bx) : t.has_luma(by, bx)) f(ty * ntx + tx);
+    }
+}
+
 constexpr int MS = 72;
 
 __device__ __forceinline__ int tslot(int r, int c) { return r * 8 + ((((c >> 1) ^ (r & 3)) << 1) | (c & 1)); }
diff --git a/jpeg-dsp-studio_amd/csrc/jds_inv_exact.hpp b/jpeg-dsp-studio_amd/csrc/jds_inv_exact.hpp
--- a/jpeg-dsp-studio_amd/csrc/jds_inv_exact.hpp
+++ b/jpeg-dsp-studio_amd/csrc/jds_inv_exact.hpp
@@ -149,21 +149,17 @@
 
   const int tid = threadIdx.x, lv = tid & 7, lb = tid >> 3;
   const int ty = tile / tiles_x, tx = tile - ty * tiles_x;
-  const InvRows<MODE> rows(ty, g.inv_yoff);
-  const int Y0 = rows.y0, X0 = tx * I::TW;
+  const InvTasks<MODE> tk(ty, tx, g.inv_yoff);
+  const InvRows<MODE>& rows = tk.rows;
   const int16_t* cf = coeffs + (size_t)frame * g.cpf;
   if (tid < 64) s_q[tid] = (int)fq[frame].q[tid];
   if (XTRA && tid == 0) s_sse = 0ull;
   __syncthreads();
 
-  const int cby0 = rows.cby0, cbx0 = X0 / (8 * I::SX) - I::RX;
-  const int cwy0 = rows.cwy0, cwx0 = X0 / I::SX - I::RX;
+  const int cwy0 = rows.cwy0, cwx0 = tk.cols.cwx0;
   auto luma_blk = [&](int r, int& by, int& bx) {
-    const int blk = r * I::RB + lb;
-    const int bi = blk / I::YBC, bj = blk - bi * I::YBC;
-    by = Y0 / 8 + bi;
-    bx = X0 / 8 + bj;
-    return by >= 0 && by < g.nby && bx < g.nbx;
+    tk.luma(r * I::RB + lb, by, bx);
+    return tk.luma_in(g, by, bx);
   };
   Col16 lq;
   {
@@ -171,10 +167,10 @@
     const bool ok = luma_blk(0, by, bx);
     lq = load_col(cf, ((long long)by * g.nbx + bx) * 64, lv, ok);
   }
-  if (lb < rows.ncbr * I::CBC) {
-    const int i = lb / I::CBC, j = lb - i * I::CBC;
-    const int by = cby0 + i, bx = cbx0 + j;
-    const bool bvalid = by >= 0 && bx >= 0 && by < g.ncy && bx < g.ncx;
+  if (lb < tk.nchroma()) {
+    int by, bx;
+    tk.chroma(lb, by, bx);
+    const bool bvalid = tk.chroma_in(g, by, bx);
     const bool need = rows.need(by, lv);
     const long long boff = ((long long)by * g.ncx + bx) * 64;
     Col16 cq = load_col(cf + g.off_cb, boff, lv, bvalid);
diff --git a/jpeg-dsp-studio_amd/csrc/jds_inv_fast.hip b/jpeg-dsp-studio_amd/csrc/jds_inv_fast.hip
--- a/jpeg-dsp-studio_amd/csrc/jds_inv_fast.hip
+++ b/jpeg-dsp-studio_amd/csrc/jds_inv_fast.hip
@@ -241,19 +241,16 @@
   __shared__ unsigned long long s_sse;
   const int tid = threadIdx.x, lv = tid & 7, lb = tid >> 3;
   const int ty = tile / tiles_x, tx = tile - ty * tiles_x;
-  const InvRows<MODE> rows(ty, g.inv_yoff);
-  const int Y0 = rows.y0, X0 = tx * I::TW;
+  const InvTasks<MODE> tk(ty, tx, g.inv_yoff);
+  const InvRows<MODE>& rows = tk.rows;
   const int16_t* cf = coeffs + (size_t)frame * g.cpf;
   int qhi = 0, qlo = 0;
 
-  const int cby0 = rows.cby0, cbx0 = X0 / (8 * I::SX) - I::RX;
-  const int cwy0 = rows.cwy0, cwx0 = X0 / I::SX - I::RX;
+  const int cbx0 = tk.cols.cbx0;
+  const int cwy0 = rows.cwy0, cwx0 = tk.cols.cwx0;
   auto luma_blk = [&](int r, int& by, int& bx) {
-    const int blk = r * I::RB + lb;
-    const int bi = blk / I::YBC, bj = blk - bi * I::YBC;
-    by = Y0 / 8 + bi;
-    bx = X0 / 8 + bj;
-    return by >= 0 && by < g.nby && bx < g.nbx;
+    tk.luma(r * I::RB + lb, by, bx);
+    return tk.luma_in(g, by, bx);
   };
   auto table_setup = [&]() {
     if (tid < 64) {
@@ -308,34 +305,30 @@
   constexpr bool MIXP = 1 && MODE == M422 && 2 * I::NCB > I::RB && 2 * I::NCB <= 2 * I::RB;
   if constexpr (MIXP) {
     constexpr int NTASK = 2 * I::NCB;
-    auto tinfo = [&](int tt, int& pp, int& ii, int& by, int& bx, bool& ok) -> long long {
+    auto tinfo = [&](int tt, int& pp, int& by, int& bx, bool& ok) -> long long {
       pp = tt >= I::NCB ? 1 : 0;
-      const int b = tt - pp * I::NCB;
-      ii = b / I::CBC;
-      const int jj = b - ii * I::CBC;
-      by = cby0 + ii;
-      bx = cbx0 + jj;
-      ok = tt < NTASK && by >= 0 && bx >= 0 && by < g.ncy && bx < g.ncx;
+      tk.chroma(tt - pp * I::NCB, by, bx);
+      ok = tt < NTASK && tk.chroma_in(g, by, bx);
       return ((long long)by * g.ncx + bx) * 64;
     };
     static_assert(NTASK <= 2 * I::RB, "two tasks per lane group at the most");
-    int p0, p1, ii, by0, bx0, by1, bx1;
+    int p0, p1, by0, bx0, by1, bx1;
     bool ok0, ok1;
-    const long long off0 = tinfo(lb, p0, ii, by0, bx0, ok0);
+    const long long off0 = tinfo(lb, p0, by0, bx0, ok0);
     const Col32 cq0 = load_col32(cf + (p0 ? g.off_cr : g.off_cb), off0, lv, ok0);
     table_setup();
     if (!AP && tid == 0) s_qmax = fq[frame].qmax;
     const bool two = lb + I::RB < NTASK;
-    const long long off1 = tinfo(lb + I::RB, p1, ii, by1, bx1, ok1);
+    const long long off1 = tinfo(lb + I::RB, p1, by1, bx1, ok1);
     Col32 cq1;
     if (two) cq1 = load_col32(cf + (p1 ? g.off_cr : g.off_cb), off1, lv, ok1);
     if (ok0) chroma_task(p0, by0, bx0, cq0);
     if (two && ok1) chroma_task(p1, by1, bx1, cq1);
   } else {
-    const bool ctask = lb < rows.ncbr * I::CBC;
-    const int ci = lb / I::CBC, cj = lb - ci * I::CBC;
-    const int cby = cby0 + ci, cbx = cbx0 + cj;
-    const bool cvalid = ctask && cby >= 0 && cbx >= 0 && cby < g.ncy && cbx < g.ncx;
+    const bool ctask = lb < tk.nchroma();
+    int cby, cbx;
+    tk.chroma(lb, cby, cbx);
+    const bool cvalid = ctask && tk.chroma_in(g, cby, cbx);
     const long long cboff = ((long long)cby * g.ncx + cbx) * 64;
     const Col32 cqb = load_col32(cf + g.off_cb, cboff, lv, cvalid);
     table_setup();
@@ -493,7 +486,6 @@
       sse_y_part[(size_t)frame * gridDim.x + tile] = a;
       atomicAdd((unsigned long long*)&st[frame].sse_rgb, s_sse);
     }
-    if (frame == 0 && tile == 0) *next_count = 0u;
   }
   if constexpr (!AP) __syncthreads();
   return sh.redo != 0;
@@ -505,7 +497,7 @@
            const uint8_t* __restrict__ rgb_in, uint8_t* __restrict__ rgb_out, jds_frame_stats* __restrict__ st,
            double* __restrict__ sse_y_part, unsigned* __restrict__ fixcount, unsigned* __restrict__ next_count,
            unsigned* __restrict__ item_cnt, const int rot, const int probe, const int in_div, const int fix_all,
-           const int fin) {
+           const int fin, unsigned* __restrict__ tilew, const int pass) {
   __shared__ __attribute__((aligned(16))) InvShared<MODE, XTRA> sh;
 #ifdef JDS_PROBE_LDS_PAD
   __shared__ unsigned s_pad[JDS_PROBE_LDS_PAD];
@@ -513,20 +505,26 @@
 #endif
   const int tid = threadIdx.x;
   const int frame = blockIdx.y, tile = blockIdx.x;
-  if (fin >= 0 && tile == 0 && tid == 0) finalize_frame(g, st + frame, fin);
   const unsigned n_items = gridDim.y, ntile = gridDim.x;
+  unsigned* const word = pass ? tilew + ((size_t)frame * ntile + tile) : nullptr;
+  const unsigned listed = pass ? *word : 0u;
+  const bool first = pass != 2, last = pass != 1;
+  if (last && fin >= 0 && tile == 0 && tid == 0) finalize_frame(g, st + frame, fin);
   unsigned* cnt_prev = item_cnt + ((rot + 2) % 3) * n_items;
   unsigned* cnt_now = item_cnt + rot * n_items;
   const unsigned prev = cnt_prev[frame];
-  if (tile == 0 && tid == 0) item_cnt[((rot + 1) % 3) * n_items + frame] = 0u;
   const bool item_exact = !probe && !fix_all && prev * 8u > ntile;
+  if (first && tile == 0 && tid == 0) {
+    item_cnt[((rot + 1) % 3) * n_items + frame] = 0u;
+    if (item_exact) {
+      cnt_now[frame] = prev;
+      atomicAdd(fixcount, ntile);
+    }
+    if (frame == 0) *next_count = 0u;
+  }
+  if (pass && (listed != 0u) != (pass == 2)) return;
   bool redo = false;
   if (item_exact) {
-    if (tile == 0 && tid == 0) {
-      cnt_now[frame] = prev;
-      atomicAdd(fixcount, ntile);
-      if (frame == 0) *next_count = 0u;
-    }
   } else {
     sh.redo = 0;
     redo = inv_fast_tile<MODE, XTRA, AP>(sh, g, tiles_x, frame, tile, coeffs, fq, rgb_in, rgb_out, st, sse_y_part,
@@ -537,6 +535,7 @@
     inv2_tile<MODE, XTRA>(sh, g, tiles_x, ntile, frame, tile, coeffs, fq, rgb_in, rgb_out, st, sse_y_part, nullptr,
                           nullptr, in_div);
 #endif
+  if (pass == 2 && tid == 0) *word = 0u;
 }
 
 #ifdef JDS_INV6
@@ -1268,10 +1267,16 @@
   }
 #endif
   auto go = [&](auto kern, const uint8_t* rin, int xtra, int f) {
-    hipLaunchKernelGGL(kern, grid, blk, 0, s, g, tx, coeffs, fq, rin, rgb_out, st, part, cnt, nxt, fx.item, fx.rot,
-                       fx.probe, in_div, fx.fix_all, f);
-    kmark(s, "k_inv_fast<%d,%d>", MODE, xtra);
-    return hipGetLastError();
+    auto launch = [&](int pass) {
+      hipLaunchKernelGGL(kern, grid, blk, 0, s, g, tx, coeffs, fq, rin, rgb_out, st, part, cnt, nxt, fx.item, fx.rot,
+                         fx.probe, in_div, fx.fix_all, f, fx.tilew, pass);
+      kmark(s, "k_inv_fast<%d,%d>", MODE, xtra);
+      return hipGetLastError();
+    };
+    if (!fx.tilew) return launch(0);
+    hipError_t e = launch(1);
+    if (e == hipSuccess) e = hipStreamWaitEvent(s, fx.join, 0);
+    return e == hipSuccess ? launch(2) : e;
   };
   if (rgb_in != nullptr)
     return fx.apriori ? go(k_inv_fast<MODE, 1, true>, rgb_in, 1, -1) : go(k_inv_fast<MODE, 1, false>, rgb_in, 1, -1);
diff --git a/jpeg-dsp-studio_amd/jds/_abi.py b/jpeg-dsp-studio_amd/jds/_abi.py
--- a/jpeg-dsp-studio_amd/jds/_abi.py
+++ b/jpeg-dsp-studio_amd/jds/_abi.py
@@ -337,6 +337,8 @@
     'jds_selftest_dct16x16': (C.c_int, [_P, _P, C.c_int64, C.c_int32]),
     'jds_selftest_area_tab': (C.c_int, [C.c_int32, C.c_int32, _P, _P, _P]),
     'jds_selftest_inv_rows': (C.c_int, [C.c_int32, C.c_int64, C.c_int32, _P, _P]),
+    'jds_selftest_inv_tilemap': (C.c_int, [C.c_int32, C.c_int64, C.c_int64, C.c_int32, C.c_int32, C.c_int32,
+                                           C.c_int32, _P, _P]),
     'jds_selftest_inv_fast': (C.c_int, [C.c_int32, _P, _P, C.c_int64, C.c_int64, C.c_int32, _P, _P]),
     'jds_selftest_inv_fast16': (C.c_int, [C.c_int32, _P, _P, C.c_int64, C.c_int64, C.c_int32, _P, _P]),
     'jds_selftest_inv_cert': (C.c_int, [_P, C.c_int64, _P, _P, _P]),
```

After: 217,800 Mpixels/s. 0.893x the previous value.
